# cvxgrp/pymde

Hardware: AMD Instinct MI355X
Metric: edges/sec/iter (avg_distortion fwd+bwd), n=1M |E|=50M d=2 (higher is better)
Workload: dtype f32; 1 GPU; BASELINE configs[3] / SURVEY 8d config 4a: n=1000000, |E|=50000000 uniform-random edges (out-degree 50), d=2, penalties.Log1p(1.5), weights in {1,2}; seeded on the device with torch.Generator(0) (the survey's recipe uses numpy default_rng(0): same distribution, another stream; --survey-seed builds that one); parallelism=single GPU, parameter_stream=codebook: 2 distinct weights ride in the packed half-edge word (4 B/half-edge)

## Files before the change

### include/mde_hip.h

```cpp
#ifndef MDE_HIP_H_
#define MDE_HIP_H_

#include <stdint.h>

#ifdef __cplusplus
extern "C" {
#endif

#define MDE_ABI_VERSION 2

#define MDE_OK 0
#define MDE_E_INVALID (-1)
#define MDE_E_SELF_EDGE (-2)
#define MDE_E_RANGE (-3)
#define MDE_E_TOO_LARGE (-4)
#define MDE_E_HIP (-5)
#define MDE_E_UNSUPPORTED (-6)

const char* mde_last_error(void);
int mde_abi_version(void);

enum {
  MDE_F_NONE = 0,
  MDE_F_LINEAR = 1,
  MDE_F_QUADRATIC = 2,
  MDE_F_CUBIC = 3,
  MDE_F_POWER = 4,
  MDE_F_HUBER = 5,
  MDE_F_LOGISTIC = 6,
  MDE_F_SIGMOID = 7,
  MDE_F_HINGE = 8,
  MDE_F_LOG1P = 9,
  MDE_F_LOG = 10,
  MDE_F_INVPOWER = 11,
  MDE_F_LOGRATIO = 12,
  MDE_F_DEADZONE_QUADRATIC = 13,
  MDE_F_DEADZONE_CUBIC = 14,
  MDE_F_CLIPPED_QUADRATIC = 15,
  MDE_F_L_QUADRATIC = 32,
  MDE_F_L_WEIGHTED_QUADRATIC = 33,
  MDE_F_L_HUBER = 34,
  MDE_F_L_CUBIC = 35,
  MDE_F_L_POWER = 36,
  MDE_F_L_WEIGHTED_POWER = 37,
  MDE_F_L_ABSOLUTE = 38,
  MDE_F_L_LOGISTIC = 39,
  MDE_F_L_FRACTIONAL = 40,
  MDE_F_L_SOFT_FRACTIONAL = 41,
  MDE_F_L_CLIPPED_QUADRATIC = 42,
  MDE_F_L_LOG1P = 43
};

typedef struct mde_func {
  int32_t kind;
  int32_t kind_neg;
  const float* a0;
  const float* a1;
  int32_t a0_scalar;
  int32_t a1_scalar;
  float s0, s1, s2;
  float n0, n1, n2;
  int32_t layout;
  const float* e0;
  const float* e1;
} mde_func;

typedef struct mde_plan mde_plan;

int mde_plan_create(int64_t n, int64_t p, const int64_t* edges, int64_t row_lo, int64_t row_hi,
                    void* stream, mde_plan** out);
int mde_plan_destroy(mde_plan* plan);
int64_t mde_plan_n(const mde_plan* plan);
int64_t mde_plan_p(const mde_plan* plan);
int64_t mde_plan_half_edges(const mde_plan* plan);
int64_t mde_plan_row_lo(const mde_plan* plan);
int64_t mde_plan_row_hi(const mde_plan* plan);
const int32_t* mde_plan_rowptr(const mde_plan* plan);
const int32_t* mde_plan_nbr(const mde_plan* plan);
const int32_t* mde_plan_eid(const mde_plan* plan);

int mde_plan_export(const mde_plan* plan, int32_t* rowptr_out, int32_t* nbr_out, int32_t* eid_out,
                    void* stream);

int mde_shard_bounds(int64_t n, int64_t p, const int64_t* edges, int32_t world,
                     int64_t* bounds_host, void* stream);

int mde_plan_expand(const mde_plan* plan, const float* in_edge, float* out_half, void* stream);

int mde_plan_layout(mde_plan* plan, int32_t d, void* stream);
int mde_plan_function_hint(mde_plan* plan, int32_t kind, int32_t kind_neg);
int64_t mde_plan_layout_half_edges(const mde_plan* plan, int32_t layout);
int mde_plan_expand_codebook(const mde_plan* plan, const float* in_edge, float* out_half,
                             int32_t* n_values_host, void* stream);
int mde_plan_expand_bytes(const mde_plan* plan, const float* in_edge, float* out_half,
                          int32_t* n_values_host, void* stream);
int mde_plan_expand_layout(const mde_plan* plan, int32_t layout, const float* in_edge,
                           float* out_half, void* stream);
int mde_plan_ring_info(const mde_plan* plan, int64_t* info_host);
int mde_plan_ring_check(const mde_plan* plan, int64_t* out_host, void* stream);
int mde_plan_row_order(mde_plan* plan, int32_t mode, void* stream, double* info_host);
int mde_plan_loss_double(const mde_plan* plan, double* dst, void* stream);

int mde_edges_deduplicate(int64_t n, int64_t p, const int64_t* edges, int64_t* edges_out,
                          int64_t* count_host, void* stream);
int mde_edges_count_unique(int64_t n, int64_t p, const int64_t* edges, int64_t* edges_out,
                           float* weights_out, int64_t* count_host, void* stream);
int mde_knn(int64_t n, int32_t nf, const float* data, int32_t k, int32_t* idx_out, float* d2_out,
            float* sqn_work, void* stream);
int mde_row_sqnorm(int64_t n, int32_t nf, const float* data, float* out, void* stream);
#define MDE_METRIC_EUCLIDEAN 0
#define MDE_METRIC_COSINE 1
#define MDE_METRIC_CORRELATION 2
#define MDE_METRIC_MANHATTAN 3
int mde_knn_l1(int64_t n, int32_t nf, const float* data, int32_t k, int32_t* idx_out, float* d_out,
               void* stream);
int mde_rows_normalize(int64_t n, int32_t nf, const float* data, int32_t center, float* out,
                       int32_t* deg_out, void* stream);
int mde_pair_distances_metric(int64_t n, int32_t nf, const float* data, int64_t p, const int64_t* edges,
                              int32_t metric, float* out, void* stream);
int mde_ann_search(int32_t nf, int32_t k, int32_t flags, int64_t n_q, const float* Q, const float* q_sqn,
                   int64_t n_qpos, const int32_t* q_map, int64_t n_b, const float* B, const float* b_sqn,
                   int64_t n_bpos, const int32_t* b_map, int64_t n_lists, const int64_t* offsets,
                   int32_t n_probe, const int32_t* probe, int64_t n_tiles, const int64_t* tiles,
                   int32_t* idx_out, float* d2_out, void* stream);
int mde_ann_centroids(int64_t n, int32_t nf, const float* data, int64_t n_members, const int32_t* members,
                      int64_t n_lists, const int64_t* offsets, float* centroids, void* stream);
int mde_sparse_validate(int64_t n, int32_t nf, int64_t nnz, const int64_t* indptr, const int32_t* indices,
                        const float* values, void* stream);
int mde_sparse_knn(int64_t n, int32_t nf, int64_t nnz, const int64_t* indptr, const int32_t* indices,
                   const float* values, int32_t k, int32_t* idx_out, float* d2_out, float* sqn_work,
                   void* stream);
int mde_sparse_distances(int64_t n, int32_t nf, int64_t nnz, const int64_t* indptr, const int32_t* indices,
                         const float* values, int64_t p, const int64_t* edges, float* out, void* stream);
int mde_sparse_rows_normalize(int64_t n, int32_t nf, int64_t nnz, const int64_t* indptr,
                              const int32_t* indices, const float* values, float* values_out,
                              int32_t* deg_out, void* stream);
int mde_graph_shortest_paths(const mde_plan* plan, const float* w, float max_length,
                             double retain_fraction, uint64_t seed, int64_t capacity,
                             int64_t* edges_out, float* dist_out, int64_t* count_host, void* stream);
int mde_knn_pairs(int64_t n, int32_t k, const int32_t* idx, const float* val, float max_value,
                  int64_t* pairs_out, void* stream);
int mde_graph_knn(const mde_plan* plan, const float* w, float max_length, int32_t direct, int32_t k,
                  int32_t* idx_out, float* dist_out, void* stream);
int mde_sample_edges(int64_t n, int64_t num_edges, uint64_t seed, const int64_t* exclude,
                     int64_t n_exclude, int64_t* edges_out, int64_t* count_host, void* stream);

int mde_average_distortion(mde_plan* plan, const float* X, int32_t d, const mde_func* f,
                           float grad_scale, float* grad, float* loss_out, void* stream);

int mde_differences(int64_t n, int64_t p, const int64_t* edges, const float* X, int32_t d,
                    float* diff_out , void* stream);
int mde_distances(int64_t n, int64_t p, const int64_t* edges, const float* X, int32_t d,
                  float* dist_out , void* stream);
int mde_distances_backward(const mde_plan* plan, const float* X, int32_t d, const float* gout,
                           float* grad , void* stream);
int mde_distortions(int64_t p, const float* dist, const mde_func* f, float* out, float* dout,
                    void* stream);

int mde_scatter(const mde_plan* plan, const float* X, int32_t d, const float* gnorm,
                const float* dist, float scale, float* grad, void* stream);

int mde_center(int64_t n, int32_t d, float* Z, double* work, void* stream);
int mde_anchor_rows(int64_t n_anchors, int32_t d, const int64_t* anchors, const float* values,
                    float* Z, void* stream);
int mde_sphere_rows(int64_t n, int32_t d, const float* X, float* Z, float radius, void* stream);
int mde_std_tangent(int64_t n, int32_t d, const float* X, float* Z, double* work, void* stream);
int mde_std_retract(int64_t n, int32_t d, float* Z, int32_t demean, double* work,
                    int32_t* status_dev, void* stream);
int mde_center_step(int64_t n, int32_t d, const float* X, const float* dir, float t, float* Z, double* work,
                    void* stream);
int mde_std_retract_step(int64_t n, int32_t d, const float* X, const float* dir, float t, float* Z,
                         int32_t demean, double* work, int32_t* status_dev, void* stream);
int mde_center_step_begin(int64_t n, int32_t d, const float* X, const float* dir, float t, float* Z, double* work,
                          void* stream);
int mde_center_step_end(int64_t n, int32_t d, float* Z, double* work, double scale, void* stream);
int mde_std_tangent_stats(int64_t n, int32_t d, const float* X, float* Z, const float* dir, double* stats,
                          double* work, void* stream);
int mde_gram(int64_t n, int32_t da, int32_t db, const float* A, const float* B, double* out,
             double* work, void* stream);
int mde_right_multiply(int64_t n, int32_t d, int32_t d2, const float* A, const double* M,
                       float* out, void* stream);
int mde_right_multiply_add(int64_t n, int32_t d, int32_t d2, const float* A, const double* M,
                           float alpha, const float* base, float* out, void* stream);
int mde_shift_rows(int64_t n, int32_t d, const double* shift, float* Z, void* stream);
int mde_row_scale(int64_t n, int32_t d, const float* scale, float* Z, void* stream);
int mde_weighted_degree(const mde_plan* plan, const float* w_plan_order, float* out, void* stream);
int64_t mde_work_doubles(int32_t d);

int mde_axpy(int64_t N, float alpha, const float* x, const float* y, float* out, void* stream);
int mde_vec_stats(int64_t N, const float* g, const float* d, const float* x, double* stats,
                  double* work, void* stream);

typedef struct mde_lbfgs mde_lbfgs;
int mde_lbfgs_create(int64_t N, int32_t history, mde_lbfgs** out);
int mde_lbfgs_destroy(mde_lbfgs* o);
int mde_lbfgs_reset(mde_lbfgs* o);
int32_t mde_lbfgs_count(const mde_lbfgs* o);
int mde_lbfgs_stage(mde_lbfgs* o, const float* g, float* g_prev, const float* d, float t,
                    double* dots, double* work, void* stream);
int mde_lbfgs_commit(mde_lbfgs* o, int32_t accept);
int mde_lbfgs_combine(mde_lbfgs* o, const float* g, float c_g, const float* cs, const float* cy,
                      float* d_out, double* stats, double* work, void* stream);
int mde_lbfgs_dev_reset(mde_lbfgs* o, void* stream);
int mde_lbfgs_dev_step(mde_lbfgs* o, const float* g, float* g_prev, const float* d, float t,
                       float* d_out, double* stats, double* work, void* stream);
int mde_lbfgs_dev_info(const mde_lbfgs* o, int32_t* count_host, int32_t* accepted_host, void* stream);
int mde_lbfgs_dev_stage(mde_lbfgs* o, const float* g, float* g_prev, const float* d, float t, double* work, void* stream);
int mde_lbfgs_dev_finish(mde_lbfgs* o, const float* g, float* d_out, double* stats, double* work, void* stream);
int32_t mde_lbfgs_dev_dots(const mde_lbfgs* o);
int mde_rank_reduce(int32_t world, int32_t count, uint64_t max_mask, const double* in, double* out,
                    int32_t loss_slot, float* loss_out, void* stream);
int mde_lbfgs_debug_knobs(int32_t unfused, int32_t blocks, int32_t spins, int32_t lds_bytes);

int mde_copy_to_host(void* dst_host, const void* src_dev, int64_t bytes, void* stream);

typedef struct mde_turn_desc {
  mde_plan* plan;
  const mde_func* func;
  int64_t n;
  int32_t d, kind;
  float* X[2];
  float* g;
  float* g_prev;
  float* dir;
  float* loss_dev;
  double* board;
  double* work;
  int32_t* status;
  mde_lbfgs* lbfgs;
  void* host_dst;
  const void* tail_src;
  int64_t read_bytes;
  const float* host_loss;
  const int32_t* host_status;
  const double* host_board;
  double seq;
  double pre_id;
} mde_turn_desc;
int mde_turn_enqueue(mde_turn_desc* T, int32_t cur, float t_prev, double f0, double c1, double c2,
                     int32_t allow_pre, void* stream);
int mde_turn_wait(mde_turn_desc* T, int32_t cur, double f0, int32_t allow_next, double c1, double c2,
                  double eps_pre, double* out, void* stream);

#ifdef __cplusplus
}
#endif
#endif
```

### pymde_amd/_lib.py

```python
import ctypes
import os
import threading

import torch

_HERE = os.path.dirname(os.path.abspath(__file__))
LIB_PATH = os.path.join(_HERE, "libmde_hip.so")

c_i32, c_i64, c_f32 = ctypes.c_int32, ctypes.c_int64, ctypes.c_float
c_vp = ctypes.c_void_p

MDE_OK = 0
MDE_E_INVALID, MDE_E_SELF_EDGE, MDE_E_RANGE = -1, -2, -3
MDE_E_TOO_LARGE, MDE_E_HIP, MDE_E_UNSUPPORTED = -4, -5, -6


class MdeFunc(ctypes.Structure):
    _fields_ = [("kind", c_i32), ("kind_neg", c_i32), ("a0", c_vp), ("a1", c_vp),
                ("a0_scalar", c_i32), ("a1_scalar", c_i32),
                ("s0", c_f32), ("s1", c_f32), ("s2", c_f32),
                ("n0", c_f32), ("n1", c_f32), ("n2", c_f32), ("layout", c_i32),
                ("e0", c_vp), ("e1", c_vp)]


class MdeTurnDesc(ctypes.Structure):
    _fields_ = [("plan", c_vp), ("func", c_vp), ("n", c_i64), ("d", c_i32), ("kind", c_i32),
                ("X", c_vp * 2), ("g", c_vp), ("g_prev", c_vp), ("dir", c_vp), ("loss_dev", c_vp),
                ("board", c_vp), ("work", c_vp), ("status", c_vp), ("lbfgs", c_vp),
                ("host_dst", c_vp), ("tail_src", c_vp), ("read_bytes", c_i64),
                ("host_loss", c_vp), ("host_status", c_vp), ("host_board", c_vp), ("seq", ctypes.c_double),
                ("pre_id", ctypes.c_double)]


SYMBOLS = {
    "mde_last_error": (ctypes.c_char_p, []),
    "mde_abi_version": (c_i32, []),
    "mde_plan_create": (c_i32, [c_i64, c_i64, c_vp, c_i64, c_i64, c_vp, ctypes.POINTER(c_vp)]),
    "mde_plan_destroy": (c_i32, [c_vp]),
    "mde_plan_n": (c_i64, [c_vp]),
    "mde_plan_p": (c_i64, [c_vp]),
    "mde_plan_half_edges": (c_i64, [c_vp]),
    "mde_plan_row_lo": (c_i64, [c_vp]),
    "mde_plan_row_hi": (c_i64, [c_vp]),
    "mde_plan_rowptr": (c_vp, [c_vp]),
    "mde_plan_nbr": (c_vp, [c_vp]),
    "mde_plan_eid": (c_vp, [c_vp]),
    "mde_plan_export": (c_i32, [c_vp, c_vp, c_vp, c_vp, c_vp]),
    "mde_shard_bounds": (c_i32, [c_i64, c_i64, c_vp, c_i32, ctypes.POINTER(c_i64), c_vp]),
    "mde_plan_expand": (c_i32, [c_vp, c_vp, c_vp, c_vp]),
    "mde_plan_layout": (c_i32, [c_vp, c_i32, c_vp]),
    "mde_plan_layout_half_edges": (c_i64, [c_vp, c_i32]),
    "mde_plan_ring_info": (c_i32, [c_vp, ctypes.POINTER(c_i64)]),
    "mde_plan_ring_check": (c_i32, [c_vp, ctypes.POINTER(c_i64), c_vp]),
    "mde_plan_row_order": (c_i32, [c_vp, c_i32, c_vp, ctypes.POINTER(ctypes.c_double)]),
    "mde_plan_function_hint": (c_i32, [c_vp, c_i32, c_i32]),
    "mde_plan_loss_double": (c_i32, [c_vp, c_vp, c_vp]),
    "mde_center_step_begin": (c_i32, [c_i64, c_i32, c_vp, c_vp, c_f32, c_vp, c_vp, c_vp]),
    "mde_center_step_end": (c_i32, [c_i64, c_i32, c_vp, c_vp, ctypes.c_double, c_vp]),
    "mde_lbfgs_dev_stage": (c_i32, [c_vp, c_vp, c_vp, c_vp, c_f32, c_vp, c_vp]),
    "mde_lbfgs_dev_finish": (c_i32, [c_vp, c_vp, c_vp, c_vp, c_vp, c_vp]),
    "mde_lbfgs_dev_dots": (c_i32, [c_vp]),
    "mde_rank_reduce": (c_i32, [c_i32, c_i32, ctypes.c_uint64, c_vp, c_vp, c_i32, c_vp, c_vp]),
    "mde_plan_expand_codebook": (c_i32, [c_vp, c_vp, c_vp, ctypes.POINTER(c_i32), c_vp]),
    "mde_plan_expand_bytes": (c_i32, [c_vp, c_vp, c_vp, ctypes.POINTER(c_i32), c_vp]),
    "mde_plan_expand_layout": (c_i32, [c_vp, c_i32, c_vp, c_vp, c_vp]),
    "mde_edges_deduplicate": (c_i32, [c_i64, c_i64, c_vp, c_vp, ctypes.POINTER(c_i64), c_vp]),
    "mde_edges_count_unique": (c_i32, [c_i64, c_i64, c_vp, c_vp, c_vp, ctypes.POINTER(c_i64), c_vp]),
    "mde_knn": (c_i32, [c_i64, c_i32, c_vp, c_i32, c_vp, c_vp, c_vp, c_vp]),
    "mde_row_sqnorm": (c_i32, [c_i64, c_i32, c_vp, c_vp, c_vp]),
    "mde_ann_search": (c_i32, [c_i32, c_i32, c_i32, c_i64, c_vp, c_vp, c_i64, c_vp, c_i64, c_vp, c_vp, c_i64, c_vp,
                               c_i64, c_vp, c_i32, c_vp, c_i64, c_vp, c_vp, c_vp, c_vp]),
    "mde_ann_centroids": (c_i32, [c_i64, c_i32, c_vp, c_i64, c_vp, c_i64, c_vp, c_vp, c_vp]),
    "mde_knn_l1": (c_i32, [c_i64, c_i32, c_vp, c_i32, c_vp, c_vp, c_vp]),
    "mde_rows_normalize": (c_i32, [c_i64, c_i32, c_vp, c_i32, c_vp, c_vp, c_vp]),
    "mde_pair_distances_metric": (c_i32, [c_i64, c_i32, c_vp, c_i64, c_vp, c_i32, c_vp, c_vp]),
    "mde_sparse_rows_normalize": (c_i32, [c_i64, c_i32, c_i64, c_vp, c_vp, c_vp, c_vp, c_vp, c_vp]),
    "mde_knn_pairs": (c_i32, [c_i64, c_i32, c_vp, c_vp, c_f32, c_vp, c_vp]),
    "mde_sparse_validate": (c_i32, [c_i64, c_i32, c_i64, c_vp, c_vp, c_vp, c_vp]),
    "mde_sparse_knn": (c_i32, [c_i64, c_i32, c_i64, c_vp, c_vp, c_vp, c_i32, c_vp, c_vp, c_vp, c_vp]),
    "mde_sparse_distances": (c_i32, [c_i64, c_i32, c_i64, c_vp, c_vp, c_vp, c_i64, c_vp, c_vp, c_vp]),
    "mde_graph_knn": (c_i32, [c_vp, c_vp, c_f32, c_i32, c_i32, c_vp, c_vp, c_vp]),
    "mde_graph_shortest_paths": (c_i32, [c_vp, c_vp, c_f32, ctypes.c_double, ctypes.c_uint64, c_i64,
                                         c_vp, c_vp, ctypes.POINTER(c_i64), c_vp]),
    "mde_sample_edges": (c_i32, [c_i64, c_i64, ctypes.c_uint64, c_vp, c_i64, c_vp,
                                 ctypes.POINTER(c_i64), c_vp]),
    "mde_average_distortion": (c_i32, [c_vp, c_vp, c_i32, ctypes.POINTER(MdeFunc), c_f32, c_vp,
                                       c_vp, c_vp]),
    "mde_differences": (c_i32, [c_i64, c_i64, c_vp, c_vp, c_i32, c_vp, c_vp]),
    "mde_distances": (c_i32, [c_i64, c_i64, c_vp, c_vp, c_i32, c_vp, c_vp]),
    "mde_distances_backward": (c_i32, [c_vp, c_vp, c_i32, c_vp, c_vp, c_vp]),
    "mde_distortions": (c_i32, [c_i64, c_vp, ctypes.POINTER(MdeFunc), c_vp, c_vp, c_vp]),
    "mde_scatter": (c_i32, [c_vp, c_vp, c_i32, c_vp, c_vp, c_f32, c_vp, c_vp]),
    "mde_center": (c_i32, [c_i64, c_i32, c_vp, c_vp, c_vp]),
    "mde_anchor_rows": (c_i32, [c_i64, c_i32, c_vp, c_vp, c_vp, c_vp]),
    "mde_sphere_rows": (c_i32, [c_i64, c_i32, c_vp, c_vp, c_f32, c_vp]),
    "mde_std_tangent": (c_i32, [c_i64, c_i32, c_vp, c_vp, c_vp, c_vp]),
    "mde_std_retract": (c_i32, [c_i64, c_i32, c_vp, c_i32, c_vp, c_vp, c_vp]),
    "mde_center_step": (c_i32, [c_i64, c_i32, c_vp, c_vp, c_f32, c_vp, c_vp, c_vp]),
    "mde_std_retract_step": (c_i32, [c_i64, c_i32, c_vp, c_vp, c_f32, c_vp, c_i32, c_vp, c_vp, c_vp]),
    "mde_std_tangent_stats": (c_i32, [c_i64, c_i32, c_vp, c_vp, c_vp, c_vp, c_vp, c_vp]),
    "mde_gram": (c_i32, [c_i64, c_i32, c_i32, c_vp, c_vp, c_vp, c_vp, c_vp]),
    "mde_right_multiply": (c_i32, [c_i64, c_i32, c_i32, c_vp, c_vp, c_vp, c_vp]),
    "mde_right_multiply_add": (c_i32, [c_i64, c_i32, c_i32, c_vp, c_vp, c_f32, c_vp, c_vp, c_vp]),
    "mde_shift_rows": (c_i32, [c_i64, c_i32, c_vp, c_vp, c_vp]),
    "mde_row_scale": (c_i32, [c_i64, c_i32, c_vp, c_vp, c_vp]),
    "mde_weighted_degree": (c_i32, [c_vp, c_vp, c_vp, c_vp]),
    "mde_work_doubles": (c_i64, [c_i32]),
    "mde_axpy": (c_i32, [c_i64, c_f32, c_vp, c_vp, c_vp, c_vp]),
    "mde_vec_stats": (c_i32, [c_i64, c_vp, c_vp, c_vp, c_vp, c_vp, c_vp]),
    "mde_lbfgs_create": (c_i32, [c_i64, c_i32, ctypes.POINTER(c_vp)]),
    "mde_lbfgs_destroy": (c_i32, [c_vp]),
    "mde_lbfgs_reset": (c_i32, [c_vp]),
    "mde_lbfgs_count": (c_i32, [c_vp]),
    "mde_lbfgs_stage": (c_i32, [c_vp, c_vp, c_vp, c_vp, c_f32, c_vp, c_vp, c_vp]),
    "mde_lbfgs_commit": (c_i32, [c_vp, c_i32]),
    "mde_lbfgs_dev_reset": (c_i32, [c_vp, c_vp]),
    "mde_lbfgs_dev_step": (c_i32, [c_vp, c_vp, c_vp, c_vp, c_f32, c_vp, c_vp, c_vp, c_vp]),
    "mde_lbfgs_debug_knobs": (c_i32, [c_i32, c_i32, c_i32, c_i32]),
    "mde_lbfgs_dev_info": (c_i32, [c_vp, ctypes.POINTER(c_i32), ctypes.POINTER(c_i32), c_vp]),
    "mde_lbfgs_combine": (c_i32, [c_vp, c_vp, c_f32, ctypes.POINTER(c_f32),
                                  ctypes.POINTER(c_f32), c_vp, c_vp, c_vp, c_vp]),
    "mde_copy_to_host": (c_i32, [c_vp, c_vp, c_i64, c_vp]),
    "mde_turn_enqueue": (c_i32, [c_vp, c_i32, c_f32, ctypes.c_double, ctypes.c_double, ctypes.c_double, c_i32, c_vp]),
    "mde_turn_wait": (c_i32, [c_vp, c_i32, ctypes.c_double, c_i32, ctypes.c_double, ctypes.c_double, ctypes.c_double,
                             c_vp, c_vp]),
}

_lib = None
_lock = threading.Lock()


class MdeHipError(RuntimeError):

    def __init__(self, code, message):
        super().__init__("libmde_hip error %d: %s" % (code, message))
        self.code = code
        self.message = message


def load():
    global _lib
    if _lib is not None:
        return _lib
    with _lock:
        if _lib is not None:
            return _lib
        from pymde_amd import _build
        if (not os.path.exists(LIB_PATH) or os.environ.get("PYMDE_AMD_REBUILD")
                or (_build._stale() and _build._hipcc() is not None)):
            _build.build(verbose=bool(os.environ.get("PYMDE_AMD_VERBOSE")))
        if not os.path.exists(LIB_PATH):
            raise ImportError(
                "pymde_amd: %s is missing and could not be built; the HIP extension is the "
                "only compute path (no CPU fallback)" % LIB_PATH)
        lib = ctypes.CDLL(os.environ.get("PYMDE_AMD_LIB_VARIANT") or LIB_PATH)
        for name, (res, args) in SYMBOLS.items():
            fn = getattr(lib, name)
            fn.restype = res
            fn.argtypes = args
        if lib.mde_abi_version() != 2:
            raise ImportError("pymde_amd: ABI version mismatch in %s" % LIB_PATH)
        _lib = lib
    return _lib


def last_error():
    msg = load().mde_last_error()
    return msg.decode(errors="replace") if msg else ""


def check(rc):
    if rc != MDE_OK:
        raise MdeHipError(rc, last_error())


def require_gpu():
    if not torch.cuda.is_available():
        raise RuntimeError(
            "pymde_amd needs an AMD GPU (MI355X / gfx950): torch.cuda.is_available() is False "
            "and there is no CPU path")


def ptr(t):
    return None if t is None else c_vp(t.data_ptr())


def stream_ptr(device=None):
    return c_vp(torch.cuda.current_stream(device).cuda_stream)
```

### pymde_amd/average_distortion.py

```python
import ctypes

import torch

from pymde_amd import _lib
from pymde_amd import util


def _check_X(X, n=None, d=None):
    if not isinstance(X, torch.Tensor) or X.dim() != 2:
        raise ValueError("the embedding must be a 2-D tensor")
    if X.dtype != torch.float32:
        raise ValueError(
            "pymde_amd computes in float32; got an embedding of dtype %s (MDE.embed and "
            "MDE.average_distortion cast float64 inputs with a warning; the kernels themselves do not)" % X.dtype)
    util.require_cuda_device(X.device)
    if n is not None and X.shape[0] != n:
        raise ValueError("embedding has %d rows, the problem has %d items" % (X.shape[0], n))


class EdgePlan(object):

    def __init__(self, n_items, edges, row_lo=0, row_hi=None):
        lib = _lib.load()
        device = util.require_cuda_device(edges.device)
        if edges.dtype != torch.int64 or edges.dim() != 2 or edges.shape[1] != 2:
            raise ValueError("edges must be an int64 tensor of shape (p, 2)")
        self.device = device
        self.n = int(n_items)
        self.p = int(edges.shape[0])
        self.edges = edges.contiguous()
        self.row_lo = int(row_lo)
        self.row_hi = self.n if row_hi is None else int(row_hi)
        handle = ctypes.c_void_p()
        with torch.cuda.device(device):
            rc = lib.mde_plan_create(self.n, self.p, _lib.ptr(self.edges), self.row_lo, self.row_hi,
                                     _lib.stream_ptr(device), ctypes.byref(handle))
        if rc == _lib.MDE_E_SELF_EDGE:
            offending = torch.where(self.edges[:, 0] == self.edges[:, 1])[0]
            raise ValueError(
                "The edge list must not contain self edges; the "
                "following rows were found to be self edges: ", offending.cpu().numpy())
        if rc == _lib.MDE_E_RANGE:
            raise ValueError("edges reference items outside [0, n_items): " + _lib.last_error())
        _lib.check(rc)
        self._handle = handle
        self.half_edges = int(lib.mde_plan_half_edges(handle))

    @property
    def handle(self):
        return self._handle

    @property
    def is_full(self):
        return self.row_lo == 0 and self.row_hi == self.n

    def expand(self, per_edge, layout=0):
        lib = _lib.load()
        t = per_edge.detach().to(device=self.device, dtype=torch.float32).contiguous().reshape(-1)
        if t.numel() != self.p:
            raise ValueError(
                "distortion function has %d parameters but the problem has %d edges"
                % (t.numel(), self.p))
        size = int(lib.mde_plan_layout_half_edges(self._handle, int(layout)))
        out = torch.empty(max(size, 1), dtype=torch.float32, device=self.device)
        with torch.cuda.device(self.device):
            _lib.check(lib.mde_plan_expand_layout(self._handle, int(layout), _lib.ptr(t),
                                                  _lib.ptr(out), _lib.stream_ptr(self.device)))
        return out

    def expand_codebook(self, per_edge):
        lib = _lib.load()
        t = per_edge.detach().to(device=self.device, dtype=torch.float32).contiguous().reshape(-1)
        if t.numel() != self.p:
            return None
        size = int(lib.mde_plan_layout_half_edges(self._handle, 1))
        out = torch.empty(max(size, 1), dtype=torch.float32, device=self.device)
        nv = ctypes.c_int32(0)
        with torch.cuda.device(self.device):
            _lib.check(lib.mde_plan_expand_codebook(self._handle, _lib.ptr(t), _lib.ptr(out),
                                                    ctypes.byref(nv), _lib.stream_ptr(self.device)))
        return out if nv.value > 0 else None

    def expand_bytes(self, per_edge):
        lib = _lib.load()
        t = per_edge.detach().to(device=self.device, dtype=torch.float32).contiguous().reshape(-1)
        if t.numel() != self.p:
            return None
        size = int(lib.mde_plan_layout_half_edges(self._handle, 1))
        out = torch.empty(max(size, 1), dtype=torch.float32, device=self.device)
        nv = ctypes.c_int32(0)
        with torch.cuda.device(self.device):
            _lib.check(lib.mde_plan_expand_bytes(self._handle, _lib.ptr(t), _lib.ptr(out),
                                                 ctypes.byref(nv), _lib.stream_ptr(self.device)))
        return out if nv.value > 0 else None

    def ring_info(self):
        lib = _lib.load()
        info = (ctypes.c_int64 * 16)()
        _lib.check(lib.mde_plan_ring_info(self._handle, info))
        names = ("built", "d", "rows_per_block", "row_blocks", "col_groups", "chunks", "ring_slots", "iterations",
                 "ring_half_edges", "padded_entries", "permuted", "hub_rows", "hub_half_edges", "hub_segments")
        out = {k: int(info[i]) for i, k in enumerate(names)}
        out["built"], out["permuted"] = bool(out["built"]), bool(out["permuted"])
        return out

    def ring_check(self):
        lib = _lib.load()
        out = (ctypes.c_int64 * 3)()
        with torch.cuda.device(self.device):
            _lib.check(lib.mde_plan_ring_check(self._handle, out, _lib.stream_ptr(self.device)))
        return {"split": int(out[0]), "shared": int(out[1]), "pairs": int(out[2])}

    def row_order(self, mode=1):
        lib = _lib.load()
        info = (ctypes.c_double * 4)()
        with torch.cuda.device(self.device):
            _lib.check(lib.mde_plan_row_order(self._handle, int(mode), _lib.stream_ptr(self.device), info))
        return {"in_use": bool(info[0]), "mean_distance_before": float(info[1]),
                "mean_distance_after": float(info[2]), "levels": int(info[3])}

    def csr(self):
        lib = _lib.load()
        nloc = self.row_hi - self.row_lo
        rowptr = torch.empty(nloc + 1, dtype=torch.int32, device=self.device)
        nbr = torch.empty(max(self.half_edges, 1), dtype=torch.int32, device=self.device)
        eid = torch.empty(max(self.half_edges, 1), dtype=torch.int32, device=self.device)
        with torch.cuda.device(self.device):
            _lib.check(lib.mde_plan_export(self._handle, _lib.ptr(rowptr), _lib.ptr(nbr),
                                           _lib.ptr(eid), _lib.stream_ptr(self.device)))
        return rowptr, nbr[:self.half_edges], eid[:self.half_edges]

    def __del__(self):
        h = getattr(self, "_handle", None)
        if h is not None and h.value:
            try:
                _lib.load().mde_plan_destroy(h)
            except Exception:
                pass
            self._handle = None


class Binding(object):

    def __init__(self, plan, function):
        self.plan = plan
        self.function = function
        self.spec = function._hip_spec() if hasattr(function, "_hip_spec") else None
        self._struct = None
        self._keep = None
        self._key = None
        self.codebook = False
        self.byte_stream = False
        self.stream_kind = None

    @property
    def fused(self):
        return self.spec is not None

    def _param_key(self, spec):
        return tuple((a.data_ptr(), a._version, a.numel(), str(a.device)) for a in spec.arrays()) + (
            spec.kind, spec.kind_neg, spec.scalars, spec.scalars_neg)

    def struct(self, d):
        lib = _lib.load()
        spec = self.function._hip_spec()
        key = self._param_key(spec) + (int(d),)
        if self._struct is None or key != self._key:
            plan = self.plan
            with torch.cuda.device(plan.device):
                _lib.check(lib.mde_plan_function_hint(plan.handle, int(spec.kind), int(spec.kind_neg)))
                layout = lib.mde_plan_layout(plan.handle, int(d), _lib.stream_ptr(plan.device))
            if layout < 0:
                _lib.check(layout)

            def prep(a):
                if a is None:
                    return None
                if a.numel() == 1:
                    return a.detach().to(device=plan.device, dtype=torch.float32).reshape(1).contiguous()
                return plan.expand(a, layout)
            a0 = None
            if layout == 1 and spec.a0 is not None and spec.a0.numel() > 1:
                a0 = plan.expand_codebook(spec.a0)
            self.codebook = a0 is not None
            self.byte_stream = False
            if a0 is None and layout == 1 and spec.a0 is not None and spec.a0.numel() > 1:
                a0 = plan.expand_bytes(spec.a0)
                self.byte_stream = a0 is not None
            if a0 is None:
                a0 = prep(spec.a0)
            a1 = prep(spec.a1)
            def edge_order(a):
                if a is None or a.numel() == 1:
                    return None
                return a.detach().to(device=plan.device, dtype=torch.float32).contiguous().reshape(-1)
            e0, e1 = (edge_order(spec.a0), edge_order(spec.a1)) if layout == 1 else (None, None)
            self._keep = (a0, a1, e0, e1)
            self._struct = spec.to_struct(a0, a1)
            self._struct.e0 = e0.data_ptr() if e0 is not None else None
            self._struct.e1 = e1.data_ptr() if e1 is not None else None
            if self.codebook:
                self._struct.a0_scalar = 2
            elif self.byte_stream:
                self._struct.a0_scalar = 3
            self.stream_kind = ("codebook" if self.codebook else "byte index" if self.byte_stream else
                                "scalar" if (spec.a0 is not None and spec.a0.numel() == 1) else "fp32")
            self._struct.layout = layout
            self._key = key
            self.spec = spec
        return self._struct


def fused_evaluate(binding, X, grad_out, loss_out, grad_scale=1.0):
    lib = _lib.load()
    plan = binding.plan
    f = binding.struct(X.shape[1])
    if X.data_ptr() & 15:
        X = X.clone()
    with torch.cuda.device(plan.device):
        _lib.check(lib.mde_average_distortion(
            plan.handle, _lib.ptr(X), X.shape[1], ctypes.byref(f), float(grad_scale),
            _lib.ptr(grad_out), _lib.ptr(loss_out), _lib.stream_ptr(plan.device)))


class _AverageDistortion(torch.autograd.Function):

    @staticmethod
    def forward(ctx, X, binding):
        plan = binding.plan
        _check_X(X, plan.n)
        if not plan.is_full:
            raise ValueError("use pymde_amd.distributed for sharded plans")
        Xc = X.detach().contiguous()
        loss = torch.empty(1, dtype=torch.float32, device=X.device)
        need_grad = X.requires_grad
        if binding.fused:
            grad = torch.empty_like(Xc) if need_grad else None
            fused_evaluate(binding, Xc, grad, loss)
        else:
            grad, value = _unfused(binding, Xc, need_grad)
            loss = value.reshape(1)
        if need_grad:
            ctx.save_for_backward(grad)
        return loss.reshape(())

    @staticmethod
    def backward(ctx, grad_output):
        (grad,) = ctx.saved_tensors
        return grad * grad_output, None


def _unfused(binding, X, need_grad):
    lib = _lib.load()
    plan = binding.plan
    f = binding.function
    n, d = X.shape
    dist = torch.empty(plan.p, dtype=torch.float32, device=X.device)
    with torch.cuda.device(plan.device):
        _lib.check(lib.mde_distances(n, plan.p, _lib.ptr(plan.edges), _lib.ptr(X), d, _lib.ptr(dist),
                                     _lib.stream_ptr(plan.device)))
    if not need_grad:
        with torch.no_grad():
            return None, f(dist).mean().to(torch.float32)
    with torch.enable_grad():
        norms = dist.detach().requires_grad_(True)
        distortion = f(norms).mean()
        (gnorm,) = torch.autograd.grad(distortion, norms)
    gnorm = gnorm.to(torch.float32).contiguous()
    grad = torch.empty_like(X)
    with torch.cuda.device(plan.device):
        _lib.check(lib.mde_scatter(plan.handle, _lib.ptr(X), d, _lib.ptr(gnorm), _lib.ptr(dist), 1.0,
                                   _lib.ptr(grad), _lib.stream_ptr(plan.device)))
    return grad, distortion.detach().to(torch.float32)


def average_distortion(X, binding):
    return _AverageDistortion.apply(X, binding)


class _Norm(torch.autograd.Function):

    @staticmethod
    def forward(ctx, X, plan):
        _check_X(X, plan.n)
        lib = _lib.load()
        Xc = X.detach().contiguous()
        n, d = Xc.shape
        dist = torch.empty(plan.p, dtype=torch.float32, device=X.device)
        with torch.cuda.device(plan.device):
            _lib.check(lib.mde_distances(n, plan.p, _lib.ptr(plan.edges), _lib.ptr(Xc), d,
                                         _lib.ptr(dist), _lib.stream_ptr(plan.device)))
        ctx.plan = plan
        ctx.save_for_backward(Xc)
        return dist

    @staticmethod
    def backward(ctx, grad_output):
        (Xc,) = ctx.saved_tensors
        plan = ctx.plan
        lib = _lib.load()
        gout = grad_output.detach().to(torch.float32).contiguous()
        grad = torch.empty_like(Xc)
        with torch.cuda.device(plan.device):
            _lib.check(lib.mde_distances_backward(plan.handle, _lib.ptr(Xc), Xc.shape[1],
                                                  _lib.ptr(gout), _lib.ptr(grad),
                                                  _lib.stream_ptr(plan.device)))
        return grad, None


def distances(X, plan):
    return _Norm.apply(X, plan)


def differences(X, plan):
    _check_X(X, plan.n)
    lib = _lib.load()
    Xc = X.detach().contiguous()
    n, d = Xc.shape
    out = torch.empty((plan.p, d), dtype=torch.float32, device=X.device)
    with torch.cuda.device(plan.device):
        _lib.check(lib.mde_differences(n, plan.p, _lib.ptr(plan.edges), _lib.ptr(Xc), d,
                                       _lib.ptr(out), _lib.stream_ptr(plan.device)))
    return out


_PLAN_CACHE = {}


def _gather_indices(idx, m):
    return idx[:, None].expand(idx.shape[0], m)


def _average_distortion(X, f, lhs, rhs):
    li = lhs[:, 0] if lhs.dim() == 2 else lhs
    ri = rhs[:, 0] if rhs.dim() == 2 else rhs
    def ident(t):
        return (t.untyped_storage().data_ptr(), t.storage_offset(), tuple(t.stride()), tuple(t.shape), t._version,
                str(t.dtype), str(t.device))
    key = (ident(lhs), ident(rhs), X.shape[0], str(X.device), id(f))
    hit = _PLAN_CACHE.get(key)
    if hit is not None and hit[3] is not f:
        hit = None
    if hit is None:
        edges = torch.stack([li, ri], dim=1).to(device=X.device, dtype=torch.int64).contiguous()
        binding = Binding(EdgePlan(X.shape[0], edges), f)
        if len(_PLAN_CACHE) > 8:
            _PLAN_CACHE.clear()
        hit = _PLAN_CACHE[key] = (binding, lhs.untyped_storage(), rhs.untyped_storage(), f)
    return _AverageDistortion.apply(X, hit[0])
```

### pymde_amd/csrc/mde_plan.h

```cpp
#pragma once
#include "mde_common.h"

struct mde_ring_layout {
  int d = 0;
  int rejected_d = 0;
  float cost_scale = 1.0f;
  int rows_per_block = 0, n_row_blocks = 0;
  int col_groups = 1;
  int chunk_cols = 0, n_chunks = 0;
  int ring_off = 0, slots = 0;
  int64_t n_iters = 0;
  int64_t H = 0;
  uint32_t* packed = nullptr;
  int32_t* eid = nullptr;
  uint32_t* hdr = nullptr;
  int32_t* wave_iter = nullptr;
  float* partial = nullptr;
  int32_t* slot_row = nullptr;
  int count_all = 0;
  int n_hub_rows = 0, n_hub_segs = 0;
  int64_t hub_half_edges = 0;
  int32_t* hub_rows = nullptr;
  int32_t* hub_seg = nullptr;
  int32_t* hub_first = nullptr;
  double* hub_partial = nullptr;
};
#define MDE_HUB_SEG 512

struct mde_plan {
  int64_t n = 0, p = 0, H = 0, row_lo = 0, row_hi = 0;
  int32_t* rowptr = nullptr;
  int32_t* nbr = nullptr;
  int32_t* eid = nullptr;
  double* partials = nullptr;
  float avg_degree = 0.f;
  mde_ring_layout ring;
  int64_t h_offset = 0;
  int32_t* hrow = nullptr;
  float* flat_rec = nullptr;
  int64_t n_tiles = 0;
  int has_empty = 0;
  int32_t* order = nullptr;
  int order_state = 0;
  double order_before = 0.0, order_after = 0.0;
  int order_levels = 0;
};

#define MDE_FLAT_U 4
#define MDE_FLAT_T (64 * MDE_FLAT_U)
int mde_plan_flat(mde_plan* plan, hipStream_t st);

hipError_t mde_sort_pairs_u32(void* tmp, size_t& tmp_bytes, const uint32_t* keys_in, uint32_t* keys_out,
                              const uint32_t* vals_in, uint32_t* vals_out, int n, int begin_bit, int end_bit,
                              hipStream_t st);
hipError_t mde_exclusive_sum_i32(void* tmp, size_t& tmp_bytes, const int32_t* in, int32_t* out, int n, hipStream_t st);
```

### pymde_amd/csrc/mde_ring.hip

```cpp
#include <algorithm>
#include <chrono>
#include <cmath>
#include <cstring>
#include <vector>

#include "mde_ring.h"

#ifndef MDE_RING_BUCKETS
#define MDE_RING_BUCKETS 32
#endif
__global__ __launch_bounds__(64) void k_ring_assign(int nloc, int R, int Q, int NC, int C, int contiguous,
                                                    const int32_t* __restrict__ rowptr,
                                                    const int32_t* __restrict__ nbr, uint32_t* __restrict__ wmap,
                                                    int32_t* __restrict__ wrows) {
  constexpr int B = MDE_RING_BUCKETS, NCWP = MDE_RING_NCW <= 8 ? 8 : 16, LPW = 64 / NCWP, BPL = B / LPW;
  static_assert(MDE_RING_NCW <= 16 && B % LPW == 0 && B <= 64, "lane map of k_ring_assign");
  __shared__ int hist[B];
  __shared__ float cpre[B];
  const int wg = blockIdx.x, rb = wg / Q, g = wg % Q, lane = threadIdx.x;
  const int j_lo = (int)(((int64_t)g * NC + Q - 1) / Q), j_hi = (int)(((int64_t)(g + 1) * NC + Q - 1) / Q);
  const int nj = max(1, j_hi - j_lo);
  const int r0 = rb * R, nr = min(R, nloc - r0);
  const int w = lane / LPW, bg = lane % LPW;
  uint32_t* out = wmap + (size_t)wg * R;
  if (contiguous) {
    const int64_t lo = rowptr[r0], hi = rowptr[r0 + nr];
    int bd[MDE_RING_NCW + 1];
    for (int t = 0; t <= MDE_RING_NCW; ++t) {
      const int64_t target = lo + ((hi - lo) * t) / MDE_RING_NCW;
      int a = r0, b = r0 + nr;
      while (a < b) {
        const int mid = (a + b) >> 1;
        if (rowptr[mid] >= target) b = mid; else a = mid + 1;
      }
      bd[t] = (t == MDE_RING_NCW) ? r0 + nr : a;
    }
    for (int r = lane; r < nr; r += 64) {
      int ww = 0;
      for (int t = 1; t < MDE_RING_NCW; ++t) ww += (bd[t] <= r0 + r);
      out[r] = (uint32_t)ww | ((uint32_t)(r0 + r - bd[ww]) << 8);
    }
    if (lane < MDE_RING_NCW) wrows[wg * MDE_RING_NCW + lane] = bd[lane + 1] - bd[lane];
    return;
  }
  float P[BPL], T[BPL];
#pragma unroll
  for (int k = 0; k < BPL; ++k) P[k] = T[k] = 0.0f;
  int myrows = 0;
  for (int r = 0; r < nr; ++r) {
    const int beg = rowptr[r0 + r], end = rowptr[r0 + r + 1];
    if (lane < B) hist[lane] = 0;
    __syncthreads();
    for (int q = beg + lane; q < end; q += 64) {
      const int j = nbr[q] / C;
      if (j >= j_lo && j < j_hi) atomicAdd(&hist[(int)(((int64_t)(j - j_lo) * B) / nj)], 1);
    }
    __syncthreads();
    int h = lane < B ? hist[lane] : 0;
#pragma unroll
    for (int o = 1; o < B; o <<= 1) {
      const int t = __shfl_up(h, o, 64);
      if (lane >= o) h += t;
    }
    if (lane < B) cpre[lane] = (float)h;
    __syncthreads();
    float c[BPL], cost = 0.0f;
#pragma unroll
    for (int k = 0; k < BPL; ++k) {
      c[k] = cpre[bg * BPL + k];
      cost = fmaf(P[k] - T[k] * (1.0f / MDE_RING_NCW), c[k], cost);
    }
#pragma unroll
    for (int o = 1; o < LPW; o <<= 1) cost += __shfl_xor(cost, o, 64);
    float bc = w < MDE_RING_NCW ? cost : 3.0e38f;
    int bn = myrows, bw = w;
#pragma unroll
    for (int o = LPW; o < 64; o <<= 1) {
      const float oc = __shfl_xor(bc, o, 64);
      const int on = __shfl_xor(bn, o, 64), ow = __shfl_xor(bw, o, 64);
      const bool take = oc < bc || (oc == bc && (on < bn || (on == bn && ow < bw)));
      bc = take ? oc : bc;
      bn = take ? on : bn;
      bw = take ? ow : bw;
    }
    if (lane == 0) out[r] = (uint32_t)bw | ((uint32_t)bn << 8);
#pragma unroll
    for (int k = 0; k < BPL; ++k) {
      T[k] += c[k];
      if (w == bw) P[k] += c[k];
    }
    myrows += (w == bw);
  }
  if (bg == 0 && w < MDE_RING_NCW) wrows[wg * MDE_RING_NCW + w] = myrows;
}

__global__ __launch_bounds__(MDE_BLOCK) void k_ring_keys(int nrows, const int32_t* __restrict__ rowptr,
                                                         const int32_t* __restrict__ nbr,
                                                         const uint32_t* __restrict__ wmap, int R, int Q,
                                                         int NC, int C, int JB, uint32_t* __restrict__ keys,
                                                         uint32_t* __restrict__ vals, int32_t* __restrict__ hrow) {
  constexpr int G = 16;
  const int lig = threadIdx.x & (G - 1);
  const int group = (blockIdx.x * MDE_BLOCK + threadIdx.x) / G;
  const int ngroups = (gridDim.x * MDE_BLOCK) / G;
  const int rmax = ((nrows + ngroups - 1) / ngroups) * ngroups;
  for (int r = group; r < rmax; r += ngroups) {
    const bool has = r < nrows;
    const int beg = has ? rowptr[r] : 0, end = has ? rowptr[r + 1] : 0;
    const int rb = has ? r / R : 0;
    const uint32_t wv = (has && lig < Q) ? (wmap[((size_t)rb * Q + lig) * R + (r - rb * R)] & 0xffu) : 0u;
    for (int q0 = beg; q0 < end; q0 += G) {
      const int q = q0 + lig;
      const bool in = q < end;
      const uint32_t j = in ? (uint32_t)(nbr[q] / C) : 0u;
      const uint32_t g = (uint32_t)(((uint64_t)j * (uint64_t)Q) / (uint64_t)NC);
      const uint32_t w = (uint32_t)__shfl((int)wv, (int)g, G);
      if (in) {
        keys[q] = ((((uint32_t)rb * (uint32_t)Q + g) * MDE_RING_NCW + w) << JB) | j;
        vals[q] = (uint32_t)q;
        hrow[q] = r;
      }
    }
  }
}

__global__ __launch_bounds__(64) void k_ring_assign_slots(int R, int Q, const int32_t* __restrict__ slot_cum,
                                                          uint32_t* __restrict__ wmap, int32_t* __restrict__ wrows) {
  const int wg = blockIdx.x, rb = wg / Q, lane = threadIdx.x;
  const int s0 = rb * R;
  uint32_t* out = wmap + (size_t)wg * R;
  const int64_t lo = slot_cum[s0], hi = slot_cum[s0 + R];
  int bd[MDE_RING_NCW + 1];
  for (int t = 0; t <= MDE_RING_NCW; ++t) {
    const int64_t target = lo + ((hi - lo) * t) / MDE_RING_NCW;
    int a = s0, b = s0 + R;
    while (a < b) {
      const int mid = (a + b) >> 1;
      if (slot_cum[mid] >= target) b = mid; else a = mid + 1;
    }
    bd[t] = (t == MDE_RING_NCW) ? s0 + R : a;
  }
  for (int r = lane; r < R; r += 64) {
    int ww = 0;
    for (int t = 1; t < MDE_RING_NCW; ++t) ww += (bd[t] <= s0 + r);
    out[r] = (uint32_t)ww | ((uint32_t)(s0 + r - bd[ww]) << 8);
  }
  if (lane < MDE_RING_NCW) wrows[wg * MDE_RING_NCW + lane] = bd[lane + 1] - bd[lane];
}

__global__ __launch_bounds__(MDE_BLOCK) void k_ring_keys_slots(int64_t H, const int32_t* __restrict__ nbr,
                                                               const int32_t* __restrict__ row_slot,
                                                               const uint32_t* __restrict__ wmap, int R, int Q, int NC, int C,
                                                               int JB, uint32_t nseg, uint32_t* __restrict__ keys,
                                                               uint32_t* __restrict__ vals, int32_t* __restrict__ hrow) {
  for (int64_t q = (int64_t)blockIdx.x * MDE_BLOCK + threadIdx.x; q < H; q += (int64_t)gridDim.x * MDE_BLOCK) {
    const int sl = row_slot[hrow[q]];
    vals[q] = (uint32_t)q;
    if (sl < 0) {
      keys[q] = nseg << JB;
      hrow[q] = 0;
      continue;
    }
    const int rb = sl / R;
    const uint32_t j = (uint32_t)(nbr[q] / C);
    const uint32_t g = (uint32_t)(((uint64_t)j * (uint64_t)Q) / (uint64_t)NC);
    const uint32_t w = wmap[((size_t)rb * Q + g) * R + (sl - rb * R)] & 0xffu;
    keys[q] = ((((uint32_t)rb * (uint32_t)Q + g) * MDE_RING_NCW + w) << JB) | j;
    hrow[q] = sl;
  }
}
__global__ __launch_bounds__(MDE_BLOCK) void k_ring_rows_to_slots(int64_t H, const int32_t* __restrict__ row_slot,
                                                                  int32_t* __restrict__ hrow) {
  for (int64_t q = (int64_t)blockIdx.x * MDE_BLOCK + threadIdx.x; q < H; q += (int64_t)gridDim.x * MDE_BLOCK)
    hrow[q] = max(row_slot[hrow[q]], 0);
}

__global__ __launch_bounds__(MDE_BLOCK) void k_ring_gather_u32(int64_t H, const uint32_t* __restrict__ idx,
                                                               const uint32_t* __restrict__ in,
                                                               uint32_t* __restrict__ out) {
  for (int64_t h = (int64_t)blockIdx.x * MDE_BLOCK + threadIdx.x; h < H; h += (int64_t)gridDim.x * MDE_BLOCK)
    out[h] = in[idx[h]];
}

__global__ __launch_bounds__(MDE_BLOCK) void k_ring_hrow(int nrows, const int32_t* __restrict__ rowptr,
                                                         int32_t* __restrict__ hrow) {
  constexpr int G = 16;
  const int lig = threadIdx.x & (G - 1);
  const int group = (blockIdx.x * MDE_BLOCK + threadIdx.x) / G;
  const int ngroups = (gridDim.x * MDE_BLOCK) / G;
  for (int r = group; r < nrows; r += ngroups)
    for (int q = rowptr[r] + lig; q < rowptr[r + 1]; q += G) hrow[q] = r;
}

__global__ __launch_bounds__(MDE_BLOCK) void k_ring_seg(int64_t H, uint32_t nseg, int JB,
                                                        const uint32_t* __restrict__ keys,
                                                        int32_t* __restrict__ seg) {
  for (int64_t h = (int64_t)blockIdx.x * MDE_BLOCK + threadIdx.x; h <= H;
       h += (int64_t)gridDim.x * MDE_BLOCK) {
    const int64_t prev = (h == 0) ? -1 : (int64_t)(keys[h - 1] >> JB);
    int64_t cur = (h == H) ? (int64_t)nseg : (int64_t)(keys[h] >> JB);
    if (cur > (int64_t)nseg) cur = nseg;
    for (int64_t t = prev + 1; t <= cur; ++t) seg[t] = (int32_t)h;
  }
}

#ifndef MDE_RING_FORCE
#define MDE_RING_FORCE 3
#endif
#ifndef MDE_RING_CARRY
#define MDE_RING_CARRY 256
#endif
#ifndef MDE_RING_ROUNDS
#define MDE_RING_ROUNDS 6
#endif
__host__ __device__ constexpr int ring_cls_shift(int d) { return d == 2 ? 3 : (d == 4 ? 4 : 2); }
__host__ __device__ constexpr int ring_cls_mask(int d) { return d == 4 ? 15 : 31; }
__global__ __launch_bounds__(MDE_BLOCK) void k_ring_meta(int64_t H, const uint32_t* __restrict__ keys,
                                                         const uint32_t* __restrict__ vals,
                                                         const int32_t* __restrict__ hrow,
                                                         const int32_t* __restrict__ nbr,
                                                         const uint32_t* __restrict__ wmap, int JB, int R, int Q, int d,
                                                         uint32_t* __restrict__ meta) {
  const int sh = ring_cls_shift(d), cm = ring_cls_mask(d), rowbytes = 4 * d;
  for (int64_t pos = (int64_t)blockIdx.x * MDE_BLOCK + threadIdx.x; pos < H; pos += (int64_t)gridDim.x * MDE_BLOCK) {
    const uint32_t q = vals[pos];
    const int wg = (int)((keys[pos] >> JB) / MDE_RING_NCW), rb = wg / Q;
    const uint32_t row = (uint32_t)(hrow[q] - rb * R);
    const uint32_t rc = ((row * (uint32_t)rowbytes) >> sh) & (uint32_t)cm;
    const uint32_t cc = (((uint32_t)nbr[q] * (uint32_t)rowbytes) >> sh) & (uint32_t)cm;
    meta[pos] = (wmap[(size_t)wg * R + row] >> 8) | (rc << 16) | (cc << 24);
  }
}

template <bool FILL>
__global__ __launch_bounds__(64) void k_ring_schedule(int nseg, const int32_t* __restrict__ seg,
                                                      const int32_t* __restrict__ wrows,
                                                      const uint32_t* __restrict__ keys,
                                                      const uint32_t* __restrict__ meta, uint32_t JM, int SPAN,
                                                      int R, int Q, int NC, int d, int cap, int bail_factor,
                                                      int32_t* __restrict__ iters,
                                                      const int32_t* __restrict__ iter_base,
                                                      int32_t* __restrict__ it_ent, int32_t* __restrict__ it_cnt,
                                                      int32_t* __restrict__ it_m, int flag_rows,
                                                      const int32_t* __restrict__ caps) {
  extern __shared__ int flag[];
  __shared__ int cq_pos[2][MDE_RING_CARRY];
  __shared__ uint32_t cq_meta[2][MDE_RING_CARRY];
  __shared__ int cq_chunk[2][MDE_RING_CARRY];
  __shared__ int cq_age[2][MDE_RING_CARRY];
  __shared__ int em[64], em_row[64];
  __shared__ int rcnt[32], ccnt[32];
  const int i = blockIdx.x, lane = threadIdx.x;
  if (i >= nseg) return;
  for (int r = lane; r < flag_rows; r += 64) flag[r] = 0x7fffffff;
  __syncthreads();
  const int beg = seg[i], end = seg[i + 1];
  constexpr int row_base = 0;
  const int first = FILL ? iter_base[i] : 0;
  int out = first, next = beg, nc = 0, cur = 0;
  const int nrows_w = max(1, wrows[i]);
  const int per_it = nrows_w < 64 ? nrows_w : 64;
  const int walk = 2 * ((NC / Q + SPAN + 1) / (SPAN + 1));
  const int bail = caps ? caps[i] - 4
                        : ((!FILL && bail_factor > 0) ? bail_factor * max((end - beg + per_it - 1) / per_it, walk) + 64 : 0x7fffffff);
  int last_chunk = (int)(((int64_t)((i / MDE_RING_NCW) % Q) * NC + Q - 1) / Q);
  int m_lead = 0;
  while (nc > 0 || next < end) {
    const int m = nc > 0 ? cq_chunk[cur][0] : (int)(keys[next] & JM);
    if (((out - first) & 1) == 0) m_lead = m;
    const int lim = m_lead + SPAN;
    int nem = 0, nnew = 0, mx = 0;
    if (lane < 32) rcnt[lane] = ccnt[lane] = 0;
    __syncthreads();
    auto offer = [&](int pos, uint32_t mw, int chunk, int age, int prio) {
      const int row = pos >= 0 ? (int)(mw & 0xffffu) - row_base : 0;
      const int rc = pos >= 0 ? (int)((mw >> 16) & 0xffu) : -1, cc = pos >= 0 ? (int)(mw >> 24) : -2;
      if (pos >= 0) atomicMin(&flag[row], prio);
      __syncthreads();
      const bool rowwin = pos >= 0 && flag[row] == prio;
      int rkR = 0, rkC = 0;
      const int rcw = rowwin ? rc : -1, ccw = rowwin ? cc : -2;
      for (int c = 0; c < 32; ++c) {
        const unsigned long long mr = __ballot(rcw == c), mc = __ballot(ccw == c);
        if (rc == c) rkR = __popcll(mr & ((1ull << lane) - 1ull));
        if (cc == c) rkC = __popcll(mc & ((1ull << lane) - 1ull));
      }
      const bool capok = rowwin && (rcnt[rc] + rkR < cap) && (ccnt[cc] + rkC < cap);
      const bool win = rowwin && (capok || age >= MDE_RING_FORCE);
      const unsigned long long wm = __ballot(win);
      const int widx = nem + __popcll(wm & ((1ull << lane) - 1ull));
      const bool emit = win && widx < 64;
      if (emit) {
        em[widx] = pos;
        em_row[widx] = row;
        atomicAdd(&rcnt[rc], 1);
        atomicAdd(&ccnt[cc], 1);
      }
      mx = max(mx, emit ? chunk : 0);
      const bool lose = pos >= 0 && !emit;
      const unsigned long long lm = __ballot(lose);
      const int lidx = nnew + __popcll(lm & ((1ull << lane) - 1ull));
      if (lose && lidx < MDE_RING_CARRY) {
        cq_pos[cur ^ 1][lidx] = pos;
        cq_meta[cur ^ 1][lidx] = mw;
        cq_chunk[cur ^ 1][lidx] = chunk;
        cq_age[cur ^ 1][lidx] = win ? age : age + 1;
      }
      nem += __popcll(__ballot(emit));
      nnew += __popcll(lm);
      __syncthreads();
    };
    int prio = 0;
    for (int c0 = 0; c0 < nc; c0 += 64) {
      const int k = c0 + lane;
      const bool has = k < nc;
      offer(has ? cq_pos[cur][k] : -1, has ? cq_meta[cur][k] : 0u, has ? cq_chunk[cur][k] : 0, has ? cq_age[cur][k] : 0,
            prio + lane);
      prio += 64;
    }
    for (int round = 0; round < MDE_RING_ROUNDS && nem < 64 && next < end && nnew + 64 <= MDE_RING_CARRY; ++round) {
      const int want = 64 - nem;
      const int cand = next + lane;
      const bool in = lane < want && cand < end;
      const int chunk = in ? (int)(keys[cand] & JM) : 0x7fffffff;
      const bool take = in && chunk <= lim;
      const int ntake = __popcll(__ballot(take));
      if (ntake == 0) break;
      offer(take ? cand : -1, take ? meta[cand] : 0u, chunk, 0, prio + lane);
      prio += 64;
      next += ntake;
    }
    if (lane < nem) flag[em_row[lane]] = 0x7fffffff;
    for (int k = lane; k < nnew; k += 64) flag[(int)(cq_meta[cur ^ 1][k] & 0xffffu) - row_base] = 0x7fffffff;
    mx = mde_wave_max(mx);
    if (nem > 0) last_chunk = mx;
    if (FILL) {
      if (lane < nem) it_ent[(size_t)out * 64 + lane] = em[lane];
      if (lane == 0) {
        it_cnt[out] = nem | (last_chunk << 8);
        it_m[out] = m;
      }
    }
    ++out;
    nc = nnew;
    cur ^= 1;
    __syncthreads();
    if (out - first > bail) {
      if (lane == 0) iters[i] = 1 << 25;
      return;
    }
  }
  while ((out - first) & 3) {
    if (FILL && lane == 0) {
      it_cnt[out] = 0 | (last_chunk << 8);
      it_m[out] = last_chunk;
    }
    ++out;
  }
  if (iters && lane == 0) iters[i] = out - first;
}

__global__ __launch_bounds__(MDE_BLOCK) void k_ring_caps(int nseg, const int32_t* __restrict__ seg,
                                                         const int32_t* __restrict__ wrows, int R, int Q, int NC, int SPAN,
                                                         int factor, int32_t* __restrict__ caps) {
  const int i = blockIdx.x * MDE_BLOCK + threadIdx.x;
  if (i > nseg) return;
  if (i == nseg) {
    caps[i] = 0;
    return;
  }
  const int nrows_w = max(1, wrows[i]);
  const int per_it = nrows_w < 64 ? nrows_w : 64;
  const int walk = 2 * ((NC / Q + SPAN + 1) / (SPAN + 1));
  const int need = max((seg[i + 1] - seg[i] + per_it - 1) / per_it, walk);
  caps[i] = (factor * need + 64 + 4 + 3) & ~3;
}

__device__ __forceinline__ int ring_place_wave(bool act, int rc, int lane) {
  const unsigned long long lt = (1ull << lane) - 1ull;
  int rank = 0, par = 0, oddacc = 0;
  for (int c = 0; c < 32; ++c) {
    const unsigned long long m = __ballot(act && rc == c);
    if (rc == c) {
      rank = __popcll(m & lt);
      par = oddacc & 1;
    }
    oddacc += __popcll(m) & 1;
  }
  const int half = (rank + par) & 1;
  int quarter = 0;
  for (int h = 0; h < 2; ++h) {
    int oa = 0;
    for (int c = 0; c < 16; ++c) {
      const unsigned long long m = __ballot(act && half == h && (rc & 15) == c);
      if (half == h && (rc & 15) == c) quarter = (__popcll(m & lt) + (oa & 1)) & 1;
      oa += __popcll(m) & 1;
    }
  }
  int pos = 0;
  for (int g = 0; g < 4; ++g) {
    const unsigned long long m = __ballot(act && half * 2 + quarter == g);
    if (half * 2 + quarter == g) pos = __popcll(m & lt);
  }
  return half * 32 + quarter * 16 + pos;
}

__global__ __launch_bounds__(MDE_BLOCK) void k_ring_pack(int64_t nit, int nseg, const int32_t* __restrict__ iter_base,
                                                         const int32_t* __restrict__ src_base,
                                                         const int32_t* __restrict__ it_ent,
                                                         const int32_t* __restrict__ it_cnt,
                                                         const int32_t* __restrict__ it_m,
                                                         const uint32_t* __restrict__ keys,
                                                         const uint32_t* __restrict__ vals,
                                                         const int32_t* __restrict__ hrow,
                                                         const int32_t* __restrict__ nbr,
                                                         const int32_t* __restrict__ eid, int R, int Q, int C, int S,
                                                         int ring_off, int JB, int d, int row_lo, int place, int count_all,
                                                         uint32_t* __restrict__ packed,
                                                         int32_t* __restrict__ peid, uint32_t* __restrict__ hdr) {
  __shared__ uint8_t s_taken[MDE_BLOCK / 64][64], s_free[MDE_BLOCK / 64][64];
  __shared__ uint32_t s_prow[MDE_BLOCK / 64][64];
  const int lane = threadIdx.x & 63, wv = threadIdx.x >> 6;
  const int64_t nw = ((int64_t)gridDim.x * MDE_BLOCK) >> 6;
  const uint32_t JM = (1u << JB) - 1u;
  const int sh = ring_cls_shift(d), cm = ring_cls_mask(d);
  const uint32_t cbytes = (uint32_t)C * 4u * (uint32_t)d;
  for (int64_t itb = (int64_t)blockIdx.x * (MDE_BLOCK / 64); itb < nit; itb += nw) {
    const int64_t it = itb + wv;
    const bool valid = it < nit;
    int64_t src = it;
    if (valid && src_base) {
      int lo = 0, hi = nseg;
      while (hi - lo > 1) {
        const int mid = (lo + hi) >> 1;
        if ((int64_t)iter_base[mid] <= it) lo = mid; else hi = mid;
      }
      src = (int64_t)src_base[lo] + (it - (int64_t)iter_base[lo]);
    }
    const int cw = valid ? __builtin_amdgcn_readfirstlane(it_cnt[src]) : 0;
    const int cnt = cw & 0xff;
    const bool act = valid && lane < cnt;
    uint32_t key = 0, q = 0, col = 0, rowaddr = 0, ring = 0;
    int grow = 0, rcls = 0;
    if (act) {
      const int pos = it_ent[(size_t)src * 64 + lane];
      key = keys[pos];
      q = vals[pos];
      const int rb = (int)((key >> JB) / MDE_RING_NCW) / Q;
      grow = hrow[q];
      rowaddr = (uint32_t)(grow - rb * R) * 4u * (uint32_t)d;
      const uint32_t j = key & JM;
      col = (uint32_t)nbr[q];
      ring = (uint32_t)ring_off + (j % (uint32_t)S) * cbytes + (col - j * (uint32_t)C) * 4u * (uint32_t)d;
      rcls = (int)((rowaddr >> sh) & (uint32_t)cm);
    }
    s_taken[wv][lane] = 0;
    s_prow[wv][lane] = 0xffffffffu;
    __syncthreads();
    const bool second = (it & 1) != 0;
    int l = lane;
    if (!second) {
      if (place) l = ring_place_wave(act, rcls, lane);
      if (act) {
        s_taken[wv][l] = 1;
        s_prow[wv][l] = rowaddr;
      }
    }
    __syncthreads();
    int pin = -1;
    if (second) {
      const uint32_t prow = s_prow[wv - 1][lane];
#pragma unroll 8
      for (int k = 0; k < 64; ++k)
        if ((uint32_t)__builtin_amdgcn_readlane((int)prow, k) == rowaddr) pin = k;
      pin = act ? pin : -1;
      if (place) l = ring_place_wave(act && pin < 0, rcls, lane);
      if (pin >= 0) {
        l = pin;
        s_taken[wv][l] = 1;
      }
    }
    __syncthreads();
    const bool moved = second && act && pin < 0 && s_taken[wv][l];
    if (second && act && !moved) s_taken[wv][l] = 1;
    __syncthreads();
    {
      const bool fr = !s_taken[wv][lane];
      const unsigned long long fm = __ballot(fr);
      if (fr) s_free[wv][__popcll(fm & ((1ull << lane) - 1ull))] = (uint8_t)lane;
    }
    __syncthreads();
    const unsigned long long mvm = __ballot(moved);
    const int nmoved = __popcll(mvm);
    if (moved) l = s_free[wv][__popcll(mvm & ((1ull << lane) - 1ull))];
    const bool counts = act && (count_all || (uint32_t)(row_lo + grow) < col);
    const int ncount = __popcll(__ballot(counts));
    const uint32_t lclass = ncount == 0 ? 0u : (ncount == cnt ? 1u : 2u);
    const uint32_t m = valid ? (uint32_t)__builtin_amdgcn_readfirstlane(it_m[src]) : 0u;
    const uint32_t need = max((uint32_t)(cw >> 8), m);
    const uint32_t mpad = valid ? (uint32_t)__builtin_amdgcn_readfirstlane(it_m[src & ~(int64_t)1]) : 0u;
    const size_t base = ((size_t)(it >> 2) * 64) * 4 + (size_t)(it & 3);
    if (act) {
      packed[base + (size_t)l * 4] = ring_pack_word(d, rowaddr, ring);
      peid[base + (size_t)l * 4] = eid[q];
    } else if (valid) {
      const int lf = s_free[wv][nmoved + lane - cnt];
      packed[base + (size_t)lf * 4] = ring_pack_word(d, (uint32_t)(R + (lf & 31)) * 4u * (uint32_t)d,
                                                     (uint32_t)ring_off + (mpad % (uint32_t)S) * cbytes);
      peid[base + (size_t)lf * 4] = -1;
    }
    if (lane == 0 && valid) {
      hdr[MDE_RING_HW * it] = m;
      hdr[MDE_RING_HW * it + 1] = need;
      hdr[MDE_RING_HW * it + 2] = lclass;
      hdr[MDE_RING_HW * it + 3] = (cnt < 64 ? MDE_RING_H3_PAD : 0u) | ((uint32_t)cnt << 8);
    }
    __syncthreads();
  }
}

__global__ __launch_bounds__(MDE_BLOCK) void k_ring_block_class(int64_t nblocks, uint32_t* __restrict__ hdr) {
  const int64_t b = (int64_t)blockIdx.x * MDE_BLOCK + threadIdx.x;
  if (b >= nblocks) return;
  bool any0 = false, any1 = false, any2 = false;
  for (int q = 0; q < 4; ++q) {
    const uint32_t* h = hdr + (size_t)MDE_RING_HW * (4 * b + q);
    if ((h[3] >> 8) == 0u) continue;
    any0 |= h[2] == 0u;
    any1 |= h[2] == 1u;
    any2 |= h[2] == 2u;
  }
  const uint32_t cls = (any2 || (any0 && any1)) ? 2u : (any1 ? 1u : 0u);
  hdr[(size_t)MDE_RING_HW * 4 * b + 3] = (hdr[(size_t)MDE_RING_HW * 4 * b + 3] & ~3u) | cls;
  for (int t = 0; t < 2; ++t) {
    uint32_t* h0 = hdr + (size_t)MDE_RING_HW * (4 * b + 2 * t);
    uint32_t* h1 = h0 + MDE_RING_HW;
    uint32_t need = h0[0];
    if ((h0[3] >> 8) != 0u) need = max(need, h0[1]);
    if ((h1[3] >> 8) != 0u) need = max(need, h1[1]);
    h0[1] = need;
  }
}

__global__ __launch_bounds__(MDE_BLOCK) void k_ring_stats(int64_t nit, const uint32_t* __restrict__ hdr,
                                                          unsigned long long* __restrict__ stats) {
  unsigned long long a = 0, b = 0, c = 0;
  for (int64_t i = (int64_t)blockIdx.x * MDE_BLOCK + threadIdx.x; i < nit; i += (int64_t)gridDim.x * MDE_BLOCK) {
    a += (hdr[MDE_RING_HW * i + 3] & MDE_RING_H3_PAD) ? 1u : 0u;
    b += hdr[MDE_RING_HW * i + 2] == 1u;
    c += hdr[MDE_RING_HW * i + 2] == 2u;
  }
  a = mde_wave_sum(a);
  b = mde_wave_sum(b);
  c = mde_wave_sum(c);
  if ((threadIdx.x & 63) == 0) {
    atomicAdd(&stats[0], a);
    atomicAdd(&stats[1], b);
    atomicAdd(&stats[2], c);
  }
}

__global__ __launch_bounds__(MDE_BLOCK) void k_ring_sweep_balance(int nwg, int ngroups, int GW, int JB,
                                                                  const uint32_t* __restrict__ keys,
                                                                  const int32_t* __restrict__ seg,
                                                                  unsigned long long* __restrict__ crit,
                                                                  unsigned long long* __restrict__ tot) {
  const int64_t idx = (int64_t)blockIdx.x * MDE_BLOCK + threadIdx.x;
  if (idx >= (int64_t)nwg * ngroups) return;
  const int wg = (int)(idx / ngroups), g = (int)(idx % ngroups);
  unsigned long long mx = 0, sm = 0;
  for (int w = 0; w < MDE_RING_NCW; ++w) {
    const uint32_t s = (uint32_t)wg * MDE_RING_NCW + (uint32_t)w;
    const int32_t lo = seg[s], hi = seg[s + 1];
    const uint64_t k0 = ((uint64_t)s << JB) + (uint64_t)g * GW, k1 = k0 + (uint64_t)GW;
    auto lower = [&](uint64_t key) {
      int32_t a = lo, b = hi;
      while (a < b) {
        const int32_t m = a + ((b - a) >> 1);
        if ((uint64_t)keys[m] < key) a = m + 1; else b = m;
      }
      return a;
    };
    const unsigned long long c = (unsigned long long)(lower(k1) - lower(k0));
    mx = c > mx ? c : mx;
    sm += c;
  }
  if (sm) {
    atomicAdd(&crit[wg], mx);
    atomicAdd(&tot[wg], sm);
  }
}

static int panel_mode() {
  const char* e = getenv("MDE_PANEL");
  return e ? atoi(e) : -1;
}

static int bits_for_u64(uint64_t maxval) {
  int b = 1;
  while (b < 64 && (maxval >> b)) ++b;
  return b;
}

struct RingSizes {
  int R, NRB, Q, C, NC, S, JB, ring_off, span, qmax;
};

static double ring_time_us(double iters_per_wave, int NC, int Q, int nwg) {
  const double rounds = std::ceil((double)nwg / 256.0);
  return rounds * std::max(0.21 * iters_per_wave, 0.14 * (double)NC / (double)Q);
}
static double csr_time_us(const mde_plan* plan, int d) {
  return (double)plan->H * ((int64_t)plan->n * d * 4 >= (6 << 20) ? 1.3e-5 : 0.6e-5);
}
static bool mid_regime(const mde_plan* plan, int d) {
  return (int64_t)plan->n * d * 4 < (6 << 20) && plan->H < ((int64_t)16 << 20);
}
#define MDE_RING_FIXED_US 11.0
#define MDE_CSR_FIXED_US 7.0
static double function_cost_scale(int kind, int kind_neg) {
  if (kind_neg != MDE_F_NONE) return 1.3;
  switch (kind) {
    case MDE_F_LOG1P: case MDE_F_QUADRATIC: case MDE_F_LINEAR: case MDE_F_CUBIC: case MDE_F_INVPOWER: case MDE_F_HUBER:
    case MDE_F_L_QUADRATIC: case MDE_F_L_WEIGHTED_QUADRATIC: case MDE_F_L_ABSOLUTE: case MDE_F_L_HUBER: case MDE_F_L_CUBIC:
      return 1.05;
    case MDE_F_LOGISTIC: case MDE_F_POWER: case MDE_F_LOG: case MDE_F_SIGMOID: case MDE_F_HINGE: case MDE_F_LOGRATIO:
    case MDE_F_L_POWER: case MDE_F_L_LOGISTIC: case MDE_F_L_FRACTIONAL: case MDE_F_L_SOFT_FRACTIONAL:
      return 1.35;
    default:
      return 2.7;
  }
}
extern "C" int mde_plan_function_hint(mde_plan* plan, int32_t kind, int32_t kind_neg) {
  if (!plan) return MDE_E_INVALID;
  plan->ring.cost_scale = (float)function_cost_scale(kind, kind_neg);
  return MDE_OK;
}

static int choose_col_groups(const mde_plan* plan, int64_t nrb, int qmax, int64_t nc) {
  int Q = (int)std::min<int64_t>(qmax, std::max<int64_t>(1, 256 / nrb));
  const double its1 = 1.4 * (double)plan->H / ((double)nrb * MDE_RING_NCW * 64.0);
  auto cost = [&](int q) {
    const double rounds = std::ceil((double)(nrb * q) / 256.0);
    return ring_time_us(its1 / q, (int)nc, q, (int)(nrb * q)) + 4.0 * rounds;
  };
  const double base = cost(Q);
  double best = base;
  for (int q = 1; q <= qmax; ++q)
    if ((int64_t)nrb * q <= MDE_MAX_PARTIALS && cost(q) < 0.95 * base && cost(q) < best) {
      best = cost(q);
      Q = q;
    }
  if (getenv("MDE_RING_Q")) Q = std::max(1, std::min(qmax, atoi(getenv("MDE_RING_Q"))));
  return Q;
}

static bool choose_sizes(const mde_plan* plan, int d, RingSizes* z) {
  const int64_t nloc = plan->row_hi - plan->row_lo;
  if (d < 1 || d > 4 || nloc <= 0 || plan->H <= 0) return false;
  const int mode = panel_mode();
  if (mode == 0) return false;
  const int C = ring_chunk_cols(d);
  const int64_t nc = (plan->n + C - 1) / C;
  if (nc > 65535 || nc < 2) return false;
  const int minch = getenv("MDE_RING_MINCH") ? std::max(1, atoi(getenv("MDE_RING_MINCH"))) : 10;
  const int qmax = (int)std::min<int64_t>(16, std::max<int64_t>(1, nc / minch));
  int64_t pr = (nloc * qmax + 255) / 256;
  if (pr < 64 * MDE_RING_NCW) pr = 64 * MDE_RING_NCW;
  if (getenv("MDE_RING_ROWS")) pr = atoi(getenv("MDE_RING_ROWS"));
  if (pr > nloc) pr = nloc;
  pr = ((pr + 63) / 64) * 64;
  const int64_t pr_max = ring_row_cap(d);
  if (pr > pr_max) pr = pr_max;
  const int64_t nrb = (nloc + pr - 1) / pr;
  int Q = choose_col_groups(plan, nrb, qmax, nc);
  if (nrb * Q > MDE_MAX_PARTIALS) return false;
  const int jb = bits_for_u64((uint64_t)nc - 1);
  if (bits_for_u64((uint64_t)(nrb * Q * MDE_RING_NCW)) + jb > 32) return false;
  if (mode != 1) {
    if (mid_regime(plan, d) && d != 2 && d != 3) return false;
  }
  const int S = ring_slots_for(d, (int)pr);
  if (S < 6) return false;
  int span = ring_max_span(S);
  if (getenv("MDE_RING_SPAN")) span = std::min(S - 2, std::max(1, atoi(getenv("MDE_RING_SPAN"))));
  if (mode != 1) {
    const double its = 1.4 * (double)plan->H / ((double)nrb * Q * MDE_RING_NCW * 64.0);
    if (ring_time_us(its, (int)nc, Q, (int)(nrb * Q)) > 0.75 * csr_time_us(plan, d)) return false;
    if (mid_regime(plan, d) &&
        plan->ring.cost_scale * ring_time_us(its, (int)nc, Q, (int)(nrb * Q)) + MDE_RING_FIXED_US >
            0.7 * (csr_time_us(plan, d) + MDE_CSR_FIXED_US))
      return false;
  }
  z->qmax = qmax;
  z->R = (int)pr;
  z->NRB = (int)nrb;
  z->Q = Q;
  z->C = C;
  z->NC = (int)nc;
  z->S = S;
  z->ring_off = ring_off_for(d, (int)pr);
  z->span = span;
  z->JB = jb;
  return true;
}

static void ring_free(mde_ring_layout& L) {
  if (L.packed) (void)hipFree(L.packed);
  if (L.eid) (void)hipFree(L.eid);
  if (L.hdr) (void)hipFree(L.hdr);
  if (L.wave_iter) (void)hipFree(L.wave_iter);
  if (L.partial) (void)hipFree(L.partial);
  void* extra[] = {L.slot_row, L.hub_rows, L.hub_seg, L.hub_first, L.hub_partial};
  for (void* q : extra)
    if (q) (void)hipFree(q);
  L = mde_ring_layout();
}
void mde_ring_release(mde_plan* plan) { ring_free(plan->ring); }

struct RowPlan {
  bool mapped = false, permuted = false;
  int nrb = 0;
  int64_t H_ring = 0;
  std::vector<int32_t> row_slot;
  std::vector<int32_t> slot_row;
  std::vector<int32_t> slot_cum;
  std::vector<int32_t> hub_rows, hub_first, hub_seg;
  int64_t hub_half_edges = 0;
  int threshold = 0;
};

static int plan_rows(const mde_plan* plan, const RingSizes& z, hipStream_t st, RowPlan* rp) {
  const int64_t nloc = plan->row_hi - plan->row_lo;
  const int R = z.R;
  rp->nrb = z.NRB;
  rp->H_ring = plan->H;
  const char* e_hub = getenv("MDE_RING_HUB");
  const char* e_perm = getenv("MDE_RING_PERMUTE");
  const int hub_env = e_hub ? atoi(e_hub) : -1, perm_env = e_perm ? atoi(e_perm) : -1;
  if (hub_env == 0 && perm_env == 0) return MDE_OK;
  std::vector<int32_t> rowptr((size_t)nloc + 1);
  MDE_HIP(hipMemcpyAsync(rowptr.data(), plan->rowptr, rowptr.size() * sizeof(int32_t), hipMemcpyDeviceToHost, st));
  MDE_HIP(hipStreamSynchronize(st));
  const int64_t H = plan->H;
  int T = (int)std::max<int64_t>(256, H / ((int64_t)z.NRB * MDE_RING_NCW * 128));
  if (hub_env > 0) T = hub_env;
  rp->threshold = T;
  int64_t hub_he = 0;
  int32_t max_deg = 0;
  if (hub_env != 0) {
    for (int64_t r = 0; r < nloc; ++r) {
      const int32_t deg = rowptr[r + 1] - rowptr[r];
      max_deg = std::max(max_deg, deg);
      if (deg > T) {
        rp->hub_rows.push_back((int32_t)r);
        hub_he += deg;
      }
    }
    if (2 * hub_he > H) {
      rp->hub_rows.clear();
      hub_he = 0;
    }
  }
  const bool peel = !rp->hub_rows.empty();
  bool permute = perm_env == 1;
  if (perm_env < 0) {
    int64_t heaviest = 0;
    size_t hi = 0;
    for (int b = 0; b < z.NRB; ++b) {
      const int64_t r0 = (int64_t)b * R, r1 = std::min<int64_t>(nloc, r0 + R);
      int64_t w = rowptr[r1] - rowptr[r0];
      while (hi < rp->hub_rows.size() && rp->hub_rows[hi] < r1) {
        w -= rowptr[rp->hub_rows[hi] + 1] - rowptr[rp->hub_rows[hi]];
        ++hi;
      }
      heaviest = std::max(heaviest, w);
    }
    permute = z.NRB > 1 && (double)heaviest > 1.08 * (double)(H - hub_he) / (double)z.NRB;
  }
  if (!peel && !permute) return MDE_OK;
  rp->mapped = true;
  rp->permuted = permute;
  rp->hub_half_edges = hub_he;
  rp->H_ring = H - hub_he;
  rp->row_slot.assign((size_t)nloc, -1);
  std::vector<uint8_t> is_hub((size_t)nloc, 0);
  for (int32_t r : rp->hub_rows) is_hub[(size_t)r] = 1;
  if (!permute) {
    rp->slot_cum.assign((size_t)z.NRB * R + 1, 0);
    int64_t cum = 0;
    for (int64_t r = 0; r < (int64_t)z.NRB * R; ++r) {
      rp->slot_cum[(size_t)r] = (int32_t)cum;
      if (r < nloc && !is_hub[(size_t)r]) {
        rp->row_slot[(size_t)r] = (int32_t)r;
        cum += rowptr[r + 1] - rowptr[r];
      }
    }
    rp->slot_cum[(size_t)z.NRB * R] = (int32_t)cum;
  } else {
    const int64_t nring = nloc - (int64_t)rp->hub_rows.size();
    const int nrb = (int)std::max<int64_t>(1, (nring + R - 1) / R);
    rp->nrb = nrb;
    int32_t dmax = 0;
    for (int64_t r = 0; r < nloc; ++r)
      if (!is_hub[(size_t)r]) dmax = std::max(dmax, rowptr[r + 1] - rowptr[r]);
    std::vector<int64_t> start((size_t)dmax + 2, 0);
    for (int64_t r = 0; r < nloc; ++r)
      if (!is_hub[(size_t)r]) ++start[(size_t)(dmax - (rowptr[r + 1] - rowptr[r])) + 1];
    for (size_t k = 1; k < start.size(); ++k) start[k] += start[k - 1];
    std::vector<int32_t> block((size_t)nloc, -1);
    for (int64_t r = 0; r < nloc; ++r) {
      if (is_hub[(size_t)r]) continue;
      const int64_t rank = start[(size_t)(dmax - (rowptr[r + 1] - rowptr[r]))]++;
      const int64_t pos = rank % (2 * (int64_t)nrb);
      block[(size_t)r] = (int32_t)(pos < nrb ? pos : 2 * (int64_t)nrb - 1 - pos);
    }
    std::vector<int32_t> fill((size_t)nrb, 0);
    rp->slot_row.assign((size_t)nrb * R, -1);
    std::vector<int32_t> slot_deg((size_t)nrb * R, 0);
    for (int64_t r = 0; r < nloc; ++r) {
      const int b = block[(size_t)r];
      if (b < 0) continue;
      const int sidx = fill[(size_t)b]++;
      if (sidx >= R) {
        mde_set_error("ring layout: a row block overflowed while the rows were dealt (internal error)");
        return MDE_E_INVALID;
      }
      const size_t sl = (size_t)b * R + (size_t)sidx;
      rp->slot_row[sl] = (int32_t)r;
      rp->row_slot[(size_t)r] = (int32_t)sl;
      slot_deg[sl] = rowptr[r + 1] - rowptr[r];
    }
    rp->slot_cum.assign((size_t)nrb * R + 1, 0);
    int64_t cum = 0;
    for (size_t t = 0; t < (size_t)nrb * R; ++t) {
      rp->slot_cum[t] = (int32_t)cum;
      cum += slot_deg[t];
    }
    rp->slot_cum[(size_t)nrb * R] = (int32_t)cum;
  }
  rp->hub_first.reserve(rp->hub_rows.size() + 1);
  for (size_t i = 0; i < rp->hub_rows.size(); ++i) {
    rp->hub_first.push_back((int32_t)(rp->hub_seg.size() / 4));
    const int32_t r = rp->hub_rows[i];
    for (int64_t b = rowptr[r]; b < rowptr[r + 1]; b += MDE_HUB_SEG) {
      rp->hub_seg.push_back((int32_t)i);
      rp->hub_seg.push_back((int32_t)b);
      rp->hub_seg.push_back((int32_t)std::min<int64_t>(rowptr[r + 1], b + MDE_HUB_SEG));
      rp->hub_seg.push_back(0);
    }
  }
  rp->hub_first.push_back((int32_t)(rp->hub_seg.size() / 4));
  if (getenv("MDE_RING_STATS"))
    fprintf(stderr, "[mde ring] rows: threshold %d half-edges, max degree %d, %zu hub rows with %lld half-edges (%.2f%%) peeled into %zu "
            "segments; blocks %s (%d)\n", T, max_deg, rp->hub_rows.size(), (long long)hub_he, 100.0 * (double)hub_he / (double)std::max<int64_t>(H, 1),
            rp->hub_seg.size() / 4, permute ? "DEALT by degree" : "of consecutive rows", rp->nrb);
  return MDE_OK;
}

static hipError_t any_stream_bailed(const int32_t* iters, int nseg, hipStream_t st, int32_t* total) {
  std::vector<int32_t> h((size_t)nseg);
  hipError_t e = hipMemcpyAsync(h.data(), iters, h.size() * sizeof(int32_t), hipMemcpyDeviceToHost, st);
  if (e == hipSuccess) e = hipStreamSynchronize(st);
  if (e != hipSuccess) return e;
  for (int i = 0; i < nseg; ++i)
    if (h[(size_t)i] >= (1 << 25)) {
      *total = -1;
      break;
    }
  return hipSuccess;
}

static int build_ring(mde_plan* plan, int d, hipStream_t st) {
  RingSizes z;
  if (!choose_sizes(plan, d, &z)) return 0;
  const int64_t nloc = plan->row_hi - plan->row_lo;
  const int64_t H = plan->H;
  RowPlan rp;
  {
    const int rc = plan_rows(plan, z, st, &rp);
    if (rc != MDE_OK) return rc;
    if (rp.mapped && rp.nrb != z.NRB) {
      z.NRB = rp.nrb;
      z.Q = choose_col_groups(plan, z.NRB, z.qmax, z.NC);
      if ((int64_t)z.NRB * z.Q > MDE_MAX_PARTIALS || bits_for_u64((uint64_t)((int64_t)z.NRB * z.Q * MDE_RING_NCW)) + z.JB > 32) return 0;
    }
  }
  const int64_t H_ring = rp.H_ring;
  if (H_ring <= 0) return 0;
  const int nseg = z.NRB * z.Q * MDE_RING_NCW;
  const uint32_t JM = (1u << z.JB) - 1u;
  uint32_t *keys = nullptr, *vals = nullptr, *keys2 = nullptr, *vals2 = nullptr, *packed = nullptr, *hdr = nullptr, *wmap = nullptr;
  int32_t *hrow = nullptr, *wrows = nullptr, *seg = nullptr, *iters = nullptr, *iter_base = nullptr;
  int32_t *it_ent = nullptr, *it_cnt = nullptr, *it_m = nullptr, *peid = nullptr;
  int32_t *row_slot = nullptr, *slot_cum = nullptr, *slot_row = nullptr, *hub_rows = nullptr, *hub_seg = nullptr, *hub_first = nullptr;
  double* hub_partial = nullptr;
  float* partial = nullptr;
  void* tmp = nullptr;
  hipError_t e = hipSuccess;
  auto release = [&](bool all) {
    void* scratch[] = {keys, vals, keys2, vals2, hrow, wrows, wmap, seg, iters, it_ent, it_cnt, it_m, tmp, row_slot, slot_cum};
    for (void* p : scratch)
      if (p) (void)hipFree(p);
    if (all) {
      void* outs[] = {packed, hdr, peid, iter_base, partial, slot_row, hub_rows, hub_seg, hub_first, hub_partial};
      for (void* p : outs)
        if (p) (void)hipFree(p);
    }
  };
  auto fail = [&](hipError_t err, const char* what) {
    release(true);
    return mde_hip_fail(err, what, __FILE__, __LINE__);
  };
#define RB(call)                                 \
  do {                                           \
    e = (call);                                  \
    if (e != hipSuccess) return fail(e, #call);  \
  } while (0)
  const bool stats_on = getenv("MDE_RING_STATS") != nullptr;
  auto t_last = std::chrono::steady_clock::now();
  auto tick = [&](const char* what) {
    if (!stats_on) return;
    (void)hipStreamSynchronize(st);
    const auto t1 = std::chrono::steady_clock::now();
    fprintf(stderr, "[mde ring build] %-28s %8.2f ms\n", what, std::chrono::duration<double, std::milli>(t1 - t_last).count());
    t_last = t1;
  };
  const size_t hb = (size_t)H * sizeof(uint32_t);
  RB(hipMalloc(&keys, hb));
  RB(hipMalloc(&vals, hb));
  RB(hipMalloc(&keys2, hb));
  RB(hipMalloc(&vals2, hb));
  RB(hipMalloc(&hrow, hb));
  RB(hipMalloc(&wrows, ((size_t)nseg + 1) * sizeof(int32_t)));
  RB(hipMalloc(&wmap, (size_t)z.NRB * z.Q * z.R * sizeof(uint32_t)));
  RB(hipMalloc(&seg, ((size_t)nseg + 1) * sizeof(int32_t)));
  RB(hipMalloc(&iters, ((size_t)nseg + 1) * sizeof(int32_t)));
  RB(hipMalloc(&iter_base, ((size_t)nseg + 1) * sizeof(int32_t)));
  tick("scratch allocations");
  const int contiguous = getenv("MDE_RING_ASSIGN") ? atoi(getenv("MDE_RING_ASSIGN")) == 0 : 1;
  auto upload = [&](int32_t** dst, const std::vector<int32_t>& src) -> hipError_t {
    hipError_t er = hipMalloc(dst, std::max<size_t>(src.size(), 1) * sizeof(int32_t));
    if (er == hipSuccess && !src.empty()) er = hipMemcpyAsync(*dst, src.data(), src.size() * sizeof(int32_t), hipMemcpyHostToDevice, st);
    return er;
  };
  if (rp.mapped) {
    RB(upload(&row_slot, rp.row_slot));
    RB(upload(&slot_cum, rp.slot_cum));
    if (rp.permuted) RB(upload(&slot_row, rp.slot_row));
    if (!rp.hub_rows.empty()) {
      RB(upload(&hub_rows, rp.hub_rows));
      RB(upload(&hub_seg, rp.hub_seg));
      RB(upload(&hub_first, rp.hub_first));
      RB(hipMalloc(&hub_partial, (rp.hub_seg.size() / 4) * 8 * sizeof(double)));
    }
    hipLaunchKernelGGL(k_ring_assign_slots, dim3(z.NRB * z.Q), dim3(64), 0, st, z.R, z.Q, slot_cum, wmap, wrows);
    RB(hipGetLastError());
    tick("slot -> wave assignment");
    hipLaunchKernelGGL(k_ring_hrow, dim3(mde_grid(nloc * 16, MDE_BLOCK, 4096)), dim3(MDE_BLOCK), 0, st, (int)nloc, plan->rowptr, hrow);
    RB(hipGetLastError());
    hipLaunchKernelGGL(k_ring_keys_slots, dim3(mde_grid(H, MDE_BLOCK, 8192)), dim3(MDE_BLOCK), 0, st, H, plan->nbr, row_slot, wmap, z.R,
                       z.Q, z.NC, z.C, z.JB, (uint32_t)nseg, keys, vals, hrow);
    RB(hipGetLastError());
  } else {
    hipLaunchKernelGGL(k_ring_assign, dim3(z.NRB * z.Q), dim3(64), 0, st, (int)nloc, z.R, z.Q, z.NC, z.C, contiguous, plan->rowptr,
                       plan->nbr, wmap, wrows);
    RB(hipGetLastError());
    tick("row -> wave assignment");
    hipLaunchKernelGGL(k_ring_keys, dim3(mde_grid(nloc * 16, MDE_BLOCK, 4096)), dim3(MDE_BLOCK), 0, st, (int)nloc,
                       plan->rowptr, plan->nbr, wmap, z.R, z.Q, z.NC, z.C, z.JB, keys, vals, hrow);
    RB(hipGetLastError());
  }
  tick("keys kernel");
  size_t tmp_bytes = 0, scan_bytes = 0;
  const int end_bit = std::min(32, bits_for_u64((uint64_t)nseg) + z.JB);
  RB(mde_sort_pairs_u32(nullptr, tmp_bytes, keys, keys2, vals, vals2, (int)H, 0, end_bit, st));
  RB(mde_exclusive_sum_i32(nullptr, scan_bytes, iters, iter_base, nseg + 1, st));
  if (scan_bytes > tmp_bytes) tmp_bytes = scan_bytes;
  RB(mde_sort_pairs_u32(nullptr, scan_bytes, keys, keys2, vals, vals2, (int)H, 0,
                                        bits_for_u64((uint64_t)plan->n), st));
  if (scan_bytes > tmp_bytes) tmp_bytes = scan_bytes;
  RB(hipMalloc(&tmp, tmp_bytes ? tmp_bytes : 16));
  tick("sort size queries + temp allocation");
  const bool by_column = getenv("MDE_RING_BYCOL") ? atoi(getenv("MDE_RING_BYCOL")) != 0
                                                  : (double)H_ring > 0.5 * (double)nloc * (double)z.NC;
  if (by_column) {
    RB(hipMemcpyAsync(keys2, plan->nbr, hb, hipMemcpyDeviceToDevice, st));
    uint32_t* skey = reinterpret_cast<uint32_t*>(hrow);
    RB(hipMemcpyAsync(skey, keys, hb, hipMemcpyDeviceToDevice, st));
    RB(mde_sort_pairs_u32(tmp, tmp_bytes, keys2, keys, vals, vals2, (int)H, 0,
                                          bits_for_u64((uint64_t)plan->n), st));
    hipLaunchKernelGGL(k_ring_gather_u32, dim3(mde_grid(H, MDE_BLOCK, 4096)), dim3(MDE_BLOCK), 0, st, H, vals2, skey, keys);
    RB(hipGetLastError());
    RB(hipMemcpyAsync(vals, vals2, hb, hipMemcpyDeviceToDevice, st));
    hipLaunchKernelGGL(k_ring_hrow, dim3(mde_grid(nloc * 16, MDE_BLOCK, 4096)), dim3(MDE_BLOCK), 0, st, (int)nloc,
                       plan->rowptr, hrow);
    RB(hipGetLastError());
    if (rp.mapped) {
      hipLaunchKernelGGL(k_ring_rows_to_slots, dim3(mde_grid(H, MDE_BLOCK, 8192)), dim3(MDE_BLOCK), 0, st, H, row_slot, hrow);
      RB(hipGetLastError());
    }
  }
  RB(mde_sort_pairs_u32(tmp, tmp_bytes, keys, keys2, vals, vals2, (int)H, 0, end_bit, st));
  tick("radix sort");
  hipLaunchKernelGGL(k_ring_seg, dim3(mde_grid(H + 1, MDE_BLOCK, 4096)), dim3(MDE_BLOCK), 0, st, H, (uint32_t)nseg,
                     z.JB, keys2, seg);
  RB(hipGetLastError());
  RB(hipMemsetAsync(iters, 0, ((size_t)nseg + 1) * sizeof(int32_t), st));
  tick("keys, sorts, segments");
  const int cap_default = d == 4 ? 8 : 4;
  const int cap = getenv("MDE_RING_CAP") ? std::max(1, atoi(getenv("MDE_RING_CAP"))) : cap_default;
  const int place = getenv("MDE_RING_PLACE") ? atoi(getenv("MDE_RING_PLACE")) : 1;
  const int span = z.span;
  uint32_t* meta = keys;
  hipLaunchKernelGGL(k_ring_meta, dim3(mde_grid(H_ring, MDE_BLOCK, 8192)), dim3(MDE_BLOCK), 0, st, H_ring, keys2, vals2, hrow, plan->nbr,
                     wmap, z.JB, z.R, z.Q, d, meta);
  RB(hipGetLastError());
  int flag_rows = 64;
  {
    std::vector<int32_t> hwr((size_t)nseg);
    RB(hipMemcpyAsync(hwr.data(), wrows, hwr.size() * sizeof(int32_t), hipMemcpyDeviceToHost, st));
    RB(hipStreamSynchronize(st));
    for (int i = 0; i < nseg; ++i) flag_rows = std::max(flag_rows, hwr[(size_t)i]);
    flag_rows = (flag_rows + 63) / 64 * 64;
  }
  const size_t flag_bytes = (size_t)flag_rows * sizeof(int);
  int32_t *caps = nullptr, *cap_base = nullptr;
  RB(hipMalloc(&caps, ((size_t)nseg + 1) * sizeof(int32_t)));
  RB(hipMalloc(&cap_base, ((size_t)nseg + 1) * sizeof(int32_t)));
  auto drop_caps = [&]() {
    if (caps) (void)hipFree(caps);
    if (cap_base) (void)hipFree(cap_base);
    caps = cap_base = nullptr;
  };
  int32_t total_iters = 0, total_cap = 0;
  hipLaunchKernelGGL(k_ring_caps, dim3((nseg + 1 + MDE_BLOCK - 1) / MDE_BLOCK), dim3(MDE_BLOCK), 0, st, nseg, seg, wrows, z.R, z.Q,
                     z.NC, span, 2, caps);
  e = hipGetLastError();
  if (e == hipSuccess) e = mde_exclusive_sum_i32(tmp, tmp_bytes, caps, cap_base, nseg + 1, st);
  if (e == hipSuccess) e = hipMemcpyAsync(&total_cap, cap_base + nseg, sizeof(int32_t), hipMemcpyDeviceToHost, st);
  if (e == hipSuccess) e = hipStreamSynchronize(st);
  bool single = e == hipSuccess && total_cap > 0 && (int64_t)total_cap * 64 < ((int64_t)1 << 33);
  if (e != hipSuccess) {
    drop_caps();
    return fail(e, "ring layout: stream capacities");
  }
  if (single) {
    e = hipMalloc(&it_ent, (size_t)total_cap * 64 * sizeof(int32_t));
    if (e == hipSuccess) e = hipMalloc(&it_cnt, (size_t)total_cap * sizeof(int32_t));
    if (e == hipSuccess) e = hipMalloc(&it_m, (size_t)total_cap * sizeof(int32_t));
    if (e != hipSuccess) {
      (void)hipGetLastError();
      single = false;
      void* ps[] = {it_ent, it_cnt, it_m};
      for (void* q : ps)
        if (q) (void)hipFree(q);
      it_ent = it_cnt = it_m = nullptr;
    }
  }
  if (single) {
    hipLaunchKernelGGL(k_ring_schedule<true>, dim3(nseg), dim3(64), flag_bytes, st, nseg, seg, wrows, keys2, meta, JM, span, z.R,
                       z.Q, z.NC, d, cap, 4, iters, cap_base, it_ent, it_cnt, it_m, flag_rows, caps);
    e = hipGetLastError();
    if (e == hipSuccess) e = mde_exclusive_sum_i32(tmp, tmp_bytes, iters, iter_base, nseg + 1, st);
    if (e == hipSuccess) e = hipMemcpyAsync(&total_iters, iter_base + nseg, sizeof(int32_t), hipMemcpyDeviceToHost, st);
    if (e == hipSuccess) e = any_stream_bailed(iters, nseg, st, &total_iters);
    if (e != hipSuccess) {
      drop_caps();
      return fail(e, "ring layout: single-pass schedule");
    }
    tick("meta + single scheduling pass");
    if (total_iters <= 0 || (int64_t)total_iters * 64 >= ((int64_t)1 << 31) - 64) {
      single = false;
      void* ps[] = {it_ent, it_cnt, it_m};
      for (void* q : ps)
        if (q) (void)hipFree(q);
      it_ent = it_cnt = it_m = nullptr;
    }
  }
  if (!single) {
    hipLaunchKernelGGL(k_ring_schedule<false>, dim3(nseg), dim3(64), flag_bytes, st, nseg, seg, wrows, keys2, meta, JM, span,
                       z.R, z.Q, z.NC, d, cap, panel_mode() == 1 ? 0 : 4, iters, nullptr, nullptr, nullptr, nullptr, flag_rows,
                       nullptr);
    e = hipGetLastError();
    if (e == hipSuccess) e = mde_exclusive_sum_i32(tmp, tmp_bytes, iters, iter_base, nseg + 1, st);
    if (e == hipSuccess) e = hipMemcpyAsync(&total_iters, iter_base + nseg, sizeof(int32_t), hipMemcpyDeviceToHost, st);
    if (e == hipSuccess) e = any_stream_bailed(iters, nseg, st, &total_iters);
    if (e != hipSuccess) {
      drop_caps();
      return fail(e, "ring layout: counting pass");
    }
    tick("meta + counting pass");
  }
  const int64_t Hp = (int64_t)total_iters * 64;
  if (total_iters <= 0 || Hp >= ((int64_t)1 << 31) - 64) {
    drop_caps();
    release(true);
    return 0;
  }
  if (panel_mode() != 1) {
    double serial = 1.0;
    {
      const int nwg = z.NRB * z.Q, GW = 4, ngroups = (z.NC + GW - 1) / GW;
      unsigned long long* bal = nullptr;
      e = hipMalloc(&bal, (size_t)2 * nwg * sizeof(unsigned long long));
      if (e == hipSuccess) e = hipMemsetAsync(bal, 0, (size_t)2 * nwg * sizeof(unsigned long long), st);
      if (e == hipSuccess) {
        hipLaunchKernelGGL(k_ring_sweep_balance, dim3((unsigned)(((int64_t)nwg * ngroups + MDE_BLOCK - 1) / MDE_BLOCK)), dim3(MDE_BLOCK),
                           0, st, nwg, ngroups, GW, z.JB, keys2, seg, bal, bal + nwg);
        e = hipGetLastError();
      }
      std::vector<unsigned long long> hb((size_t)2 * nwg);
      if (e == hipSuccess) e = hipMemcpyAsync(hb.data(), bal, hb.size() * sizeof(unsigned long long), hipMemcpyDeviceToHost, st);
      if (e == hipSuccess) e = hipStreamSynchronize(st);
      if (bal) (void)hipFree(bal);
      if (e != hipSuccess) {
        drop_caps();
        return fail(e, "ring layout: sweep balance");
      }
      unsigned long long cmax = 0, tsum = 0;
      for (int i = 0; i < nwg; ++i) {
        cmax = std::max(cmax, hb[(size_t)i]);
        tsum += hb[(size_t)nwg + i];
      }
      if (tsum > 0) serial = (double)cmax / ((double)tsum / (double)nseg);
    }
    const double t_ring = std::max(1.0, serial / 1.15) *
                              ring_time_us((double)total_iters / (double)nseg, z.NC, z.Q, z.NRB * z.Q) +
                          (double)rp.hub_half_edges * 1.3e-5;
    if (getenv("MDE_RING_STATS"))
      fprintf(stderr, "[mde ring] sweep balance: critical path of the slowest workgroup / mean stream = %.2f\n", serial);
    const double mid_ring = plan->ring.cost_scale * (rp.permuted ? 1.3 : 1.0) * t_ring + MDE_RING_FIXED_US +
                            (rp.hub_half_edges > 0 ? 4.0 : 0.0);
    const bool mid_bad = mid_regime(plan, d) && mid_ring > 0.85 * (csr_time_us(plan, d) + MDE_CSR_FIXED_US);
    if ((double)Hp > 4.0 * (double)H_ring || t_ring > 0.9 * csr_time_us(plan, d) || mid_bad) {
      drop_caps();
      release(true);
      return 0;
    }
  }
  e = hipSuccess;
  if (!single) {
    e = hipMalloc(&it_ent, (size_t)total_iters * 64 * sizeof(int32_t));
    if (e == hipSuccess) e = hipMalloc(&it_cnt, (size_t)total_iters * sizeof(int32_t));
    if (e == hipSuccess) e = hipMalloc(&it_m, (size_t)total_iters * sizeof(int32_t));
  }
  if (e == hipSuccess) e = hipMalloc(&packed, (size_t)Hp * sizeof(uint32_t));
  if (e == hipSuccess) e = hipMalloc(&peid, (size_t)Hp * sizeof(int32_t));
  if (e == hipSuccess) e = hipMalloc(&hdr, (size_t)total_iters * MDE_RING_HW * sizeof(uint32_t));
  const size_t partial_floats = (size_t)z.Q * (size_t)nloc * (size_t)d;
  if (e == hipSuccess && z.Q > 1) e = hipMalloc(&partial, sizeof(float) * (partial_floats + 2 * (size_t)z.NRB));
  if (e == hipSuccess && z.Q > 1) e = hipMemsetAsync(partial + partial_floats, 0, sizeof(float) * 2 * (size_t)z.NRB, st);
  if (e != hipSuccess) {
    drop_caps();
    return fail(e, "ring layout: output allocations");
  }
  tick("output allocations");
  if (!single) {
    hipLaunchKernelGGL(k_ring_schedule<true>, dim3(nseg), dim3(64), flag_bytes, st, nseg, seg, wrows, keys2, meta, JM, span, z.R,
                       z.Q, z.NC, d, cap, 0, nullptr, iter_base, it_ent, it_cnt, it_m, flag_rows, nullptr);
    e = hipGetLastError();
  }
  if (e == hipSuccess) {
    hipLaunchKernelGGL(k_ring_pack, dim3(mde_grid((int64_t)total_iters * 64, MDE_BLOCK, 8192)), dim3(MDE_BLOCK), 0, st,
                       (int64_t)total_iters, nseg, iter_base, single ? cap_base : nullptr, it_ent, it_cnt, it_m, keys2, vals2, hrow,
                       plan->nbr, plan->eid, z.R, z.Q, z.C, z.S, z.ring_off, z.JB, d, (int)plan->row_lo, place, rp.permuted ? 1 : 0,
                       packed, peid, hdr);
    e = hipGetLastError();
  }
  if (e == hipSuccess) e = hipStreamSynchronize(st);
  drop_caps();
  if (e != hipSuccess) return fail(e, "ring layout: fill / pack");
  hipLaunchKernelGGL(k_ring_block_class, dim3((unsigned)((total_iters / 4 + MDE_BLOCK - 1) / MDE_BLOCK)), dim3(MDE_BLOCK), 0, st,
                     (int64_t)(total_iters / 4), hdr);
  RB(hipGetLastError());
  RB(hipStreamSynchronize(st));
  if (getenv("MDE_RING_STATS")) {
    unsigned long long* dstat = reinterpret_cast<unsigned long long*>(iters);
    unsigned long long hstat[3] = {0, 0, 0};
    RB(hipMemsetAsync(dstat, 0, sizeof(hstat), st));
    hipLaunchKernelGGL(k_ring_stats, dim3(256), dim3(MDE_BLOCK), 0, st, (int64_t)total_iters, hdr, dstat);
    RB(hipMemcpyAsync(hstat, dstat, sizeof(hstat), hipMemcpyDeviceToHost, st));
    RB(hipStreamSynchronize(st));
    {
      std::vector<int32_t> hb((size_t)nseg + 1);
      RB(hipMemcpy(hb.data(), iter_base, hb.size() * sizeof(int32_t), hipMemcpyDeviceToHost));
      int mx = 0, mn = 1 << 30, wg_mx = 0;
      for (int i = 0; i < nseg; ++i) {
        mx = std::max(mx, hb[i + 1] - hb[i]);
        mn = std::min(mn, hb[i + 1] - hb[i]);
      }
      for (int g = 0; g + MDE_RING_NCW <= nseg; g += MDE_RING_NCW) wg_mx = std::max(wg_mx, hb[g + MDE_RING_NCW] - hb[g]);
      fprintf(stderr, "[mde ring] iterations per consumer wave: min %d mean %.1f max %d; per workgroup: mean %.1f max %d\n", mn,
              (double)total_iters / nseg, mx, (double)total_iters * MDE_RING_NCW / nseg, wg_mx);
    }
    {
      std::vector<uint32_t> hh((size_t)total_iters * MDE_RING_HW);
      RB(hipMemcpy(hh.data(), hdr, hh.size() * sizeof(uint32_t), hipMemcpyDeviceToHost));
      long long bad = 0;
      int worst = 0;
      for (int64_t it = 0; it + 1 < total_iters; it += 2) {
        const int gap = (int)hh[it * MDE_RING_HW + 1] - (int)hh[it * MDE_RING_HW];
        if (gap > span || hh[(it + 1) * MDE_RING_HW] < hh[it * MDE_RING_HW]) {
          if (bad < 8)
            fprintf(stderr, "[mde ring] pair at iteration %lld: m %u need %u | next m %u need %u\n", (long long)it, hh[it * MDE_RING_HW],
                    hh[it * MDE_RING_HW + 1], hh[(it + 1) * MDE_RING_HW], hh[(it + 1) * MDE_RING_HW + 1]);
          ++bad;
        }
        worst = std::max(worst, gap);
      }
      fprintf(stderr, "[mde ring] hand-shake contract: %lld of %d pairs exceed the window (worst gap %d chunks)\n", bad, total_iters / 2, worst);
      {
        std::vector<int32_t> hb2((size_t)nseg + 1);
        RB(hipMemcpy(hb2.data(), iter_base, hb2.size() * sizeof(int32_t), hipMemcpyDeviceToHost));
        std::vector<int> sp;
        for (int g0 = 0; g0 + MDE_RING_NCW <= nseg; g0 += MDE_RING_NCW) {
          int len = 1 << 30;
          for (int w = 0; w < MDE_RING_NCW; ++w) len = std::min(len, hb2[g0 + w + 1] - hb2[g0 + w]);
          if (len < 16) continue;
          for (int k = 0; k < len; k += 2) {
            int lo = 1 << 30, hi2 = 0;
            for (int w = 0; w < MDE_RING_NCW; ++w) {
              const int nit_w = hb2[g0 + w + 1] - hb2[g0 + w];
              const int64_t it = hb2[g0 + w] + (((int64_t)k * nit_w / len) & ~(int64_t)1);
              const int m = (int)hh[it * MDE_RING_HW];
              lo = std::min(lo, m);
              hi2 = std::max(hi2, m);
            }
            sp.push_back(hi2 - lo);
          }
        }
        if (!sp.empty()) {
          std::sort(sp.begin(), sp.end());
          double mean = 0;
          for (int v : sp) mean += v;
          fprintf(stderr, "[mde ring] spread of a workgroup's consumer waves along the column sweep (chunks): mean %.2f median %d p90 %d max %d\n",
                  mean / sp.size(), sp[sp.size() / 2], sp[sp.size() * 9 / 10], sp.back());
        }
      }
    }
    fprintf(stderr, "[mde ring] d=%d R=%d NRB=%d Q=%d chunks=%d x %d cols, window %d, cap %d, placement %d: %d iterations for %lld half-edges "
            "(%.1f%% padding), %.1f%% with padding lanes; loss terms: %.1f%% of the iterations add all, %.2f%% test per lane\n",
            d, z.R, z.NRB, z.Q, z.NC, z.C, span, cap, place, total_iters, (long long)H_ring,
            100.0 * ((double)Hp - (double)H_ring) / (double)H_ring, 100.0 * hstat[0] / total_iters, 100.0 * hstat[1] / total_iters,
            100.0 * hstat[2] / total_iters);
  }
#undef RB
  tick("fill pass, pack, classes");
  release(false);
  tick("scratch release");
  mde_ring_layout& L = plan->ring;
  ring_free(L);
  L.d = d;
  L.rows_per_block = z.R;
  L.n_row_blocks = z.NRB;
  L.col_groups = z.Q;
  L.chunk_cols = z.C;
  L.n_chunks = z.NC;
  L.ring_off = z.ring_off;
  L.slots = z.S;
  L.n_iters = total_iters;
  L.H = Hp;
  L.packed = packed;
  L.eid = peid;
  L.hdr = hdr;
  L.wave_iter = iter_base;
  L.partial = partial;
  L.slot_row = slot_row;
  L.count_all = rp.permuted ? 1 : 0;
  L.n_hub_rows = (int)rp.hub_rows.size();
  L.n_hub_segs = (int)(rp.hub_seg.size() / 4);
  L.hub_half_edges = rp.hub_half_edges;
  L.hub_rows = hub_rows;
  L.hub_seg = hub_seg;
  L.hub_first = hub_first;
  L.hub_partial = hub_partial;
  return 1;
}

extern "C" int mde_plan_layout(mde_plan* plan, int32_t d, void* stream) {
  if (!plan || d <= 0) return MDE_E_INVALID;
  if (plan->ring.packed && plan->ring.d == d) return 1;
  RingSizes z;
  if (!choose_sizes(plan, d, &z)) return 0;
  if (plan->ring.rejected_d == d && panel_mode() != 1) return 0;
  const int rc = build_ring(plan, d, mde_stream(stream));
  if (rc == 0) plan->ring.rejected_d = d;
  return rc;
}

__global__ __launch_bounds__(MDE_BLOCK) void k_expand_ring(int64_t H, const int32_t* __restrict__ eid,
                                                           const float* __restrict__ in,
                                                           float* __restrict__ out) {
  for (int64_t q = (int64_t)blockIdx.x * MDE_BLOCK + threadIdx.x; q < H;
       q += (int64_t)gridDim.x * MDE_BLOCK)
    out[q] = eid[q] >= 0 ? in[eid[q]] : 0.0f;
}

extern "C" int64_t mde_plan_layout_half_edges(const mde_plan* plan, int32_t layout) {
  if (!plan) return 0;
  return (layout == 1 && plan->ring.packed) ? plan->ring.H + MDE_RING_CB_VALUES : plan->H;
}

#define MDE_CB_EMPTY 0xFFFFFFFFu

__global__ __launch_bounds__(MDE_BLOCK) void k_codebook_scan(int64_t p, const float* __restrict__ in,
                                                             unsigned int* __restrict__ table,
                                                             int* __restrict__ overflow) {
  __shared__ unsigned int stb[MDE_RING_CB_VALUES];
  if (threadIdx.x < MDE_RING_CB_VALUES) stb[threadIdx.x] = MDE_CB_EMPTY;
  __syncthreads();
  unsigned int last0 = MDE_CB_EMPTY, last1 = MDE_CB_EMPTY;
  const int64_t stride = (int64_t)gridDim.x * MDE_BLOCK;
  constexpr int U = 4;
  for (int64_t i0 = (int64_t)blockIdx.x * MDE_BLOCK + threadIdx.x; i0 < p; i0 += U * stride) {
    unsigned int vv[U];
    bool in_range[U];
#pragma unroll
    for (int k = 0; k < U; ++k) {
      const int64_t i = i0 + k * stride;
      in_range[k] = i < p;
      vv[k] = in_range[k] ? __float_as_uint(in[i]) : 0u;
    }
#pragma unroll
    for (int k = 0; k < U; ++k) {
      const unsigned int v = vv[k];
      if (!in_range[k]) continue;
      if (v == MDE_CB_EMPTY) {
        *overflow = 1;
        return;
      }
      if (v == last0 || v == last1) continue;
      last1 = last0;
      last0 = v;
      bool placed = false, mine = false;
      for (int s = 0; s < MDE_RING_CB_VALUES && !placed; ++s) {
        const unsigned int old = atomicCAS(&stb[s], MDE_CB_EMPTY, v);
        mine = (old == MDE_CB_EMPTY);
        placed = mine || old == v;
      }
      if (placed && !mine) continue;
      placed = false;
      for (int s = 1; s < MDE_RING_CB_VALUES && !placed; ++s) {
        unsigned int cur = __hip_atomic_load(&table[s], __ATOMIC_RELAXED, __HIP_MEMORY_SCOPE_AGENT);
        if (cur == MDE_CB_EMPTY) cur = atomicCAS(&table[s], MDE_CB_EMPTY, v);
        placed = (cur == MDE_CB_EMPTY || cur == v);
      }
      if (!placed) {
        *overflow = 1;
        return;
      }
    }
  }
}

__global__ __launch_bounds__(MDE_BLOCK) void k_codebook_pack(int64_t H, const uint32_t* __restrict__ packed,
                                                             const int32_t* __restrict__ eid,
                                                             const float* __restrict__ in,
                                                             const unsigned int* __restrict__ table,
                                                             uint32_t* __restrict__ out) {
  unsigned int tb[MDE_RING_CB_VALUES];
#pragma unroll
  for (int s = 0; s < MDE_RING_CB_VALUES; ++s) tb[s] = table[s];
  for (int64_t q = (int64_t)blockIdx.x * MDE_BLOCK + threadIdx.x; q < H;
       q += (int64_t)gridDim.x * MDE_BLOCK) {
    uint32_t w = packed[q];
    if (eid[q] >= 0) {
      const unsigned int v = __float_as_uint(in[eid[q]]);
      uint32_t idx = 0;
#pragma unroll
      for (int s = 1; s < MDE_RING_CB_VALUES; ++s) idx = (tb[s] == v) ? (uint32_t)s : idx;
      w |= idx;
    }
    out[q] = w;
  }
}

extern "C" int mde_plan_expand_codebook(const mde_plan* plan, const float* in_edge, float* out_half,
                                        int32_t* n_values_host, void* stream) {
  if (!plan || !in_edge || !out_half || !n_values_host) return MDE_E_INVALID;
  *n_values_host = 0;
  const mde_ring_layout& L = plan->ring;
  if (!L.packed || (L.d != 2 && L.d != 3) || L.H == 0 || plan->p == 0) return MDE_OK;
  const int max_values = L.d == 2 ? 7 : 3;
  const char* e = getenv("MDE_CODEBOOK");
  if (e && atoi(e) == 0) return MDE_OK;
  hipStream_t st = mde_stream(stream);
  unsigned int* table = reinterpret_cast<unsigned int*>(out_half) + L.H;
  int* overflow = reinterpret_cast<int*>(plan->partials + MDE_MAX_PARTIALS + 1);
  hipError_t err = hipMemsetAsync(overflow, 0, sizeof(int), st);
  if (err == hipSuccess) err = hipMemsetAsync(table, 0xFF, MDE_RING_CB_VALUES * sizeof(unsigned int), st);
  unsigned int host_tb[MDE_RING_CB_VALUES];
  int host_overflow = 0;
  if (err == hipSuccess) {
    hipLaunchKernelGGL(k_codebook_scan, dim3(mde_grid(plan->p, MDE_BLOCK, 2048)), dim3(MDE_BLOCK), 0, st, plan->p,
                       in_edge, table, overflow);
    err = hipGetLastError();
  }
  if (err == hipSuccess) err = hipMemcpyAsync(host_tb, table, sizeof(host_tb), hipMemcpyDeviceToHost, st);
  if (err == hipSuccess) err = hipMemcpyAsync(&host_overflow, overflow, sizeof(int), hipMemcpyDeviceToHost, st);
  if (err == hipSuccess) err = hipStreamSynchronize(st);
  if (err != hipSuccess) return mde_hip_fail(err, "parameter codebook scan", __FILE__, __LINE__);
  if (host_overflow) return MDE_OK;
  int nv = 0;
  unsigned int vals[MDE_RING_CB_VALUES];
  vals[0] = 0u;
  for (int s = 1; s < MDE_RING_CB_VALUES; ++s)
    if (host_tb[s] != MDE_CB_EMPTY) vals[1 + nv++] = host_tb[s];
  if (nv == 0 || nv > max_values) return MDE_OK;
  for (int s = 1; s <= nv; ++s) {
    float fv;
    memcpy(&fv, &vals[s], sizeof(float));
    if (!std::isfinite(fv) || std::fabs(fv) > 1.0e6f) return MDE_OK;
  }
  for (int a = 2; a <= nv; ++a)
    for (int b = a; b > 1 && vals[b - 1] > vals[b]; --b) {
      const unsigned int t = vals[b];
      vals[b] = vals[b - 1];
      vals[b - 1] = t;
    }
  for (int s = nv + 1; s < MDE_RING_CB_VALUES; ++s) vals[s] = MDE_CB_EMPTY;
  MDE_HIP(hipMemcpyAsync(table, vals, sizeof(vals), hipMemcpyHostToDevice, st));
  hipLaunchKernelGGL(k_codebook_pack, dim3(mde_grid(L.H, MDE_BLOCK, 4096)), dim3(MDE_BLOCK), 0, st, L.H, L.packed,
                     L.eid, in_edge, table, reinterpret_cast<uint32_t*>(out_half));
  MDE_LAUNCH_CHECK();
  MDE_HIP(hipStreamSynchronize(st));
  *n_values_host = nv;
  return MDE_OK;
}

#define MDE_BX_SLOTS 1024
__device__ __forceinline__ uint32_t bx_hash(uint32_t v) {
  v ^= v >> 16;
  v *= 0x7feb352du;
  v ^= v >> 15;
  v *= 0x846ca68bu;
  v ^= v >> 16;
  return v & (MDE_BX_SLOTS - 1);
}
__device__ __forceinline__ int bx_insert(unsigned int* tb, uint32_t v) {
  uint32_t h = bx_hash(v);
  for (int probe = 0; probe < MDE_BX_SLOTS; ++probe) {
    const unsigned int old = atomicCAS(&tb[h], MDE_CB_EMPTY, v);
    if (old == MDE_CB_EMPTY) return 1;
    if (old == v) return 0;
    h = (h + 1) & (MDE_BX_SLOTS - 1);
  }
  return -1;
}
__global__ __launch_bounds__(MDE_BLOCK) void k_bytes_scan(int64_t p, const float* __restrict__ in,
                                                          unsigned int* __restrict__ table, int* __restrict__ state) {
  __shared__ unsigned int stb[MDE_BX_SLOTS];
  __shared__ int s_count;
  for (int i = threadIdx.x; i < MDE_BX_SLOTS; i += MDE_BLOCK) stb[i] = MDE_CB_EMPTY;
  if (threadIdx.x == 0) s_count = 0;
  __syncthreads();
  unsigned int last0 = MDE_CB_EMPTY, last1 = MDE_CB_EMPTY;
  const int64_t stride = (int64_t)gridDim.x * MDE_BLOCK;
  for (int64_t i = (int64_t)blockIdx.x * MDE_BLOCK + threadIdx.x; i < p; i += stride) {
    if (__hip_atomic_load(&state[1], __ATOMIC_RELAXED, __HIP_MEMORY_SCOPE_AGENT)) return;
    const unsigned int v = __float_as_uint(in[i]);
    if (v == last0 || v == last1) continue;
    last1 = last0;
    last0 = v;
    if (v == MDE_CB_EMPTY) {
      state[1] = 1;
      return;
    }
    const int fresh = bx_insert(stb, v);
    if (fresh == 0) continue;
    if (fresh < 0 || atomicAdd(&s_count, 1) >= MDE_RING_BX_VALUES - 1) {
      state[1] = 1;
      return;
    }
    const int g = bx_insert(table, v);
    if (g < 0 || (g == 1 && atomicAdd(&state[0], 1) >= MDE_RING_BX_VALUES - 1)) {
      state[1] = 1;
      return;
    }
  }
}

__global__ __launch_bounds__(MDE_BLOCK) void k_bytes_pack(int64_t H, const int32_t* __restrict__ eid,
                                                          const float* __restrict__ in,
                                                          const unsigned int* __restrict__ table, int nv,
                                                          uint8_t* __restrict__ out) {
  __shared__ unsigned int tb[MDE_RING_BX_VALUES];
  for (int i = threadIdx.x; i < MDE_RING_BX_VALUES; i += MDE_BLOCK) tb[i] = table[i];
  __syncthreads();
  for (int64_t q = (int64_t)blockIdx.x * MDE_BLOCK + threadIdx.x; q < H; q += (int64_t)gridDim.x * MDE_BLOCK) {
    uint32_t idx = 0;
    if (eid[q] >= 0) {
      const unsigned int v = __float_as_uint(in[eid[q]]);
      int lo = 1, hi = nv;
      while (lo < hi) {
        const int mid = (lo + hi) >> 1;
        if (tb[mid] < v) lo = mid + 1; else hi = mid;
      }
      idx = (uint32_t)lo;
    }
    out[q] = (uint8_t)idx;
  }
}

extern "C" int mde_plan_expand_bytes(const mde_plan* plan, const float* in_edge, float* out_half,
                                     int32_t* n_values_host, void* stream) {
  if (!plan || !in_edge || !out_half || !n_values_host) return MDE_E_INVALID;
  *n_values_host = 0;
  const mde_ring_layout& L = plan->ring;
  if (!L.packed || (L.d != 2 && L.d != 3) || L.H < 4 * MDE_RING_BX_VALUES || plan->p == 0) return MDE_OK;
  if (MDE_RING_LDS_BYTES - (L.ring_off + L.slots * ring_chunk_bytes(L.d)) < 4 * MDE_RING_BX_VALUES) return MDE_OK;
  const char* e = getenv("MDE_BYTE_STREAM");
  if (e && atoi(e) == 0) return MDE_OK;
  hipStream_t st = mde_stream(stream);
  unsigned int* dtable = nullptr;
  int* dstate = nullptr;
  MDE_HIP(hipMalloc(&dtable, MDE_BX_SLOTS * sizeof(unsigned int) + 2 * sizeof(int)));
  dstate = reinterpret_cast<int*>(dtable + MDE_BX_SLOTS);
  hipError_t err = hipMemsetAsync(dtable, 0xFF, MDE_BX_SLOTS * sizeof(unsigned int), st);
  if (err == hipSuccess) err = hipMemsetAsync(dstate, 0, 2 * sizeof(int), st);
  std::vector<unsigned int> host_tb(MDE_BX_SLOTS);
  int host_state[2] = {0, 0};
  if (err == hipSuccess) {
    hipLaunchKernelGGL(k_bytes_scan, dim3(mde_grid(plan->p, MDE_BLOCK, 2048)), dim3(MDE_BLOCK), 0, st, plan->p, in_edge, dtable,
                       dstate);
    err = hipGetLastError();
  }
  if (err == hipSuccess) err = hipMemcpyAsync(host_tb.data(), dtable, MDE_BX_SLOTS * sizeof(unsigned int), hipMemcpyDeviceToHost, st);
  if (err == hipSuccess) err = hipMemcpyAsync(host_state, dstate, sizeof(host_state), hipMemcpyDeviceToHost, st);
  if (err == hipSuccess) err = hipStreamSynchronize(st);
  if (err != hipSuccess) {
    (void)hipFree(dtable);
    return mde_hip_fail(err, "byte-index stream: value scan", __FILE__, __LINE__);
  }
  std::vector<unsigned int> vals;
  if (!host_state[1])
    for (unsigned int v : host_tb)
      if (v != MDE_CB_EMPTY) vals.push_back(v);
  bool ok = !host_state[1] && !vals.empty() && (int)vals.size() <= MDE_RING_BX_VALUES - 1;
  for (size_t i = 0; ok && i < vals.size(); ++i) {
    float fv;
    memcpy(&fv, &vals[i], sizeof(float));
    if (!std::isfinite(fv) || std::fabs(fv) > 1.0e6f) ok = false;
  }
  if (!ok) {
    (void)hipFree(dtable);
    return MDE_OK;
  }
  std::sort(vals.begin(), vals.end());
  const int nv = (int)vals.size();
  std::vector<unsigned int> tb(MDE_RING_BX_VALUES, 0u);
  for (int i = 0; i < nv; ++i) tb[1 + i] = vals[i];
  unsigned int* table = reinterpret_cast<unsigned int*>(out_half) + L.H / 4;
  err = hipMemcpyAsync(table, tb.data(), MDE_RING_BX_VALUES * sizeof(unsigned int), hipMemcpyHostToDevice, st);
  if (err == hipSuccess) {
    hipLaunchKernelGGL(k_bytes_pack, dim3(mde_grid(L.H, MDE_BLOCK, 4096)), dim3(MDE_BLOCK), 0, st, L.H, L.eid, in_edge, table, nv,
                       reinterpret_cast<uint8_t*>(out_half));
    err = hipGetLastError();
  }
  if (err == hipSuccess) err = hipStreamSynchronize(st);
  (void)hipFree(dtable);
  if (err != hipSuccess) return mde_hip_fail(err, "byte-index stream: pack", __FILE__, __LINE__);
  *n_values_host = nv;
  return MDE_OK;
}

extern "C" int mde_plan_loss_double(const mde_plan* plan, double* dst, void* stream) {
  if (!plan || !dst) return MDE_E_INVALID;
  MDE_HIP(hipMemcpyAsync(dst, plan->partials + MDE_PARTIALS_LOSS_D, sizeof(double), hipMemcpyDeviceToDevice, mde_stream(stream)));
  return MDE_OK;
}

extern "C" int mde_plan_ring_info(const mde_plan* plan, int64_t* info) {
  if (!plan || !info) return MDE_E_INVALID;
  const mde_ring_layout& L = plan->ring;
  for (int i = 0; i < 16; ++i) info[i] = 0;
  if (!L.packed) return MDE_OK;
  info[0] = 1;
  info[1] = L.d;
  info[2] = L.rows_per_block;
  info[3] = L.n_row_blocks;
  info[4] = L.col_groups;
  info[5] = L.n_chunks;
  info[6] = L.slots;
  info[7] = L.n_iters;
  info[8] = plan->H - L.hub_half_edges;
  info[9] = L.H;
  info[10] = L.slot_row ? 1 : 0;
  info[11] = L.n_hub_rows;
  info[12] = L.hub_half_edges;
  info[13] = L.n_hub_segs;
  return MDE_OK;
}

__global__ __launch_bounds__(MDE_BLOCK) void k_ring_pair_check(int64_t npairs, const uint32_t* __restrict__ packed, int d, int R,
                                                               unsigned long long* __restrict__ out) {
  const int lane = threadIdx.x & 63;
  const int64_t nw = ((int64_t)gridDim.x * MDE_BLOCK) >> 6;
  const uint32_t mask = d == 2 ? 0xfff8u : 0xfffcu, dummy = (uint32_t)R * 4u * (uint32_t)d;
  unsigned long long split = 0, shared = 0, pairs = 0;
  for (int64_t pr = ((int64_t)blockIdx.x * MDE_BLOCK + threadIdx.x) >> 6; pr < npairs; pr += nw) {
    const int64_t it = 2 * pr;
    const size_t base = ((size_t)(it >> 2) * 64 + (size_t)lane) * 4 + (size_t)(it & 3);
    const uint32_t ra = packed[base] & mask, rb = packed[base + 1] & mask;
    int found = -1;
    for (int k = 0; k < 64; ++k)
      if ((uint32_t)__builtin_amdgcn_readlane((int)ra, k) == rb) found = k;
    const bool real = rb < dummy;
    split += __popcll(__ballot(real && found >= 0 && found != lane));
    shared += __popcll(__ballot(real && found >= 0));
    ++pairs;
  }
  if (lane == 0) {
    atomicAdd(&out[0], split);
    atomicAdd(&out[1], shared);
    atomicAdd(&out[2], pairs);
  }
}

extern "C" int mde_plan_ring_check(const mde_plan* plan, int64_t* out_host, void* stream) {
  if (!plan || !out_host) return MDE_E_INVALID;
  const mde_ring_layout& L = plan->ring;
  for (int i = 0; i < 3; ++i) out_host[i] = 0;
  if (!L.packed || L.n_iters == 0) return MDE_OK;
  hipStream_t st = mde_stream(stream);
  unsigned long long* dout = nullptr;
  hipError_t e = hipMalloc(&dout, 3 * sizeof(unsigned long long));
  if (e == hipSuccess) e = hipMemsetAsync(dout, 0, 3 * sizeof(unsigned long long), st);
  if (e == hipSuccess) {
    hipLaunchKernelGGL(k_ring_pair_check, dim3(mde_grid(L.n_iters / 2 * 64, MDE_BLOCK, 4096)), dim3(MDE_BLOCK), 0, st,
                       L.n_iters / 2, L.packed, L.d, L.rows_per_block, dout);
    e = hipGetLastError();
  }
  unsigned long long h[3] = {0, 0, 0};
  if (e == hipSuccess) e = hipMemcpyAsync(h, dout, sizeof(h), hipMemcpyDeviceToHost, st);
  if (e == hipSuccess) e = hipStreamSynchronize(st);
  if (dout) (void)hipFree(dout);
  if (e != hipSuccess) {
    mde_set_error("mde_plan_ring_check: %s", hipGetErrorString(e));
    return MDE_E_HIP;
  }
  for (int i = 0; i < 3; ++i) out_host[i] = (int64_t)h[i];
  return MDE_OK;
}

extern "C" int mde_plan_expand_layout(const mde_plan* plan, int32_t layout, const float* in_edge,
                                      float* out_half, void* stream) {
  if (!plan || !in_edge || !out_half) return MDE_E_INVALID;
  if (layout == 0) return mde_plan_expand(plan, in_edge, out_half, stream);
  if (layout != 1 || !plan->ring.eid) {
    mde_set_error("mde_plan_expand_layout: the LDS-ring layout has not been built");
    return MDE_E_INVALID;
  }
  if (plan->ring.H == 0) return MDE_OK;
  hipLaunchKernelGGL(k_expand_ring, dim3(mde_grid(plan->ring.H, MDE_BLOCK, 4096)), dim3(MDE_BLOCK), 0,
                     mde_stream(stream), plan->ring.H, plan->ring.eid, in_edge, out_half);
  MDE_LAUNCH_CHECK();
  return MDE_OK;
}

template <int D>
__global__ __launch_bounds__(MDE_BLOCK) void k_hub_rows(const int32_t* __restrict__ hub_rows, const int32_t* __restrict__ hub_seg,
                                                        int row_lo, const int32_t* __restrict__ nbr,
                                                        const int32_t* __restrict__ eid, const float* __restrict__ e0,
                                                        const float* __restrict__ e1, int e0_scalar, int e1_scalar,
                                                        const float* __restrict__ X, FnRuntime fn, float inv_p, int count_all,
                                                        double* __restrict__ partial) {
  __shared__ double smem[8];
  const int sgi = blockIdx.x;
  const int hi = hub_seg[4 * sgi], beg = hub_seg[4 * sgi + 1], end = hub_seg[4 * sgi + 2];
  const int64_t v = (int64_t)row_lo + hub_rows[hi];
  float xv[D];
#pragma unroll
  for (int c = 0; c < D; ++c) xv[c] = X[v * D + c];
  const float e0s = e0_scalar ? e0[0] : 0.0f;
  const float e1s = (e1 && e1_scalar) ? e1[0] : 0.0f;
  double acc[D], loss = 0.0;
#pragma unroll
  for (int c = 0; c < D; ++c) acc[c] = 0.0;
  for (int h = beg + (int)threadIdx.x; h < end; h += MDE_BLOCK) {
    const int u = nbr[h], k = eid[h];
    const float p0 = e0_scalar ? e0s : e0[k];
    const float p1 = (e1 && !e1_scalar) ? e1[k] : e1s;
    float diff[D], ss = 0.0f;
#pragma unroll
    for (int c = 0; c < D; ++c) {
      diff[c] = xv[c] - X[(size_t)u * D + c];
      ss = fmaf(diff[c], diff[c], ss);
    }
    float f, gd;
    fn.eval(ss, p0, p1, f, gd);
    const float g = mde_fix_g(gd * inv_p);
    if (count_all || v < (int64_t)u) loss += (double)f;
#pragma unroll
    for (int c = 0; c < D; ++c) acc[c] += (double)(g * diff[c]);
  }
#pragma unroll
  for (int c = 0; c < D; ++c) {
    const double t = mde_block_sum(acc[c], smem);
    if (threadIdx.x == 0) partial[(size_t)sgi * 8 + c] = t;
  }
  const double tl = mde_block_sum(loss, smem);
  if (threadIdx.x == 0) partial[(size_t)sgi * 8 + 4] = tl;
}

template <int D>
__global__ __launch_bounds__(64) void k_hub_finish(int n_hub, int n_seg, const int32_t* __restrict__ hub_rows,
                                                   const int32_t* __restrict__ hub_first,
                                                   const double* __restrict__ partial, int row_lo, float grad_scale,
                                                   float* __restrict__ grad, double loss_scale, float* __restrict__ loss_out,
                                                   double* __restrict__ loss_d) {
  const int lane = threadIdx.x;
  if ((int)blockIdx.x < n_hub) {
    if (!grad) return;
    const int i = blockIdx.x;
    double a[D];
#pragma unroll
    for (int c = 0; c < D; ++c) a[c] = 0.0;
    for (int sg = hub_first[i] + lane; sg < hub_first[i + 1]; sg += 64) {
#pragma unroll
      for (int c = 0; c < D; ++c) a[c] += partial[(size_t)sg * 8 + c];
    }
#pragma unroll
    for (int c = 0; c < D; ++c) a[c] = mde_wave_sum(a[c]);
    if (lane == 0) {
      const int64_t v = (int64_t)row_lo + hub_rows[i];
#pragma unroll
      for (int c = 0; c < D; ++c) grad[v * D + c] = (float)a[c] * grad_scale;
    }
    return;
  }
  double t = 0.0;
  for (int sg = lane; sg < n_seg; sg += 64) t += partial[(size_t)sg * 8 + 4];
  const double tot = mde_wave_sum(t);
  if (lane == 0) {
    *loss_d += tot * loss_scale;
    *loss_out = (float)*loss_d;
  }
}

template <int D>
static int hub_launch_d(const mde_plan* plan, const float* X, const mde_func* f, const float* e0, const float* e1, int e0_scalar,
                        int e1_scalar, float grad_scale, float* grad, float inv_p, hipStream_t st, float* loss_out, double loss_scale) {
  const mde_ring_layout& L = plan->ring;
  FnRuntime fn{ring_func_args(f)};
  hipLaunchKernelGGL(k_hub_rows<D>, dim3(L.n_hub_segs), dim3(MDE_BLOCK), 0, st, L.hub_rows, L.hub_seg, (int)plan->row_lo, plan->nbr,
                     plan->eid, e0, e1, e0_scalar, e1_scalar, X, fn, inv_p, L.count_all, L.hub_partial);
  MDE_LAUNCH_CHECK();
  const int nb = L.n_hub_rows + 1;
  hipLaunchKernelGGL(k_hub_finish<D>, dim3(nb), dim3(64), 0, st, L.n_hub_rows, L.n_hub_segs, L.hub_rows, L.hub_first,
                     L.hub_partial, (int)plan->row_lo, grad_scale, grad, (L.count_all ? 1.0 : 2.0) * loss_scale, loss_out,
                     plan->partials + MDE_PARTIALS_LOSS_D);
  MDE_LAUNCH_CHECK();
  return MDE_OK;
}

static int hub_launch(const mde_plan* plan, const float* X, int d, const mde_func* f, float grad_scale, float* grad, float inv_p,
                      hipStream_t st, float* loss_out, double loss_scale) {
  const float *e0 = f->e0, *e1 = f->e1;
  int e0_scalar = 0, e1_scalar = 0;
  if (f->a0_scalar == 1) {
    e0 = f->a0;
    e0_scalar = 1;
  }
  if (f->a1 && f->a1_scalar) {
    e1 = f->a1;
    e1_scalar = 1;
  }
  if (!e0 || (f->a1 && !e1)) {
    mde_set_error("this plan's LDS-ring layout peels %d hub rows off to the CSR hub kernel: mde_func.e0 (and e1 for two-parameter "
                  "functions) must point at the per-edge arrays in the caller's edge order", plan->ring.n_hub_rows);
    return MDE_E_INVALID;
  }
  switch (d) {
    case 1: return hub_launch_d<1>(plan, X, f, e0, e1, e0_scalar, e1_scalar, grad_scale, grad, inv_p, st, loss_out, loss_scale);
    case 2: return hub_launch_d<2>(plan, X, f, e0, e1, e0_scalar, e1_scalar, grad_scale, grad, inv_p, st, loss_out, loss_scale);
    case 3: return hub_launch_d<3>(plan, X, f, e0, e1, e0_scalar, e1_scalar, grad_scale, grad, inv_p, st, loss_out, loss_scale);
    default: return hub_launch_d<4>(plan, X, f, e0, e1, e0_scalar, e1_scalar, grad_scale, grad, inv_p, st, loss_out, loss_scale);
  }
}

int mde_ring_try(mde_plan* plan, const float* X, int d, const mde_func* f, float grad_scale,
                 float* grad, float inv_p, hipStream_t st, int* nblocks, float* loss_out,
                 double loss_scale) {
  if (!plan->ring.packed || plan->ring.d != d) return 0;
  const RingArgs A{plan, X, d, f->a0, f->a1, f->a0_scalar, f->a1_scalar, grad, inv_p, grad_scale, st,
                   loss_out, loss_scale};
  int rc = 0;
  if (f->kind_neg != MDE_F_NONE)
    rc = mde_ring_launch_pushpull(A, f, nblocks);
  else if (f->kind == MDE_F_LOG1P)
    rc = mde_ring_launch_log1p(A, f, nblocks);
  else if (f->kind == MDE_F_L_QUADRATIC || f->kind == MDE_F_L_WEIGHTED_QUADRATIC || f->kind == MDE_F_L_ABSOLUTE ||
           f->kind == MDE_F_L_HUBER)
    rc = mde_ring_launch_loss(A, f, nblocks);
  else if (f->kind == MDE_F_L_CUBIC || f->kind == MDE_F_L_POWER || f->kind == MDE_F_L_LOGISTIC ||
           f->kind == MDE_F_L_FRACTIONAL || f->kind == MDE_F_L_SOFT_FRACTIONAL)
    rc = mde_ring_launch_loss2(A, f, nblocks);
  else if (f->kind == MDE_F_LOGISTIC || f->kind == MDE_F_SIGMOID || f->kind == MDE_F_HINGE || f->kind == MDE_F_POWER ||
           f->kind == MDE_F_INVPOWER || f->kind == MDE_F_LOGRATIO)
    rc = mde_ring_launch_penalty2(A, f, nblocks);
  else
    rc = mde_ring_launch_penalty(A, f, nblocks);
  if (rc == 0) rc = mde_ring_launch_runtime(A, f, nblocks);
  if (rc == 1 && plan->ring.n_hub_rows > 0) {
    const int hrc = hub_launch(plan, X, d, f, grad_scale, grad, inv_p, st, loss_out, loss_scale);
    if (hrc != MDE_OK) return hrc;
  }
  return rc;
}
```

### pymde_amd/csrc/mde_ring_kernel.h

```cpp
#pragma once
#include <algorithm>
#include <cstring>
#include <type_traits>
#include <vector>

#include "mde_ring.h"
#define COMMA ,

#define MDE_RING23(FN, LIN)                                    \
  do {                                                         \
    FN fn{a};                                                  \
    int rc;                                                    \
    if (A.d == 2)                                              \
      rc = launch_ring<2, FN, LIN>(A, fn, nblocks);            \
    else                                                       \
      rc = launch_ring<3, FN, LIN>(A, fn, nblocks);            \
    return rc == MDE_OK ? 1 : rc;                              \
  } while (0)

typedef uint32_t ring_u4 __attribute__((ext_vector_type(4)));
typedef float ring_f4 __attribute__((ext_vector_type(4)));

template <int D>
struct RingVec;
template <>
struct RingVec<1> {
  typedef float T;
};
template <>
struct RingVec<2> {
  typedef float2 T;
};
template <>
struct RingVec<4> {
  typedef float4 T;
};
template <int D>
__device__ __forceinline__ void ring_ld(const char* p, float (&v)[D]) {
  if constexpr (D == 3) {
    const float* q = reinterpret_cast<const float*>(p);
    v[0] = q[0];
    v[1] = q[1];
    v[2] = q[2];
  } else {
    const typename RingVec<D>::T t = *reinterpret_cast<const typename RingVec<D>::T*>(p);
    const float* q = reinterpret_cast<const float*>(&t);
#pragma unroll
    for (int c = 0; c < D; ++c) v[c] = q[c];
  }
}
template <int D>
__device__ __forceinline__ void ring_ld_operand(char* lds_base, uint32_t addr, float (&v)[D]) {
  typedef __attribute__((address_space(3))) const volatile float* lds_vf;
  typedef float ring_f2v __attribute__((ext_vector_type(2)));
  typedef float ring_f4v __attribute__((ext_vector_type(4)));
  if constexpr (D == 2) {
    const ring_f2v t = *(__attribute__((address_space(3))) const volatile ring_f2v*)(lds_base + addr);
    v[0] = t.x;
    v[1] = t.y;
  } else if constexpr (D == 4) {
    const ring_f4v t = *(__attribute__((address_space(3))) const volatile ring_f4v*)(lds_base + addr);
    v[0] = t.x;
    v[1] = t.y;
    v[2] = t.z;
    v[3] = t.w;
  } else {
    lds_vf q = (lds_vf)(lds_base + addr);
#pragma unroll
    for (int c = 0; c < D; ++c) v[c] = q[c];
  }
}
template <int D>
__device__ __forceinline__ void ring_st(char* p, const float (&v)[D]) {
  if constexpr (D == 3) {
    float* q = reinterpret_cast<float*>(p);
    q[0] = v[0];
    q[1] = v[1];
    q[2] = v[2];
  } else {
    typename RingVec<D>::T t;
    float* q = reinterpret_cast<float*>(&t);
#pragma unroll
    for (int c = 0; c < D; ++c) q[c] = v[c];
    *reinterpret_cast<typename RingVec<D>::T*>(p) = t;
  }
}

__device__ __forceinline__ void ring_ctrl_store(uint32_t addr, int v) {
  asm volatile("ds_write_b32 %0, %1" ::"v"(addr), "v"(v) : "memory");
}
__device__ __forceinline__ void ring_ctrl_store_counted(char* lds_base, uint32_t addr, int v) {
  typedef __attribute__((address_space(3))) volatile int* lds_vint;
  *(lds_vint)(lds_base + addr) = v;
}
__device__ __forceinline__ int ring_ctrl_load(uint32_t addr) {
  int v;
  asm volatile("ds_read_b32 %0, %1\n\ts_waitcnt lgkmcnt(0)" : "=&v"(v) : "v"(addr) : "memory");
  return v;
}

#if MDE_RING_ABLATE
static __device__ unsigned long long g_ring_probe[8][1024];
static __device__ int g_ring_diag[64][8];
static __device__ int g_ring_ndiag;
#ifndef MDE_RING_SPINMAX
#define MDE_RING_SPINMAX 100000
#endif
#define RING_CLK() __builtin_readcyclecounter()
#endif
#ifndef MDE_RING_FWORDS
#define MDE_RING_FWORDS 0
#endif
#ifdef MDE_RING_EVAL2
constexpr bool defined_MDE_RING_EVAL2 = true;
#else
constexpr bool defined_MDE_RING_EVAL2 = false;
#endif
template <int D, class Fn, bool HAS_GRAD, int PS, bool LIN>
__global__ __launch_bounds__(MDE_RING_BS) void k_fused_ring(
    int nloc, int row_lo, int n, int R, int Q, int NC, int ring_off, int S, const int32_t* __restrict__ wave_iter,
    const uint32_t* __restrict__ hdr, const uint32_t* __restrict__ packed, const uint32_t* __restrict__ bidx,
    const int32_t* __restrict__ slot_row, const float* __restrict__ a0, const float* __restrict__ a1, int a0_scalar, int a1_scalar,
    const float* __restrict__ X,
    float* __restrict__ grad, float* __restrict__ partial, double* __restrict__ loss_partials, Fn fn,
    float fix_value, float grad_scale, float* __restrict__ loss_out, double loss_scale, int fold, int dbg_arg) {
#if MDE_RING_ABLATE
#ifndef MDE_RING_ABLATE_MASK
#define MDE_RING_ABLATE_MASK (~0)
#endif
  const int dbg = dbg_arg & (MDE_RING_ABLATE_MASK);
#else
  constexpr int dbg = 0;
#endif
  constexpr int BS = MDE_RING_BS, NCW = MDE_RING_NCW, NPROD = MDE_RING_NPROD;
  constexpr bool CB = PS == 1, BX = PS == 2;
  constexpr int GR_OFF = ring_gr_off(D), CTRL_PROG = MDE_RING_CTRL_PROG(D), CTRL_F = MDE_RING_CTRL_F(D), CTRL_CB = MDE_RING_CTRL_CB(D);
  constexpr int C = ring_chunk_cols(D), CBYTES = ring_chunk_bytes(D), PIECES = CBYTES / 1024;
  static_assert(GR_OFF + (ring_row_cap(D) + 32) * 4 * D <= 65536 + GR_OFF && GR_OFF < 65536 && CTRL_CB + 32 < 65536,
                "region bases must fit the 16-bit offset of the LDS instructions");
  static_assert(NPROD <= 8 && NCW <= 16, "control-word layout");
  __shared__ __attribute__((aligned(16))) char L[MDE_RING_LDS_BYTES];
  float* XR = reinterpret_cast<float*>(L);
  float* GR = reinterpret_cast<float*>(L + GR_OFF);
  const int tid = threadIdx.x, lane = tid & 63;
  const int wave = __builtin_amdgcn_readfirstlane(tid >> 6);
  const int rb = blockIdx.x / Q, qg = blockIdx.x % Q;
  const int j_lo = (int)(((int64_t)qg * NC + Q - 1) / Q), j_hi = (int)(((int64_t)(qg + 1) * NC + Q - 1) / Q);
  const int r0 = rb * R;
  const int nr = min(R, nloc - r0);
  const uint32_t dummy_row = (uint32_t)R * 4u * (uint32_t)D;
  const float a0s = (a0_scalar && PS == 0) ? a0[0] : 1.0f;
  const uint32_t tab_off = (uint32_t)ring_off + (uint32_t)S * (uint32_t)CBYTES;
  const float a1s = (a1 && a1_scalar) ? a1[0] : 0.0f;
  const bool a1_arr = a1 && !a1_scalar;
  {
    float4* z = reinterpret_cast<float4*>(L + GR_OFF);
    const int nz = ((R + 32) * 4 * D + 15) / 16;
    for (int i = tid; i < nz; i += BS) z[i] = make_float4(0.f, 0.f, 0.f, 0.f);
    const float* Xrow = X + (size_t)(row_lo + r0) * D;
    if (slot_row) {
      const int32_t* sr = slot_row + (size_t)rb * R;
      for (int sl = tid; sl < R; sl += BS) {
        const int r = sr[sl];
        float xv[D];
#pragma unroll
        for (int c = 0; c < D; ++c) xv[c] = r >= 0 ? X[(size_t)(row_lo + r) * D + c] : 0.0f;
#pragma unroll
        for (int c = 0; c < D; ++c) XR[sl * D + c] = xv[c];
      }
    } else if ((reinterpret_cast<uintptr_t>(Xrow) & 15) == 0) {
      const ring_f4* X4 = reinterpret_cast<const ring_f4*>(Xrow);
      ring_f4* XR4 = reinterpret_cast<ring_f4*>(L);
      const int n4 = (nr * D) >> 2;
      for (int i0 = 0; i0 < n4; i0 += 8 * BS) {
        ring_f4 t[8];
#pragma unroll
        for (int k = 0; k < 8; ++k) t[k] = X4[min(i0 + tid + k * BS, max(n4 - 1, 0))];
#pragma unroll
        for (int k = 0; k < 8; ++k)
          if (i0 + tid + k * BS < n4) XR4[i0 + tid + k * BS] = t[k];
      }
      for (int i = (n4 << 2) + tid; i < nr * D; i += BS) XR[i] = Xrow[i];
    } else {
      for (int i = tid; i < nr * D; i += BS) XR[i] = Xrow[i];
    }
    if (tid < 32 * D) XR[R * D + tid] = 0.0f;
    int* prog = reinterpret_cast<int*>(L + CTRL_PROG);
    int* F = reinterpret_cast<int*>(L + CTRL_F);
    if (tid < 16) prog[tid] = (tid < NCW) ? j_lo : MDE_RING_DONE;
#if MDE_RING_FWORDS
    static_assert(NPROD == 4 && MDE_RING_UNIT == 1, "MDE_RING_FWORDS: four producers, one chunk per step");
    if (tid >= 16 && tid < 16 + NPROD) F[tid - 16] = (j_lo + (tid - 16) < j_hi) ? j_lo + (tid - 16) : MDE_RING_DONE;
#else
    if (tid == 16) F[0] = j_lo;
#endif
    if (CB && tid >= 32 && tid < 32 + MDE_RING_CB_VALUES)
      reinterpret_cast<float*>(L + CTRL_CB)[tid - 32] = a0[tid - 32] * Fn::kParamScale;
    if (BX && tid >= 64 && tid < 64 + MDE_RING_BX_VALUES)
      reinterpret_cast<float*>(L + tab_off)[tid - 64] = a0[tid - 64] * Fn::kParamScale;
  }
  __syncthreads();
  float loss = 0.0f, loss2 = 0.0f;

  if (wave >= NCW) {
    if (MDE_RING_PRODPRIO) __builtin_amdgcn_s_setprio(MDE_RING_PRODPRIO);
    const int p = wave - NCW;
    const char* Xb = reinterpret_cast<const char*>(X);
    const size_t nbytes = (size_t)n * D * 4;
    const size_t last16 = nbytes - 16;
    constexpr int DEPTH = MDE_RING_DEPTH, UNIT = MDE_RING_UNIT;
    ring_f4 buf[DEPTH][UNIT * PIECES];
    auto ld16 = [&](ring_f4& dst, const ring_f4* src) __attribute__((always_inline)) {
#if MDE_RING_ASMLOAD
      asm volatile("global_load_dwordx4 %0, %1, off" : "=v"(dst) : "v"(src) : "memory");
#else
      dst = *src;
#endif
    };
    auto fetch = [&](int k, int j0u) __attribute__((always_inline)) {
#pragma unroll
      for (int c = 0; c < UNIT; ++c) {
        const int j = j0u + c;
        if (j < NC - 1) {
          const ring_f4* src = reinterpret_cast<const ring_f4*>(Xb + (size_t)j * CBYTES + (size_t)lane * 16);
#pragma unroll
          for (int i = 0; i < PIECES; ++i) ld16(buf[k][c * PIECES + i], src + i * 64);
        } else {
          const size_t off0 = (size_t)min(j, NC - 1) * CBYTES + (size_t)lane * 16;
#pragma unroll
          for (int i = 0; i < PIECES; ++i) {
            const size_t off = off0 + (size_t)i * 1024;
            ld16(buf[k][c * PIECES + i], reinterpret_cast<const ring_f4*>(Xb + (off < last16 ? off : last16)));
          }
        }
      }
    };
    auto wait_buf = [&](int k) __attribute__((always_inline)) {
#if MDE_RING_ASMLOAD
      static_assert(UNIT * PIECES == 4 || UNIT * PIECES == 2 || UNIT * PIECES == 3 || UNIT * PIECES == 8 || UNIT * PIECES == 6, "operand list of the wait");
      constexpr int NEWER = (DEPTH - 1) * UNIT * PIECES;
      if constexpr (UNIT * PIECES == 4)
        asm volatile("s_waitcnt vmcnt(%4)" : "+v"(buf[k][0]), "+v"(buf[k][1]), "+v"(buf[k][2]), "+v"(buf[k][3]) : "n"(NEWER) : "memory");
      else if constexpr (UNIT * PIECES == 3)
        asm volatile("s_waitcnt vmcnt(%3)" : "+v"(buf[k][0]), "+v"(buf[k][1]), "+v"(buf[k][2]) : "n"(NEWER) : "memory");
      else if constexpr (UNIT * PIECES == 2)
        asm volatile("s_waitcnt vmcnt(%2)" : "+v"(buf[k][0]), "+v"(buf[k][1]) : "n"(NEWER) : "memory");
      else if constexpr (UNIT * PIECES == 6)
        asm volatile("s_waitcnt vmcnt(%6)" : "+v"(buf[k][0]), "+v"(buf[k][1]), "+v"(buf[k][2]), "+v"(buf[k][3]), "+v"(buf[k][4]),
                     "+v"(buf[k][5]) : "n"(NEWER) : "memory");
      else
        asm volatile("s_waitcnt vmcnt(%8)" : "+v"(buf[k][0]), "+v"(buf[k][1]), "+v"(buf[k][2]), "+v"(buf[k][3]), "+v"(buf[k][4]),
                     "+v"(buf[k][5]), "+v"(buf[k][6]), "+v"(buf[k][7]) : "n"(NEWER) : "memory");
#endif
    };
    ring_f4 tail_v = {0.0f, 0.0f, 0.0f, 0.0f};
    int tail_rel = -1;
    if ((nbytes & 15) != 0 && j_hi == NC) {
      const size_t off_str = nbytes & ~(size_t)15;
      const size_t rel = off_str - (size_t)(NC - 1) * CBYTES;
      if (off_str >= (size_t)(NC - 1) * CBYTES && lane == (int)((rel & 1023) >> 4)) {
        tail_rel = (int)rel;
        const float* tp = reinterpret_cast<const float*>(Xb + off_str);
        const int nt = (int)((nbytes - off_str) >> 2);
        tail_v[0] = tp[0];
        if (nt > 1) tail_v[1] = tp[1];
        if (nt > 2) tail_v[2] = tp[2];
      }
    }
    int minprog = j_lo, landed = j_lo;
    const uint32_t poll_addr = lane < 16 ? CTRL_PROG + 4u * (uint32_t)lane : (uint32_t)CTRL_F;
#if MDE_RING_ABLATE
    unsigned long long pr_t0 = RING_CLK(), pr_blocked = 0, pr_polls = 0, pr_chain = 0, pr_data = 0, pr_write = 0;
#endif
#pragma unroll
    for (int k = 0; k < DEPTH; ++k) fetch(k, j_lo + UNIT * (p + k * NPROD));
    int slot = (j_lo + UNIT * p) % S;
    for (int j0 = j_lo + UNIT * p; j0 < j_hi && !(dbg & 128); j0 += UNIT * DEPTH * NPROD) {
#pragma unroll
      for (int k = 0; k < DEPTH; ++k) {
        const int j = j0 + k * UNIT * NPROD;
        if (j < j_hi) {
          const int jl = min(j + UNIT, j_hi) - 1;
          while (jl - S >= minprog && !(dbg & 8)) {
#if MDE_RING_ABLATE
            const unsigned long long tb0 = RING_CLK();
            ++pr_polls;
#endif
            int v = ring_ctrl_load(poll_addr);
            asm volatile("s_nop 1\n\tv_min_i32_dpp %0, %0, %0 row_shr:1 row_mask:0xf bank_mask:0xf\n\t"
                         "s_nop 1\n\tv_min_i32_dpp %0, %0, %0 row_shr:2 row_mask:0xf bank_mask:0xf\n\t"
                         "s_nop 1\n\tv_min_i32_dpp %0, %0, %0 row_shr:4 row_mask:0xf bank_mask:0xf\n\ts_nop 1"
                         : "+v"(v));
            if (NCW > 8) asm volatile("v_min_i32_dpp %0, %0, %0 row_shr:8 row_mask:0xf bank_mask:0xf\n\ts_nop 1" : "+v"(v));
            minprog = __builtin_amdgcn_readlane(v, NCW <= 8 ? 7 : 15);
            landed = __builtin_amdgcn_readlane(v, 16);
            if (jl - S >= minprog) __builtin_amdgcn_s_sleep(MDE_RING_PSLEEP);
#if MDE_RING_ABLATE
            pr_blocked += RING_CLK() - tb0;
            if (pr_polls > MDE_RING_SPINMAX) {
              if (lane == 0) {
                const int kk = atomicAdd(&g_ring_ndiag, 1);
                if (kk < 64) {
                  int* r = g_ring_diag[kk];
                  r[0] = 2; r[1] = blockIdx.x; r[2] = p; r[3] = j; r[4] = minprog; r[5] = S; r[6] = j_lo; r[7] = j_hi;
                }
              }
              pr_polls = 0;
              minprog = jl;
            }
#endif
          }
#if MDE_RING_ABLATE
          unsigned long long td0 = 0;
          if (dbg & 512) {
            td0 = RING_CLK();
            __builtin_amdgcn_s_waitcnt(0x0F70 | (((DEPTH - 1) * UNIT * PIECES) & 15) | ((((DEPTH - 1) * UNIT * PIECES) >> 4) << 14));
            pr_data += RING_CLK() - td0;
            td0 = RING_CLK();
          }
#endif
          wait_buf(k);
#pragma unroll
          for (int c = 0; c < UNIT; ++c) {
            const int jc = j + c;
            if (UNIT > 1 && jc >= j_hi) break;
            int sc = slot + c;
            if (UNIT > 1 && sc >= S) sc -= S;
            char* dst = L + (uint32_t)__builtin_amdgcn_readfirstlane(ring_off + sc * CBYTES) + lane * 16;
#pragma unroll
            for (int i = 0; i < PIECES; ++i) *reinterpret_cast<ring_f4*>(dst + i * 1024) = buf[k][c * PIECES + i];
            if (jc == NC - 1 && tail_rel >= 0) *reinterpret_cast<ring_f4*>(dst - lane * 16 + tail_rel) = tail_v;
          }
          asm volatile("" ::: "memory");
#if MDE_RING_FWORDS
          (void)landed;
          ring_ctrl_store_counted(L, CTRL_F + 4u * (uint32_t)p, (j + NPROD < j_hi) ? j + NPROD : MDE_RING_DONE);
#else
          while (landed != j && !(dbg & 8)) {
            landed = __builtin_amdgcn_readfirstlane(ring_ctrl_load((uint32_t)CTRL_F + 0u * (uint32_t)lane));
#if MDE_RING_ABLATE
            ++pr_chain;
#endif
            if (landed != j) __builtin_amdgcn_s_sleep(0);
          }
          ring_ctrl_store_counted(L, CTRL_F, jl + 1);
#endif
#if MDE_RING_ABLATE
          if (dbg & 512) pr_write += RING_CLK() - td0;
#endif
          fetch(k, j + UNIT * DEPTH * NPROD);
          slot += UNIT * NPROD;
          while (slot >= S) slot -= S;
        }
      }
    }
#if MDE_RING_ABLATE
    if ((dbg & 512) && lane == 0 && blockIdx.x < 1024) {
      atomicAdd(&g_ring_probe[3][blockIdx.x], RING_CLK() - pr_t0);
      atomicAdd(&g_ring_probe[4][blockIdx.x], pr_blocked);
      atomicAdd(&g_ring_probe[6][blockIdx.x], pr_polls);
      atomicAdd(&g_ring_probe[5][blockIdx.x], pr_data);
      atomicAdd(&g_ring_probe[7][blockIdx.x], pr_write);
    }
#endif
  } else {
    if (MDE_RING_CONSPRIO) __builtin_amdgcn_s_setprio(MDE_RING_CONSPRIO);
    const int ib = __builtin_amdgcn_readfirstlane(wave_iter[blockIdx.x * NCW + wave]);
    const int NB = (__builtin_amdgcn_readfirstlane(wave_iter[blockIdx.x * NCW + wave + 1]) - ib) >> 2;
    if (NB > 0 && !(dbg & 64)) {
      const bool a0_arr = !a0_scalar && PS == 0;
      const uint32_t* bp = BX ? bidx + (size_t)(ib >> 2) * 64 + lane : nullptr;
      const ring_u4* sp = reinterpret_cast<const ring_u4*>(packed) + (size_t)(ib >> 2) * 64 + lane;
      const ring_f4* ap = reinterpret_cast<const ring_f4*>(a0_arr ? a0 : reinterpret_cast<const float*>(packed)) +
                          (size_t)(ib >> 2) * 64 + lane;
      const int lastb = NB - 1;
      constexpr int PFB = MDE_RING_PFB;
      ring_u4 pq[PFB] = {};
      uint32_t hv[PFB] = {};
      ring_f4 wq[PFB] = {};
      uint32_t bq[PFB] = {};
      const uint32_t* hvp = hdr + (size_t)ib * MDE_RING_HW + (lane & 15);
      auto load_block = [&](int u, int b) __attribute__((always_inline)) {
        const int bc = min(b, lastb);
#if defined(MDE_RING_STREAM_L2)
        pq[u] = sp[(size_t)(bc & 7) * 64];
#elif defined(MDE_RING_STREAM_NT)
        pq[u] = __builtin_nontemporal_load(&sp[(size_t)bc * 64]);
#else
        pq[u] = sp[(size_t)bc * 64];
#endif
        hv[u] = hvp[(size_t)bc * 16];
        if (PS == 0) wq[u] = ap[(size_t)bc * 64];
        if (BX) bq[u] = bp[(size_t)bc * 64];
      };
#if MDE_RING_ABLATE
      unsigned long long cs_t0 = RING_CLK(), cs_poll = 0, cs_trips = 0;
#endif

      struct Pre {
        float xr[D], xc[D], p0;
#ifdef MDE_RING_KEEPROW
        uint32_t row;
#endif
      };
#ifdef MDE_RING_PROBE_ROWLIN
      auto row_of = [&](uint32_t w) __attribute__((always_inline)) { return ((w & 0x7f00u) | ((uint32_t)lane << 3)) & 0xfff8u; };
#else
      auto row_of = [&](uint32_t w) __attribute__((always_inline)) { return D == 2 ? (w & 0xfff8u) : (w & 0xfffcu); };
#endif
#ifdef MDE_RING_PROBE_COLLIN
      auto col_of = [&](uint32_t w) __attribute__((always_inline)) {
        return (((w >> 13) & 0x3f000u) | ((uint32_t)lane << 3)) & 0x3fff8u;
      };
#else
      auto col_of = [&](uint32_t w) __attribute__((always_inline)) {
        return D == 2 ? ((w >> 13) & 0x3fff8u) : ((w >> 14) & 0x3fffcu);
      };
#endif
      auto issue_x = [&](uint32_t w, float p0, uint32_t bi4) __attribute__((always_inline)) {
        Pre r;
        if constexpr (BX)
          r.p0 = *reinterpret_cast<const float*>(L + tab_off + bi4);
        else
          r.p0 = CB ? *reinterpret_cast<const float*>(L + CTRL_CB + ((w & (D == 2 ? 7u : 3u)) << 2)) : p0 * Fn::kParamScale;
#ifdef MDE_RING_KEEPROW
        r.row = row_of(w);
        ring_ld_operand<D>(L, r.row, r.xr);
#else
        ring_ld_operand<D>(L, row_of(w), r.xr);
#endif
        ring_ld_operand<D>(L, col_of(w), r.xc);
        return r;
      };
      auto bx4 = [&](uint32_t bw, int q) __attribute__((always_inline)) { return BX ? ((bw >> (8 * q)) & 0xffu) << 2 : 0u; };
      auto counts_here = [&](uint32_t w, uint32_t hm) __attribute__((always_inline)) {
        const uint32_t off = col_of(w) - (uint32_t)ring_off;
        const uint32_t slot = off / (uint32_t)CBYTES, cidx = (off - slot * (uint32_t)CBYTES) / (4u * (uint32_t)D);
        const uint32_t ms = hm % (uint32_t)S;
        const uint32_t j = hm + (slot >= ms ? slot - ms : slot + (uint32_t)S - ms);
        const uint32_t u = j * (uint32_t)C + cidx;
        const uint32_t vv = (uint32_t)(row_lo + r0) + row_of(w) / (4u * (uint32_t)D);
        return vv < u;
      };
      auto finish = [&](auto lc_tag, uint32_t w, const Pre& x, float (&acc)[D], float p1, uint32_t hm)
          __attribute__((always_inline)) {
        constexpr int LC = decltype(lc_tag)::value;
#ifdef MDE_RING_KEEPROW
        const uint32_t rowaddr = x.row;
#else
        const uint32_t rowaddr = row_of(w);
#endif
        float v[D], ss = (defined_MDE_RING_EVAL2 && Fn::kRingFused) ? 1.0e-30f : 0.0f;
#pragma unroll
        for (int c = 0; c < D; ++c) {
          v[c] = x.xr[c] - x.xc[c];
          ss = fmaf(v[c], v[c], ss);
        }
        float gd;
        if constexpr (Fn::kRingFused) {
          const float d = mde_sqrt(ss), sd = mde_sqrt(d);
          const float t = fmaf(d, sd, 1.0f);
          const float r = defined_MDE_RING_EVAL2 ? mde_rcp(sd + ss) : mde_rcp(fmaf(sd, t, 1.0e-30f));
          gd = x.p0 * r;
          if constexpr (LC != 0) {
            const float c = d * sd - (t - 1.0f);
            float wl = x.p0, gc = gd;
            if (!LIN) {
              const bool real = rowaddr < dummy_row;
              wl = real ? wl : 0.0f;
              gc = real ? gc : 0.0f;
            }
            if constexpr (LC == 2) {
              const bool here = counts_here(w, hm);
              wl = here ? wl : 0.0f;
              gc = here ? gc : 0.0f;
            }
            loss = fmaf(wl, mde_log2(t), loss);
            loss2 = fmaf(gc, sd * c, loss2);
          }
        } else {
          float f;
          fn.eval(ss, x.p0, p1, f, gd);
          if constexpr (LC != 0) {
            if (!LIN) f = (rowaddr < dummy_row) ? f : 0.0f;
            if constexpr (LC == 2) f = counts_here(w, hm) ? f : 0.0f;
            loss += f;
          }
        }
        if (!HAS_GRAD) return;
        const float g = (Fn::kFiniteG && PS != 0) ? gd : mde_fix_g_to(gd, fix_value);
#pragma unroll
        for (int c = 0; c < D; ++c) acc[c] = fmaf(v[c], g, acc[c]);
        ring_st<D>(L + GR_OFF + rowaddr, acc);
      };
      const uint32_t prog_addr = CTRL_PROG + 4u * (uint32_t)wave;
      int ready = j_lo;
      typedef __attribute__((address_space(3))) const volatile int* lds_cvint;
      const uint32_t f_addr = (uint32_t)CTRL_F + 0u * (uint32_t)lane;
#if MDE_RING_FWORDS
      typedef int ring_i4 __attribute__((ext_vector_type(4)));
      typedef __attribute__((address_space(3))) const volatile ring_i4* lds_cvint4;
      auto min4 = [](const ring_i4& v) __attribute__((always_inline)) { return min(min(v.x, v.y), min(v.z, v.w)); };
      ring_i4 fl_pre = *(lds_cvint4)(L + CTRL_F);
#else
      int fl_pre = *(lds_cvint)(L + CTRL_F);
#endif
      auto wait_pair = [&](int u, int q) __attribute__((always_inline)) {
        const int need = __builtin_amdgcn_readlane((int)hv[u], 4 * q + 1);
        if (__builtin_expect(need >= ready && !(dbg & 1), 0)) {
#if MDE_RING_FWORDS
          ready = __builtin_amdgcn_readfirstlane(min4(fl_pre));
#else
          ready = __builtin_amdgcn_readfirstlane(fl_pre);
#endif
          if (__builtin_expect(need >= ready, 0)) {
#if MDE_RING_ABLATE
            const unsigned long long tp0 = RING_CLK();
#endif
            for (;;) {
#if MDE_RING_FWORDS
              {
                ring_i4 fv;
                asm volatile("ds_read_b128 %0, %1\n\ts_waitcnt lgkmcnt(0)" : "=&v"(fv) : "v"(f_addr) : "memory");
                ready = __builtin_amdgcn_readfirstlane(min4(fv));
              }
#else
              ready = __builtin_amdgcn_readfirstlane(ring_ctrl_load(f_addr));
#endif
#if MDE_RING_ABLATE
              ++cs_trips;
              if (cs_trips > MDE_RING_SPINMAX) {
                if (lane == 0) {
                  const int k = atomicAdd(&g_ring_ndiag, 1);
                  if (k < 64) {
                    int* r = g_ring_diag[k];
                    r[0] = 1; r[1] = blockIdx.x; r[2] = wave; r[3] = need; r[4] = ready; r[5] = 0; r[6] = u * 4 + q; r[7] = NB;
                  }
                }
                cs_trips = 0;
                ready = need + 1;
                break;
              }
#endif
              if (need < ready) break;
              __builtin_amdgcn_s_sleep(MDE_RING_CSLEEP);
            }
#if MDE_RING_ABLATE
            cs_poll += RING_CLK() - tp0;
#endif
          }
          asm volatile("" ::: "memory");
        }
      };
#if MDE_RING_FWORDS
      auto prefetch_landed = [&]() __attribute__((always_inline)) { fl_pre = *(lds_cvint4)(L + CTRL_F); };
#else
      auto prefetch_landed = [&]() __attribute__((always_inline)) { fl_pre = *(lds_cvint)(L + CTRL_F); };
#endif
      const uint32_t rel_addr[2] = {lane == 0 ? 4u * (uint32_t)wave : 128u + 4u * (uint32_t)(lane & 31),
                                    lane == 8 ? 4u * (uint32_t)wave : 128u + 4u * (uint32_t)(lane & 31)};
      auto release_to = [&](int u, int q) __attribute__((always_inline)) {
        ring_ctrl_store_counted(L, CTRL_PROG + rel_addr[q >> 1], (int)hv[u]);
      };

      Pre xa, xb;
      float acc[D], accb[D];
      auto block_body = [&](auto lc_tag, int u, int b) __attribute__((always_inline)) {
#pragma unroll
        for (int h = 0; h < 2; ++h) {
          const int q = 2 * h;
          const int un = h == 0 ? u : (u + 1) % PFB, qn = (q + 2) & 3;
          wait_pair(un, qn);
          const Pre xna = issue_x(pq[un][qn], (a0_scalar || PS != 0) ? a0s : wq[un][qn], bx4(bq[un], qn));
          const Pre xnb = issue_x(pq[un][qn + 1], (a0_scalar || PS != 0) ? a0s : wq[un][qn + 1], bx4(bq[un], qn + 1));
          release_to((u + 1) % PFB, q);
          prefetch_landed();
          const float p1a = a1_arr ? a1[((size_t)((ib >> 2) + b) * 64 + lane) * 4 + q] : a1s;
          const float p1b = a1_arr ? a1[((size_t)((ib >> 2) + b) * 64 + lane) * 4 + q + 1] : a1s;
          const bool lc2 = decltype(lc_tag)::value == 2;
          const uint32_t hma = lc2 ? (uint32_t)__builtin_amdgcn_readlane((int)hv[u], 4 * q) : 0u;
          const uint32_t hmb = lc2 ? (uint32_t)__builtin_amdgcn_readlane((int)hv[u], 4 * q + 4) : 0u;
          finish(lc_tag, pq[u][q], xa, acc, p1a, hma);
          if (HAS_GRAD) {
            const bool same = row_of(pq[u][q + 1]) == row_of(pq[u][q]);
#pragma unroll
            for (int c = 0; c < D; ++c) accb[c] = same ? acc[c] : accb[c];
          }
          finish(lc_tag, pq[u][q + 1], xb, accb, p1b, hmb);
          if (HAS_GRAD) {
            ring_ld<D>(L + GR_OFF + row_of(pq[un][qn]), acc);
            ring_ld<D>(L + GR_OFF + row_of(pq[un][qn + 1]), accb);
          }
          xa = xna;
          xb = xnb;
        }
      };
#pragma unroll
      for (int u = 0; u < PFB; ++u) load_block(u, u);
      release_to(0, 0);
      wait_pair(0, 0);
      xa = issue_x(pq[0][0], (a0_scalar || PS != 0) ? a0s : wq[0][0], bx4(bq[0], 0));
      xb = issue_x(pq[0][1], (a0_scalar || PS != 0) ? a0s : wq[0][1], bx4(bq[0], 1));
      release_to(0, 2);
      prefetch_landed();
      if (HAS_GRAD) {
        ring_ld<D>(L + GR_OFF + row_of(pq[0][0]), acc);
        ring_ld<D>(L + GR_OFF + row_of(pq[0][1]), accb);
      }
      for (int base = 0; base < NB; base += PFB) {
#pragma unroll
        for (int u = 0; u < PFB; ++u) {
          const int b = base + u;
          if (b < NB) {
            const int bcls = __builtin_amdgcn_readlane((int)hv[u], 3) & 3;
            if (bcls == 0)
              block_body(std::integral_constant<int, 0>(), u, b);
            else if (bcls == 1)
              block_body(std::integral_constant<int, 1>(), u, b);
            else
              block_body(std::integral_constant<int, 2>(), u, b);
          }
          load_block(u, b + PFB);
        }
      }
#if MDE_RING_ABLATE
      if ((dbg & 512) && lane == 0 && blockIdx.x < 1024) {
        atomicAdd(&g_ring_probe[0][blockIdx.x], RING_CLK() - cs_t0);
        atomicAdd(&g_ring_probe[1][blockIdx.x], cs_poll);
        atomicAdd(&g_ring_probe[2][blockIdx.x], cs_trips);
      }
#endif
    }
    if constexpr (Fn::kRingFused) loss = fmaf(loss, 0.6931471805599453f, loss2) * (1.0f / Fn::kParamScale);
    ring_ctrl_store_counted(L, CTRL_PROG + 4u * (uint32_t)wave, MDE_RING_DONE);
    __builtin_amdgcn_s_waitcnt(0x0F70);
  }
  __syncthreads();
  if (HAS_GRAD && slot_row) {
    const int32_t* sr = slot_row + (size_t)rb * R;
    if (fold) {
      unsigned int* sync = reinterpret_cast<unsigned int*>(partial + (size_t)Q * nloc * D) + 2 * rb;
      int* tk = reinterpret_cast<int*>(L + 512);
      if (tid == 0) *tk = (int)__hip_atomic_fetch_add(&sync[0], 1u, __ATOMIC_RELAXED, __HIP_MEMORY_SCOPE_AGENT);
      __syncthreads();
      const bool second = *tk != 0;
      float* mine = partial + (size_t)qg * nloc * D;
      const float* other = partial + (size_t)(1 - qg) * nloc * D;
      if (!second) {
        for (int sl = tid; sl < R; sl += BS) {
          const int r = sr[sl];
          if (r < 0) continue;
#pragma unroll
          for (int c = 0; c < D; ++c)
            __hip_atomic_store(mine + (size_t)r * D + c, GR[sl * D + c], __ATOMIC_RELAXED, __HIP_MEMORY_SCOPE_AGENT);
        }
        __builtin_amdgcn_s_waitcnt(0x0F70);
        __syncthreads();
        if (tid == 0) __hip_atomic_store(&sync[1], 1u, __ATOMIC_RELAXED, __HIP_MEMORY_SCOPE_AGENT);
      } else {
        if (tid == 0) {
          while (__hip_atomic_load(&sync[1], __ATOMIC_RELAXED, __HIP_MEMORY_SCOPE_AGENT) == 0u) __builtin_amdgcn_s_sleep(2);
          __hip_atomic_store(&sync[1], 0u, __ATOMIC_RELAXED, __HIP_MEMORY_SCOPE_AGENT);
          __hip_atomic_store(&sync[0], 0u, __ATOMIC_RELAXED, __HIP_MEMORY_SCOPE_AGENT);
        }
        __syncthreads();
        for (int s0 = 0; s0 < R; s0 += 8 * BS) {
          int rr[8];
          float o[8][D];
#pragma unroll
          for (int k = 0; k < 8; ++k) rr[k] = s0 + tid + k * BS < R ? sr[s0 + tid + k * BS] : -1;
#pragma unroll
          for (int k = 0; k < 8; ++k)
#pragma unroll
            for (int c = 0; c < D; ++c)
              o[k][c] = __hip_atomic_load(other + (size_t)max(rr[k], 0) * D + c, __ATOMIC_RELAXED, __HIP_MEMORY_SCOPE_AGENT);
#pragma unroll
          for (int k = 0; k < 8; ++k) {
            if (rr[k] < 0) continue;
            const int sl = s0 + tid + k * BS;
#pragma unroll
            for (int c = 0; c < D; ++c) {
              const float m = GR[sl * D + c];
              grad[(size_t)(row_lo + rr[k]) * D + c] = (qg == 0 ? m + o[k][c] : o[k][c] + m) * grad_scale;
            }
          }
        }
      }
      __syncthreads();
    } else {
      float* dst = (Q == 1) ? grad + (size_t)row_lo * D : partial + (size_t)qg * nloc * D;
      const float sc = (Q == 1) ? grad_scale : 1.0f;
      for (int sl = tid; sl < R; sl += BS) {
        const int r = sr[sl];
        if (r < 0) continue;
#pragma unroll
        for (int c = 0; c < D; ++c) dst[(size_t)r * D + c] = GR[sl * D + c] * sc;
      }
    }
  } else if (HAS_GRAD && fold) {
    unsigned int* sync = reinterpret_cast<unsigned int*>(partial + (size_t)Q * nloc * D) + 2 * rb;
    int* tk = reinterpret_cast<int*>(L + 512);
    if (tid == 0) *tk = (int)__hip_atomic_fetch_add(&sync[0], 1u, __ATOMIC_RELAXED, __HIP_MEMORY_SCOPE_AGENT);
    __syncthreads();
    const bool second = *tk != 0;
    float* mine = partial + ((size_t)qg * nloc + r0) * D;
    const float* other = partial + ((size_t)(1 - qg) * nloc + r0) * D;
    float* grow = grad + (size_t)(row_lo + r0) * D;
    static_assert(GR_OFF % 16 == 0, "16-byte accumulator pieces");
    const bool vec = ((reinterpret_cast<uintptr_t>(mine) | reinterpret_cast<uintptr_t>(other) | reinterpret_cast<uintptr_t>(grow)) & 15) == 0;
    const int n4 = vec ? (nr * D) >> 2 : 0, n1 = nr * D;
    const ring_f4* GR4 = reinterpret_cast<const ring_f4*>(GR);
    if (!second) {
      for (int i = tid; i < n4; i += BS) {
        const ring_f4 v4 = GR4[i];
        asm volatile("global_store_dwordx4 %0, %1, off sc1" ::"v"(reinterpret_cast<ring_f4*>(mine) + i), "v"(v4) : "memory");
      }
      for (int i = (n4 << 2) + tid; i < n1; i += BS) __hip_atomic_store(mine + i, GR[i], __ATOMIC_RELAXED, __HIP_MEMORY_SCOPE_AGENT);
      __builtin_amdgcn_s_waitcnt(0x0F70);
      __syncthreads();
      if (tid == 0) __hip_atomic_store(&sync[1], 1u, __ATOMIC_RELAXED, __HIP_MEMORY_SCOPE_AGENT);
    } else {
      if (tid == 0) {
        while (__hip_atomic_load(&sync[1], __ATOMIC_RELAXED, __HIP_MEMORY_SCOPE_AGENT) == 0u) __builtin_amdgcn_s_sleep(2);
        __hip_atomic_store(&sync[1], 0u, __ATOMIC_RELAXED, __HIP_MEMORY_SCOPE_AGENT);
        __hip_atomic_store(&sync[0], 0u, __ATOMIC_RELAXED, __HIP_MEMORY_SCOPE_AGENT);
      }
      __syncthreads();
      const ring_f4* o4p = reinterpret_cast<const ring_f4*>(other);
      for (int i0 = 0; i0 < n4; i0 += 8 * BS) {
        ring_f4 o[8];
#pragma unroll
        for (int k = 0; k < 8; ++k)
          asm volatile("global_load_dwordx4 %0, %1, off sc1" : "=v"(o[k]) : "v"(o4p + min(i0 + tid + k * BS, n4 - 1)) : "memory");
        asm volatile("s_waitcnt vmcnt(0)" : "+v"(o[0]), "+v"(o[1]), "+v"(o[2]), "+v"(o[3]), "+v"(o[4]), "+v"(o[5]), "+v"(o[6]), "+v"(o[7])::"memory");
#pragma unroll
        for (int k = 0; k < 8; ++k) {
          const int i = i0 + tid + k * BS;
          if (i < n4) {
            const ring_f4 m = GR4[i];
            reinterpret_cast<ring_f4*>(grow)[i] = (qg == 0 ? m + o[k] : o[k] + m) * grad_scale;
          }
        }
      }
      for (int i0 = n4 << 2; i0 < n1; i0 += 8 * BS) {
        float o[8];
#pragma unroll
        for (int k = 0; k < 8; ++k) o[k] = __hip_atomic_load(other + min(i0 + tid + k * BS, n1 - 1), __ATOMIC_RELAXED, __HIP_MEMORY_SCOPE_AGENT);
#pragma unroll
        for (int k = 0; k < 8; ++k) {
          const int i = i0 + tid + k * BS;
          if (i < n1) grow[i] = (qg == 0 ? GR[i] + o[k] : o[k] + GR[i]) * grad_scale;
        }
      }
    }
    __syncthreads();
  } else if (HAS_GRAD) {
    float* grow = (Q == 1) ? grad + (size_t)(row_lo + r0) * D : partial + ((size_t)qg * nloc + r0) * D;
    const float sc = (Q == 1) ? grad_scale : 1.0f;
    const int n4 = (reinterpret_cast<uintptr_t>(grow) & 15) == 0 ? (nr * D) >> 2 : 0;
    for (int i = tid; i < n4; i += BS) reinterpret_cast<ring_f4*>(grow)[i] = reinterpret_cast<const ring_f4*>(GR)[i] * sc;
    for (int i = (n4 << 2) + tid; i < nr * D; i += BS) grow[i] = GR[i] * sc;
  }
  double* red = reinterpret_cast<double*>(L);
  unsigned int* ticket = reinterpret_cast<unsigned int*>(loss_partials + MDE_MAX_PARTIALS);
  const double v = mde_wave_sum((double)loss);
  if (lane == 0) red[wave] = v;
  __syncthreads();
  if (tid == 0) {
    double s = 0.0;
    for (int i = 0; i < NCW; ++i) s += red[i];
    mde_st_partial(loss_partials + blockIdx.x, s);
  }
  int* last_flag = reinterpret_cast<int*>(L + 256);
  __builtin_amdgcn_s_waitcnt(0x0F70);
  __syncthreads();
  if (tid == 0) {
    const unsigned int k = __hip_atomic_fetch_add(ticket, 1u, __ATOMIC_RELAXED, __HIP_MEMORY_SCOPE_AGENT);
    *last_flag = (k == gridDim.x - 1u) ? 1 : 0;
    if (*last_flag) __hip_atomic_store(ticket, 0u, __ATOMIC_RELAXED, __HIP_MEMORY_SCOPE_AGENT);
  }
  __syncthreads();
  if (!*last_flag) return;
  double t = 0.0;
  for (int i = tid; i < (int)gridDim.x; i += BS) t += mde_ld_partial(loss_partials + i);
  t = mde_wave_sum(t);
  __syncthreads();
  if (lane == 0) red[wave] = t;
  __syncthreads();
  if (tid == 0) {
    double s = 0.0;
    for (int i = 0; i < BS / 64; ++i) s += red[i];
    *loss_out = (float)(s * loss_scale);
    loss_partials[MDE_PARTIALS_LOSS_D] = s * loss_scale;
  }
}

template <class V>
__global__ __launch_bounds__(MDE_BLOCK) void k_ring_combine(int64_t m, int Q, const V* __restrict__ partial,
                                                            float scale, V* __restrict__ out) {
  constexpr int W = sizeof(V) / sizeof(float);
  const int64_t i = (int64_t)blockIdx.x * MDE_BLOCK + threadIdx.x;
  if (i >= m) return;
  V a[8];
#pragma unroll
  for (int q = 0; q < 8; ++q)
    if (q < Q) a[q] = partial[(size_t)q * m + i];
  float s[W];
#pragma unroll
  for (int k = 0; k < W; ++k) s[k] = reinterpret_cast<const float*>(&a[0])[k];
#pragma unroll
  for (int q = 1; q < 8; ++q)
    if (q < Q) {
#pragma unroll
      for (int k = 0; k < W; ++k) s[k] += reinterpret_cast<const float*>(&a[q])[k];
    }
  for (int q = 8; q < Q; ++q) {
    const V t = partial[(size_t)q * m + i];
#pragma unroll
    for (int k = 0; k < W; ++k) s[k] += reinterpret_cast<const float*>(&t)[k];
  }
  V r;
#pragma unroll
  for (int k = 0; k < W; ++k) reinterpret_cast<float*>(&r)[k] = s[k] * scale;
  out[i] = r;
}


template <int D, class Fn, bool LIN>
static int launch_ring(const RingArgs& A, const Fn& fn, int* nblocks) {
  const mde_ring_layout& L = A.plan->ring;
  const bool cb = A.a0_scalar == 2, bx = A.a0_scalar == 3;
  if ((cb || bx) && D != 2 && D != 3) {
    mde_set_error("codebook / byte-index parameter streams exist for d = 2 and d = 3 only");
    return MDE_E_INVALID;
  }
  if (bx && MDE_RING_LDS_BYTES - (L.ring_off + L.slots * ring_chunk_bytes(D)) < 4 * MDE_RING_BX_VALUES) {
    mde_set_error("byte-index parameter stream: no room for the value table behind the ring");
    return MDE_E_INVALID;
  }
  if (reinterpret_cast<uintptr_t>(A.X) & 15) {
    mde_set_error("the LDS-ring kernel needs a 16-byte aligned embedding matrix");
    return MDE_E_INVALID;
  }
  if constexpr (LIN) {
    if (A.a0_scalar == 1) return launch_ring<D, Fn, false>(A, fn, nblocks);
  }
  auto kern = A.grad ? k_fused_ring<D, Fn, true, 0, LIN> : k_fused_ring<D, Fn, false, 0, LIN>;
  if constexpr (D == 2 || D == 3) {
    if (cb) kern = A.grad ? k_fused_ring<D, Fn, true, 1, LIN> : k_fused_ring<D, Fn, false, 1, LIN>;
    if (bx) kern = A.grad ? k_fused_ring<D, Fn, true, 2, LIN> : k_fused_ring<D, Fn, false, 2, LIN>;
  }
  const uint32_t* stream = cb ? reinterpret_cast<const uint32_t*>(A.a0) : L.packed;
  const uint32_t* bidx = bx ? reinterpret_cast<const uint32_t*>(A.a0) : nullptr;
  const float* a0 = cb ? A.a0 + L.H : (bx ? A.a0 + L.H / 4 : A.a0);
  const int Q = L.col_groups;
  *nblocks = L.n_row_blocks * Q;
  const float out_scale = A.grad_scale * A.inv_p;
  const float fix_value = A.inv_p > 0.0f ? 1.0f / A.inv_p : 1.0f;
#if MDE_RING_ABLATE
  const int dbg = getenv("MDE_RING_DBG") ? atoi(getenv("MDE_RING_DBG")) : 0;
#else
  const int dbg = 0;
#endif
  static const int fold_env = getenv("MDE_RING_FOLD") ? atoi(getenv("MDE_RING_FOLD")) : 1;
  const int fold = (Q == 2 && A.grad && fold_env) ? 1 : 0;
  hipLaunchKernelGGL(kern, dim3(L.n_row_blocks * Q), dim3(MDE_RING_BS), 0, A.st,
                     (int)(A.plan->row_hi - A.plan->row_lo), (int)A.plan->row_lo, (int)A.plan->n,
                     L.rows_per_block, Q, L.n_chunks, L.ring_off, L.slots, L.wave_iter, L.hdr, stream, bidx, L.slot_row, a0, A.a1,
                     A.a0_scalar, A.a1_scalar, A.X, A.grad, L.partial, A.plan->partials, fn, fix_value, out_scale,
                     A.loss_out, (L.count_all ? 1.0 : 2.0) * A.loss_scale, fold, dbg);
  MDE_LAUNCH_CHECK();
#if MDE_RING_ABLATE
  {
    static int dl = 0;
    if (++dl == 3) {
      int nd = 0;
      int hd[64][8];
      (void)hipStreamSynchronize(A.st);
      (void)hipMemcpyFromSymbol(&nd, HIP_SYMBOL(g_ring_ndiag), sizeof(int));
      (void)hipMemcpyFromSymbol(hd, HIP_SYMBOL(g_ring_diag), sizeof(hd));
      fprintf(stderr, "[mde ring diag] %d give-ups in the first launches\n", nd);
      for (int k = 0; k < nd && k < 24; ++k)
        fprintf(stderr, hd[k][0] == 1 ? "[mde ring diag] consumer wg %d wave %d: need %d ready %d m %d slot %d NB %d\n"
                                      : "[mde ring diag] producer wg %d p %d: j %d minprog %d infl %d oldest %d j_hi %d\n",
                hd[k][1], hd[k][2], hd[k][3], hd[k][4], hd[k][5], hd[k][6], hd[k][7]);
    }
  }
  if (dbg & 512) {
    static int launches = 0;
    if (++launches == 8) {
      std::vector<unsigned long long> h(8 * 1024);
      (void)hipStreamSynchronize(A.st);
      (void)hipMemcpyFromSymbol(h.data(), HIP_SYMBOL(g_ring_probe), sizeof(unsigned long long) * 8 * 1024);
      const int nb = std::min(1024, L.n_row_blocks * Q);
      double s[8] = {0};
      for (int k = 0; k < 8; ++k)
        for (int i = 0; i < nb; ++i) s[k] += (double)h[k * 1024 + i];
      const double L8 = 8.0 * nb;
      fprintf(stderr, "[mde ring probe] per consumer wave and launch: loop %.0f clk, in chunk polls %.0f clk (%.1f%%), %.0f poll trips | "
              "per producer wave: loop %.0f clk, blocked on a slot %.0f (%.1f%%), waiting for the chunk's loads %.0f (%.1f%%), %.0f slot polls, LDS stores + ordered publish %.0f clk\n",
              s[0] / L8 / MDE_RING_NCW, s[1] / L8 / MDE_RING_NCW, 100.0 * s[1] / s[0], s[2] / L8 / MDE_RING_NCW,
              s[3] / L8 / MDE_RING_NPROD, s[4] / L8 / MDE_RING_NPROD, 100.0 * s[4] / s[3], s[5] / L8 / MDE_RING_NPROD,
              100.0 * s[5] / s[3], s[6] / L8 / MDE_RING_NPROD, s[7] / L8 / MDE_RING_NPROD);
      std::vector<double> loop(nb), work(nb);
      for (int i = 0; i < nb; ++i) {
        loop[i] = (double)h[i] / 8.0 / MDE_RING_NCW;
        work[i] = ((double)h[i] - (double)h[1024 + i]) / 8.0 / MDE_RING_NCW;
      }
      auto quant = [&](std::vector<double> v, const char* what) {
        std::sort(v.begin(), v.end());
        double m = 0;
        for (double x : v) m += x;
        fprintf(stderr, "[mde ring probe] per workgroup, %s: min %.0f p10 %.0f median %.0f mean %.0f p90 %.0f max %.0f clk\n", what, v[0],
                v[v.size() / 10], v[v.size() / 2], m / v.size(), v[v.size() * 9 / 10], v.back());
      };
      quant(loop, "consumer loop");
      quant(work, "consumer loop minus polls");
      for (int q8 = 0; q8 < 8; ++q8) {
        double a = 0, b2 = 0;
        int c = 0;
        for (int i = q8 * nb / 8; i < (q8 + 1) * nb / 8; ++i, ++c) {
          a += loop[i];
          b2 += work[i];
        }
        fprintf(stderr, "[mde ring probe] workgroups %d..%d: loop %.0f, minus polls %.0f\n", q8 * nb / 8, (q8 + 1) * nb / 8 - 1, a / c, b2 / c);
      }
    }
  }
#endif
  if (Q > 1 && A.grad && !fold) {
    const int64_t nlocD = (A.plan->row_hi - A.plan->row_lo) * (int64_t)D;
    float* out = A.grad + (size_t)A.plan->row_lo * D;
    if (nlocD % 4 == 0 && (reinterpret_cast<uintptr_t>(out) & 15) == 0) {
      const int64_t m = nlocD / 4;
      hipLaunchKernelGGL(k_ring_combine<float4>, dim3((unsigned)((m + MDE_BLOCK - 1) / MDE_BLOCK)), dim3(MDE_BLOCK),
                         0, A.st, m, Q, reinterpret_cast<const float4*>(L.partial), out_scale,
                         reinterpret_cast<float4*>(out));
    } else {
      hipLaunchKernelGGL(k_ring_combine<float>, dim3((unsigned)((nlocD + MDE_BLOCK - 1) / MDE_BLOCK)),
                         dim3(MDE_BLOCK), 0, A.st, nlocD, Q, L.partial, out_scale, out);
    }
    MDE_LAUNCH_CHECK();
  }
  return MDE_OK;
}
```

Before: 320.7 billion edges/s/iter.

## Balance edge-ownership classes across ring workgroups via checkerboard group assignment

Changes which endpoint counts each half-edge for loss: instead of always the lower vertex id, row-block groups are paired in a checkerboard pattern so class-1 (fully counted) iterations spread evenly across workgroups. The pack kernel now precomputes a per-iteration offset, flip and mask bit in the header, and the consumer's counts_here test becomes a few integer ops on those header words instead of a modular slot-to-column reconstruction. This aims to reduce load imbalance and per-edge ALU work in mixed-class iterations. It also adds diagnostics for class shares and timestamp probes, at the cost of extra build-time work and a larger header encoding.

```diff
diff --git a/include/mde_hip.h b/include/mde_hip.h
--- a/include/mde_hip.h
+++ b/include/mde_hip.h
@@ -97,6 +97,7 @@
 int mde_plan_expand_layout(const mde_plan* plan, int32_t layout, const float* in_edge,
                            float* out_half, void* stream);
 int mde_plan_ring_info(const mde_plan* plan, int64_t* info_host);
+int mde_plan_ring_balance(const mde_plan* plan, double* out_host);
 int mde_plan_ring_check(const mde_plan* plan, int64_t* out_host, void* stream);
 int mde_plan_row_order(mde_plan* plan, int32_t mode, void* stream, double* info_host);
 int mde_plan_loss_double(const mde_plan* plan, double* dst, void* stream);
diff --git a/pymde_amd/_lib.py b/pymde_amd/_lib.py
--- a/pymde_amd/_lib.py
+++ b/pymde_amd/_lib.py
@@ -51,6 +51,7 @@
     "mde_plan_layout": (c_i32, [c_vp, c_i32, c_vp]),
     "mde_plan_layout_half_edges": (c_i64, [c_vp, c_i32]),
     "mde_plan_ring_info": (c_i32, [c_vp, ctypes.POINTER(c_i64)]),
+    "mde_plan_ring_balance": (c_i32, [c_vp, ctypes.POINTER(ctypes.c_double)]),
     "mde_plan_ring_check": (c_i32, [c_vp, ctypes.POINTER(c_i64), c_vp]),
     "mde_plan_row_order": (c_i32, [c_vp, c_i32, c_vp, ctypes.POINTER(ctypes.c_double)]),
     "mde_plan_function_hint": (c_i32, [c_vp, c_i32, c_i32]),
diff --git a/pymde_amd/average_distortion.py b/pymde_amd/average_distortion.py
--- a/pymde_amd/average_distortion.py
+++ b/pymde_amd/average_distortion.py
@@ -102,6 +102,10 @@
                  "ring_half_edges", "padded_entries", "permuted", "hub_rows", "hub_half_edges", "hub_segments")
         out = {k: int(info[i]) for i, k in enumerate(names)}
         out["built"], out["permuted"] = bool(out["built"]), bool(out["permuted"])
+        bal = (ctypes.c_double * 4)()
+        _lib.check(lib.mde_plan_ring_balance(self._handle, bal))
+        out["class1_share_min"], out["class1_share_mean"], out["class1_share_max"] = float(bal[0]), float(bal[1]), float(bal[2])
+        out["balance_group"] = int(bal[3])
         return out
 
     def ring_check(self):
diff --git a/pymde_amd/csrc/mde_plan.h b/pymde_amd/csrc/mde_plan.h
--- a/pymde_amd/csrc/mde_plan.h
+++ b/pymde_amd/csrc/mde_plan.h
@@ -18,6 +18,8 @@
   float* partial = nullptr;
   int32_t* slot_row = nullptr;
   int count_all = 0;
+  int balance_g = 0;
+  float* wg_cls1 = nullptr;
   int n_hub_rows = 0, n_hub_segs = 0;
   int64_t hub_half_edges = 0;
   int32_t* hub_rows = nullptr;
diff --git a/pymde_amd/csrc/mde_ring.hip b/pymde_amd/csrc/mde_ring.hip
--- a/pymde_amd/csrc/mde_ring.hip
+++ b/pymde_amd/csrc/mde_ring.hip
@@ -416,7 +416,7 @@
                                                          const int32_t* __restrict__ nbr,
                                                          const int32_t* __restrict__ eid, int R, int Q, int C, int S,
                                                          int ring_off, int JB, int d, int row_lo, int place, int count_all,
-                                                         uint32_t* __restrict__ packed,
+                                                         int balance_g, uint32_t* __restrict__ packed,
                                                          int32_t* __restrict__ peid, uint32_t* __restrict__ hdr) {
   __shared__ uint8_t s_taken[MDE_BLOCK / 64][64], s_free[MDE_BLOCK / 64][64];
   __shared__ uint32_t s_prow[MDE_BLOCK / 64][64];
@@ -441,12 +441,12 @@
     const int cnt = cw & 0xff;
     const bool act = valid && lane < cnt;
     uint32_t key = 0, q = 0, col = 0, rowaddr = 0, ring = 0;
-    int grow = 0, rcls = 0;
+    int grow = 0, rcls = 0, rb = 0;
     if (act) {
       const int pos = it_ent[(size_t)src * 64 + lane];
       key = keys[pos];
       q = vals[pos];
-      const int rb = (int)((key >> JB) / MDE_RING_NCW) / Q;
+      rb = (int)((key >> JB) / MDE_RING_NCW) / Q;
       grow = hrow[q];
       rowaddr = (uint32_t)(grow - rb * R) * 4u * (uint32_t)d;
       const uint32_t j = key & JM;
@@ -493,7 +493,10 @@
     const unsigned long long mvm = __ballot(moved);
     const int nmoved = __popcll(mvm);
     if (moved) l = s_free[wv][__popcll(mvm & ((1ull << lane) - 1ull))];
-    const bool counts = act && (count_all || (uint32_t)(row_lo + grow) < col);
+    const uint32_t vglob = (uint32_t)(row_lo + grow);
+    const int sv = balance_g ? rb / balance_g : 0, su = balance_g ? (int)(col / (uint32_t)R) / balance_g : 0;
+    bool counts = act && (count_all || vglob < col);
+    if (balance_g) counts = act && (sv == su ? col < vglob : ((vglob < col) != (((sv + su) & 1) != 0)));
     const int ncount = __popcll(__ballot(counts));
     const uint32_t lclass = ncount == 0 ? 0u : (ncount == cnt ? 1u : 2u);
     const uint32_t m = valid ? (uint32_t)__builtin_amdgcn_readfirstlane(it_m[src]) : 0u;
@@ -509,11 +512,34 @@
                                                      (uint32_t)ring_off + (mpad % (uint32_t)S) * cbytes);
       peid[base + (size_t)lf * 4] = -1;
     }
+    long long K = 0;
+    uint32_t Mbit = 0u, flip = 0u;
+    const long long r0b = (long long)__builtin_amdgcn_readfirstlane(rb) * R, mcol = (long long)m * C;
+    if (!balance_g) {
+      K = (mcol - row_lo - r0b) * 4 * d;
+      Mbit = 1u;
+    } else if (__ballot(act && su == sv)) {
+      K = (mcol - r0b) * 4 * d + 1;
+      Mbit = 1u;
+      flip = 1u;
+    } else {
+      int smin = act ? su : 0x7fffffff, smax = act ? su : -1;
+      for (int o = 32; o > 0; o >>= 1) {
+        smin = min(smin, __shfl_xor(smin, o));
+        smax = max(smax, __shfl_xor(smax, o));
+      }
+      const bool low_counts = __ballot(act && su == smin && counts) != 0ull;
+      const long long T = smax > smin ? ((long long)smax * balance_g * R - mcol) * 4 * d : 0;
+      flip = (smax > smin) == low_counts ? 1u : 0u;
+      K = 1 - T;
+    }
+    K = max(-(1ll << 27) + 1, min((1ll << 27) - 1, K));
+    const uint32_t a_m = (uint32_t)ring_off + (m % (uint32_t)S) * cbytes;
     if (lane == 0 && valid) {
       hdr[MDE_RING_HW * it] = m;
       hdr[MDE_RING_HW * it + 1] = need;
-      hdr[MDE_RING_HW * it + 2] = lclass;
-      hdr[MDE_RING_HW * it + 3] = (cnt < 64 ? MDE_RING_H3_PAD : 0u) | ((uint32_t)cnt << 8);
+      hdr[MDE_RING_HW * it + 2] = lclass | (flip << 2) | (Mbit << 3) | ((uint32_t)(int)K << 4);
+      hdr[MDE_RING_HW * it + 3] = (cnt < 64 ? MDE_RING_H3_PAD : 0u) | ((uint32_t)cnt << 8) | ((a_m >> 2) << 16);
     }
     __syncthreads();
   }
@@ -525,10 +551,10 @@
   bool any0 = false, any1 = false, any2 = false;
   for (int q = 0; q < 4; ++q) {
     const uint32_t* h = hdr + (size_t)MDE_RING_HW * (4 * b + q);
-    if ((h[3] >> 8) == 0u) continue;
-    any0 |= h[2] == 0u;
-    any1 |= h[2] == 1u;
-    any2 |= h[2] == 2u;
+    if (((h[3] >> 8) & 0xffu) == 0u) continue;
+    any0 |= (h[2] & 3u) == 0u;
+    any1 |= (h[2] & 3u) == 1u;
+    any2 |= (h[2] & 3u) == 2u;
   }
   const uint32_t cls = (any2 || (any0 && any1)) ? 2u : (any1 ? 1u : 0u);
   hdr[(size_t)MDE_RING_HW * 4 * b + 3] = (hdr[(size_t)MDE_RING_HW * 4 * b + 3] & ~3u) | cls;
@@ -536,10 +562,21 @@
     uint32_t* h0 = hdr + (size_t)MDE_RING_HW * (4 * b + 2 * t);
     uint32_t* h1 = h0 + MDE_RING_HW;
     uint32_t need = h0[0];
-    if ((h0[3] >> 8) != 0u) need = max(need, h0[1]);
-    if ((h1[3] >> 8) != 0u) need = max(need, h1[1]);
+    if (((h0[3] >> 8) & 0xffu) != 0u) need = max(need, h0[1]);
+    if (((h1[3] >> 8) & 0xffu) != 0u) need = max(need, h1[1]);
     h0[1] = need;
   }
+}
+
+__global__ __launch_bounds__(MDE_BLOCK) void k_ring_stream_classes(int nseg, const int32_t* __restrict__ iter_base,
+                                                                   const uint32_t* __restrict__ hdr, int32_t* __restrict__ out) {
+  const int s = blockIdx.x * MDE_BLOCK + threadIdx.x;
+  if (s >= nseg) return;
+  const int b0 = iter_base[s] >> 2, b1 = iter_base[s + 1] >> 2;
+  int c1 = 0;
+  for (int b = b0; b < b1; ++b) c1 += (hdr[(size_t)MDE_RING_HW * 4 * b + 3] & 3u) == 1u;
+  out[2 * s] = b1 - b0;
+  out[2 * s + 1] = c1;
 }
 
 __global__ __launch_bounds__(MDE_BLOCK) void k_ring_stats(int64_t nit, const uint32_t* __restrict__ hdr,
@@ -547,8 +584,8 @@
   unsigned long long a = 0, b = 0, c = 0;
   for (int64_t i = (int64_t)blockIdx.x * MDE_BLOCK + threadIdx.x; i < nit; i += (int64_t)gridDim.x * MDE_BLOCK) {
     a += (hdr[MDE_RING_HW * i + 3] & MDE_RING_H3_PAD) ? 1u : 0u;
-    b += hdr[MDE_RING_HW * i + 2] == 1u;
-    c += hdr[MDE_RING_HW * i + 2] == 2u;
+    b += (hdr[MDE_RING_HW * i + 2] & 3u) == 1u;
+    c += (hdr[MDE_RING_HW * i + 2] & 3u) == 2u;
   }
   a = mde_wave_sum(a);
   b = mde_wave_sum(b);
@@ -714,6 +751,7 @@
   void* extra[] = {L.slot_row, L.hub_rows, L.hub_seg, L.hub_first, L.hub_partial};
   for (void* q : extra)
     if (q) (void)hipFree(q);
+  free(L.wg_cls1);
   L = mde_ring_layout();
 }
 void mde_ring_release(mde_plan* plan) { ring_free(plan->ring); }
@@ -871,6 +909,16 @@
   return hipSuccess;
 }
 
+static int mde_ring_balance_group(const mde_plan* plan, const RingSizes& z, bool mapped) {
+  if (getenv("MDE_RING_BALANCE") && atoi(getenv("MDE_RING_BALANCE")) == 0) return 0;
+  if (mapped || plan->row_lo != 0 || plan->row_hi != plan->n || z.NRB < 4) return 0;
+  const double N = (double)z.NRB / (double)z.Q;
+  int G = std::max(1, (int)std::lround(0.75 * std::sqrt(std::max(N, 1.0))));
+  const int64_t window = (int64_t)(z.span + 1) * z.C;
+  while ((int64_t)G * z.R < window) ++G;
+  return 2 * G <= z.NRB ? G : 0;
+}
+
 static int build_ring(mde_plan* plan, int d, hipStream_t st) {
   RingSizes z;
   if (!choose_sizes(plan, d, &z)) return 0;
@@ -889,6 +937,7 @@
   const int64_t H_ring = rp.H_ring;
   if (H_ring <= 0) return 0;
   const int nseg = z.NRB * z.Q * MDE_RING_NCW;
+  const int balance_g = mde_ring_balance_group(plan, z, rp.mapped);
   const uint32_t JM = (1u << z.JB) - 1u;
   uint32_t *keys = nullptr, *vals = nullptr, *keys2 = nullptr, *vals2 = nullptr, *packed = nullptr, *hdr = nullptr, *wmap = nullptr;
   int32_t *hrow = nullptr, *wrows = nullptr, *seg = nullptr, *iters = nullptr, *iter_base = nullptr;
@@ -1165,7 +1214,7 @@
     hipLaunchKernelGGL(k_ring_pack, dim3(mde_grid((int64_t)total_iters * 64, MDE_BLOCK, 8192)), dim3(MDE_BLOCK), 0, st,
                        (int64_t)total_iters, nseg, iter_base, single ? cap_base : nullptr, it_ent, it_cnt, it_m, keys2, vals2, hrow,
                        plan->nbr, plan->eid, z.R, z.Q, z.C, z.S, z.ring_off, z.JB, d, (int)plan->row_lo, place, rp.permuted ? 1 : 0,
-                       packed, peid, hdr);
+                       balance_g, packed, peid, hdr);
     e = hipGetLastError();
   }
   if (e == hipSuccess) e = hipStreamSynchronize(st);
@@ -1175,6 +1224,26 @@
                      (int64_t)(total_iters / 4), hdr);
   RB(hipGetLastError());
   RB(hipStreamSynchronize(st));
+  std::vector<float> wg_cls1((size_t)z.NRB * z.Q, 0.0f);
+  {
+    int32_t* dcls = nullptr;
+    RB(hipMalloc(&dcls, sizeof(int32_t) * 2 * (size_t)nseg));
+    hipLaunchKernelGGL(k_ring_stream_classes, dim3((unsigned)((nseg + MDE_BLOCK - 1) / MDE_BLOCK)), dim3(MDE_BLOCK), 0, st, nseg,
+                       iter_base, hdr, dcls);
+    std::vector<int32_t> hcls(2 * (size_t)nseg);
+    e = hipMemcpyAsync(hcls.data(), dcls, sizeof(int32_t) * hcls.size(), hipMemcpyDeviceToHost, st);
+    if (e == hipSuccess) e = hipStreamSynchronize(st);
+    (void)hipFree(dcls);
+    if (e != hipSuccess) return fail(e, "ring layout: class shares");
+    for (size_t g = 0; g < wg_cls1.size(); ++g) {
+      int64_t nb = 0, n1 = 0;
+      for (int w = 0; w < MDE_RING_NCW; ++w) {
+        nb += hcls[2 * (g * MDE_RING_NCW + w)];
+        n1 += hcls[2 * (g * MDE_RING_NCW + w) + 1];
+      }
+      wg_cls1[g] = nb > 0 ? (float)((double)n1 / (double)nb) : 0.0f;
+    }
+  }
   if (getenv("MDE_RING_STATS")) {
     unsigned long long* dstat = reinterpret_cast<unsigned long long*>(iters);
     unsigned long long hstat[3] = {0, 0, 0};
@@ -1268,6 +1337,9 @@
   L.partial = partial;
   L.slot_row = slot_row;
   L.count_all = rp.permuted ? 1 : 0;
+  L.balance_g = balance_g;
+  L.wg_cls1 = static_cast<float*>(malloc(sizeof(float) * wg_cls1.size()));
+  if (L.wg_cls1) memcpy(L.wg_cls1, wg_cls1.data(), sizeof(float) * wg_cls1.size());
   L.n_hub_rows = (int)rp.hub_rows.size();
   L.n_hub_segs = (int)(rp.hub_seg.size() / 4);
   L.hub_half_edges = rp.hub_half_edges;
@@ -1590,6 +1662,25 @@
   info[11] = L.n_hub_rows;
   info[12] = L.hub_half_edges;
   info[13] = L.n_hub_segs;
+  return MDE_OK;
+}
+
+extern "C" int mde_plan_ring_balance(const mde_plan* plan, double* out) {
+  if (!plan || !out) return MDE_E_INVALID;
+  const mde_ring_layout& L = plan->ring;
+  for (int i = 0; i < 4; ++i) out[i] = 0.0;
+  if (!L.packed || !L.wg_cls1) return MDE_OK;
+  const int nwg = L.n_row_blocks * L.col_groups;
+  double mn = 1.0, mx = 0.0, sm = 0.0;
+  for (int g = 0; g < nwg; ++g) {
+    mn = std::min(mn, (double)L.wg_cls1[g]);
+    mx = std::max(mx, (double)L.wg_cls1[g]);
+    sm += L.wg_cls1[g];
+  }
+  out[0] = mn;
+  out[1] = sm / std::max(nwg, 1);
+  out[2] = mx;
+  out[3] = L.balance_g;
   return MDE_OK;
 }
 
diff --git a/pymde_amd/csrc/mde_ring_kernel.h b/pymde_amd/csrc/mde_ring_kernel.h
--- a/pymde_amd/csrc/mde_ring_kernel.h
+++ b/pymde_amd/csrc/mde_ring_kernel.h
@@ -101,12 +101,21 @@
 
 #if MDE_RING_ABLATE
 static __device__ unsigned long long g_ring_probe[8][1024];
+static __device__ unsigned long long g_ring_stamp[4][1024];
+#define RING_STAMP(k)                                                                       \
+  do {                                                                                      \
+    if ((dbg & 512) && tid == 0 && blockIdx.x < 1024) g_ring_stamp[k][blockIdx.x] = wall_clock64(); \
+  } while (0)
 static __device__ int g_ring_diag[64][8];
 static __device__ int g_ring_ndiag;
 #ifndef MDE_RING_SPINMAX
 #define MDE_RING_SPINMAX 100000
 #endif
 #define RING_CLK() __builtin_readcyclecounter()
+#else
+#define RING_STAMP(k) \
+  do {                \
+  } while (0)
 #endif
 #ifndef MDE_RING_FWORDS
 #define MDE_RING_FWORDS 0
@@ -144,6 +153,7 @@
   float* GR = reinterpret_cast<float*>(L + GR_OFF);
   const int tid = threadIdx.x, lane = tid & 63;
   const int wave = __builtin_amdgcn_readfirstlane(tid >> 6);
+  RING_STAMP(0);
   const int rb = blockIdx.x / Q, qg = blockIdx.x % Q;
   const int j_lo = (int)(((int64_t)qg * NC + Q - 1) / Q), j_hi = (int)(((int64_t)(qg + 1) * NC + Q - 1) / Q);
   const int r0 = rb * R;
@@ -200,6 +210,7 @@
       reinterpret_cast<float*>(L + tab_off)[tid - 64] = a0[tid - 64] * Fn::kParamScale;
   }
   __syncthreads();
+  RING_STAMP(1);
   float loss = 0.0f, loss2 = 0.0f;
 
   if (wave >= NCW) {
@@ -433,16 +444,16 @@
         return r;
       };
       auto bx4 = [&](uint32_t bw, int q) __attribute__((always_inline)) { return BX ? ((bw >> (8 * q)) & 0xffu) << 2 : 0u; };
-      auto counts_here = [&](uint32_t w, uint32_t hm) __attribute__((always_inline)) {
-        const uint32_t off = col_of(w) - (uint32_t)ring_off;
-        const uint32_t slot = off / (uint32_t)CBYTES, cidx = (off - slot * (uint32_t)CBYTES) / (4u * (uint32_t)D);
-        const uint32_t ms = hm % (uint32_t)S;
-        const uint32_t j = hm + (slot >= ms ? slot - ms : slot + (uint32_t)S - ms);
-        const uint32_t u = j * (uint32_t)C + cidx;
-        const uint32_t vv = (uint32_t)(row_lo + r0) + row_of(w) / (4u * (uint32_t)D);
-        return vv < u;
-      };
-      auto finish = [&](auto lc_tag, uint32_t w, const Pre& x, float (&acc)[D], float p1, uint32_t hm)
+      constexpr uint32_t RING_BYTES_MAX = MDE_RING_LDS_BYTES;
+      const uint32_t ring_bytes = (uint32_t)S * (uint32_t)CBYTES;
+      auto counts_here = [&](uint32_t w, uint32_t h2, uint32_t h3) __attribute__((always_inline)) {
+        static_assert(RING_BYTES_MAX < (1u << 18), "t fits 18 bits");
+        const uint32_t t0 = col_of(w) - ((h3 >> 16) << 2);
+        const uint32_t t = min(t0, t0 + ring_bytes);
+        const int rowm = (h2 & 8u) ? (int)row_of(w) : 0;
+        return (((int)t + ((int)h2 >> 4)) > rowm) != ((h2 & 4u) != 0u);
+      };
+      auto finish = [&](auto lc_tag, uint32_t w, const Pre& x, float (&acc)[D], float p1, uint32_t hm, uint32_t hm3)
           __attribute__((always_inline)) {
         constexpr int LC = decltype(lc_tag)::value;
 #ifdef MDE_RING_KEEPROW
@@ -471,7 +482,7 @@
               gc = real ? gc : 0.0f;
             }
             if constexpr (LC == 2) {
-              const bool here = counts_here(w, hm);
+              const bool here = counts_here(w, hm, hm3);
               wl = here ? wl : 0.0f;
               gc = here ? gc : 0.0f;
             }
@@ -483,7 +494,7 @@
           fn.eval(ss, x.p0, p1, f, gd);
           if constexpr (LC != 0) {
             if (!LIN) f = (rowaddr < dummy_row) ? f : 0.0f;
-            if constexpr (LC == 2) f = counts_here(w, hm) ? f : 0.0f;
+            if constexpr (LC == 2) f = counts_here(w, hm, hm3) ? f : 0.0f;
             loss += f;
           }
         }
@@ -578,15 +589,17 @@
           const float p1a = a1_arr ? a1[((size_t)((ib >> 2) + b) * 64 + lane) * 4 + q] : a1s;
           const float p1b = a1_arr ? a1[((size_t)((ib >> 2) + b) * 64 + lane) * 4 + q + 1] : a1s;
           const bool lc2 = decltype(lc_tag)::value == 2;
-          const uint32_t hma = lc2 ? (uint32_t)__builtin_amdgcn_readlane((int)hv[u], 4 * q) : 0u;
-          const uint32_t hmb = lc2 ? (uint32_t)__builtin_amdgcn_readlane((int)hv[u], 4 * q + 4) : 0u;
-          finish(lc_tag, pq[u][q], xa, acc, p1a, hma);
+          const uint32_t hma = lc2 ? (uint32_t)__builtin_amdgcn_readlane((int)hv[u], 4 * q + 2) : 0u;
+          const uint32_t hma3 = lc2 ? (uint32_t)__builtin_amdgcn_readlane((int)hv[u], 4 * q + 3) : 0u;
+          const uint32_t hmb = lc2 ? (uint32_t)__builtin_amdgcn_readlane((int)hv[u], 4 * q + 6) : 0u;
+          const uint32_t hmb3 = lc2 ? (uint32_t)__builtin_amdgcn_readlane((int)hv[u], 4 * q + 7) : 0u;
+          finish(lc_tag, pq[u][q], xa, acc, p1a, hma, hma3);
           if (HAS_GRAD) {
             const bool same = row_of(pq[u][q + 1]) == row_of(pq[u][q]);
 #pragma unroll
             for (int c = 0; c < D; ++c) accb[c] = same ? acc[c] : accb[c];
           }
-          finish(lc_tag, pq[u][q + 1], xb, accb, p1b, hmb);
+          finish(lc_tag, pq[u][q + 1], xb, accb, p1b, hmb, hmb3);
           if (HAS_GRAD) {
             ring_ld<D>(L + GR_OFF + row_of(pq[un][qn]), acc);
             ring_ld<D>(L + GR_OFF + row_of(pq[un][qn + 1]), accb);
@@ -636,6 +649,7 @@
     __builtin_amdgcn_s_waitcnt(0x0F70);
   }
   __syncthreads();
+  RING_STAMP(2);
   if (HAS_GRAD && slot_row) {
     const int32_t* sr = slot_row + (size_t)rb * R;
     if (fold) {
@@ -780,6 +794,7 @@
     if (*last_flag) __hip_atomic_store(ticket, 0u, __ATOMIC_RELAXED, __HIP_MEMORY_SCOPE_AGENT);
   }
   __syncthreads();
+  RING_STAMP(3);
   if (!*last_flag) return;
   double t = 0.0;
   for (int i = tid; i < (int)gridDim.x; i += BS) t += mde_ld_partial(loss_partials + i);
@@ -925,6 +940,60 @@
         }
         fprintf(stderr, "[mde ring probe] workgroups %d..%d: loop %.0f, minus polls %.0f\n", q8 * nb / 8, (q8 + 1) * nb / 8 - 1, a / c, b2 / c);
       }
+      std::vector<unsigned long long> hs(4 * 1024);
+      (void)hipMemcpyFromSymbol(hs.data(), HIP_SYMBOL(g_ring_stamp), sizeof(unsigned long long) * 4 * 1024);
+      unsigned long long t_first = ~0ull, t_last = 0;
+      for (int i = 0; i < nb; ++i) {
+        t_first = std::min(t_first, hs[i]);
+        t_last = std::max(t_last, hs[3 * 1024 + i]);
+      }
+      std::vector<double> pro(nb), mainp(nb), epi(nb), start(nb), fin(nb);
+      for (int i = 0; i < nb; ++i) {
+        pro[i] = 0.01 * (double)(hs[1024 + i] - hs[i]);
+        mainp[i] = 0.01 * (double)(hs[2 * 1024 + i] - hs[1024 + i]);
+        epi[i] = 0.01 * (double)(hs[3 * 1024 + i] - hs[2 * 1024 + i]);
+        start[i] = 0.01 * (double)(hs[i] - t_first);
+        fin[i] = 0.01 * (double)(t_last - hs[3 * 1024 + i]);
+      }
+      auto quant_us = [&](std::vector<double> v, const char* what) {
+        std::sort(v.begin(), v.end());
+        double m = 0;
+        for (double x : v) m += x;
+        fprintf(stderr, "[mde ring stamps] %s: min %.2f p10 %.2f median %.2f mean %.2f p90 %.2f max %.2f us\n", what, v[0], v[v.size() / 10],
+                v[v.size() / 2], m / v.size(), v[v.size() * 9 / 10], v.back());
+      };
+      fprintf(stderr, "[mde ring stamps] first entry to last exit: %.2f us\n", 0.01 * (double)(t_last - t_first));
+      quant_us(start, "entry after the first workgroup's");
+      quant_us(pro, "prologue (entry .. first barrier)");
+      quant_us(mainp, "main phase (both roles' loops)");
+      quant_us(epi, "epilogue (fold, loss tail)");
+      quant_us(fin, "exit before the last workgroup's");
+      const float* share = A.plan->ring.wg_cls1;
+      for (int q8 = 0; q8 < 8; ++q8) {
+        double a = 0, b2 = 0, c1 = 0, mx = 0;
+        int c = 0;
+        for (int i = q8 * nb / 8; i < (q8 + 1) * nb / 8; ++i, ++c) {
+          a += mainp[i];
+          b2 += loop[i];
+          c1 += share ? share[i] : 0.0;
+          mx = std::max(mx, mainp[i]);
+        }
+        fprintf(stderr, "[mde ring stamps] workgroups %d..%d: class-1 share %.3f, main phase mean %.2f max %.2f us, consumer loop %.0f clk\n",
+                q8 * nb / 8, (q8 + 1) * nb / 8 - 1, c1 / c, a / c, mx, b2 / c);
+      }
+      if (share) {
+        double sx = 0, sy = 0, sxx = 0, sxy = 0;
+        for (int i = 0; i < nb; ++i) {
+          sx += share[i];
+          sy += mainp[i];
+          sxx += (double)share[i] * share[i];
+          sxy += (double)share[i] * mainp[i];
+        }
+        const double den = nb * sxx - sx * sx;
+        const double b1 = den > 0 ? (nb * sxy - sx * sy) / den : 0.0;
+        fprintf(stderr, "[mde ring stamps] main phase ~ %.2f us + %.2f us x class-1 share (least squares over %d workgroups)\n",
+                (sy - b1 * sx) / nb, b1, nb);
+      }
     }
   }
 #endif
```

Result: no change. 320.5 billion edges/s/iter, median of 5 (-0.0%).
